# OpenVisualCloud/SVT-VP9

Hardware: AMD Instinct MI355X
Metric: hot-path frames/sec (+ Mpixels/sec): block-level DSP path (picture analysis + ME + inter prediction from reconstructed references + DCT/quant/recon + deblock + reference padding), 3840x2160p60 yuv420p enc-mode 8; no mode decision, no entropy coding -- not encoded frames (higher is better)
Workload: dtype u8

## Files before the change

### svt-vp9_amd/csrc/encdec.hip

```cpp
#include <hip/hip_runtime.h>
#include <stdlib.h>
#include <string.h>
#include "svt_ctx.h"
#include "encdec_core.h"

#define ED_MAX_PICS 32
#define ED_MAX_SETS 8

struct svt_encdec_work {
    int           max_pics, width, height, n_sb, sb_cols, mi_rows, mi_cols;
    size_t        cap_per_pic;
    svt_tq_block *d_blocks;
    void         *last_hb;
    uint32_t     *d_pos;
    uint16_t     *d_eob;
    int32_t      *d_counts;
    int32_t      *d_totals, *d_bases;
    int32_t      *d_off_cnt;
    int32_t      *d_status;
    int32_t      *d_intra_sync;
    svt_quant_tables *d_qtabs;
    int16_t      *d_iscan;
    svt_encdec_stage_hook hook;
    void         *hook_user;
};

namespace {

struct ed_pic_dev {
    const svt_me_pu_result *res;
    svt_mc_mode_info       *mc_mi;
    svt_lf_mode_info       *lf_mi;
    uint8_t                *nz;
    uint16_t               *eob_map;
    svt_lf_mask            *lfm;
    svt_tq_pic_geom         g;
};
struct ed_batch_dev {
    ed_pic_dev pic[ED_MAX_PICS];
    uint32_t   iscan_off[16];
    int32_t    n_pics, n_sb, sb_cols, mi_rows, mi_cols, mi_stride, width, height;
    uint32_t   lambda;
    int32_t    filter_level;
};

__device__ __forceinline__ int wave_sum(int v) {
    _Pragma("unroll") for (int d = 32; d >= 1; d >>= 1) v += __shfl_xor(v, d, 64);
    return v;
}
__device__ __forceinline__ int wave_excl_prefix(int v, int lane) {
    int incl = v;
    _Pragma("unroll") for (int d = 1; d < 64; d <<= 1) {
        const int o = __shfl_up(incl, d, 64);
        if (lane >= d) incl += o;
    }
    return incl - v;
}

__global__ __launch_bounds__(64) void svt_tq_count_kernel(const ed_batch_dev *__restrict__ B, int32_t *__restrict__ counts, int32_t *__restrict__ status) {
    const int sb = (int)blockIdx.x % B->n_sb, pic = (int)blockIdx.x / B->n_sb, lane = (int)threadIdx.x;
    const ed_pic_dev &P = B->pic[pic];
    const int ur = (sb / B->sb_cols) * 8 + (lane >> 3), uc = (sb % B->sb_cols) * 8 + (lane & 7);
    int cnt[4] = {0, 0, 0, 0};
    if (ur < B->mi_rows && uc < B->mi_cols) P.nz[ur * B->mi_stride + uc] = 0;
    const int o = svt_tq_unit_is_origin(P.lf_mi, B->mi_stride, B->mi_rows, B->mi_cols, ur, uc);
    if (o < 0) atomicOr(status, 1);
    if (o == 1) svt_tq_unit_counts(P.lf_mi, B->mi_stride, ur, uc, cnt);
    _Pragma("unroll") for (int s = 0; s < 4; s++) {
        const int v = wave_sum(cnt[s]);
        if (lane == 0) counts[(s * B->n_pics + pic) * B->n_sb + sb] = v;
    }
}

__global__ __launch_bounds__(256) void svt_scan_sb_kernel(int32_t *__restrict__ a, int n_sb, int32_t *__restrict__ totals) {
    __shared__ int32_t part[256];
    int32_t *p = a + (size_t)blockIdx.x * n_sb;
    const int t = (int)threadIdx.x, per = (n_sb + 255) / 256, b = t * per, e = b + per < n_sb ? b + per : n_sb;
    int s = 0;
    for (int i = b; i < e; i++) s += p[i];
    part[t] = s;
    __syncthreads();
    for (int d = 1; d < 256; d <<= 1) {
        const int v = t >= d ? part[t - d] : 0;
        __syncthreads();
        part[t] += v;
        __syncthreads();
    }
    int run = part[t] - s;
    for (int i = b; i < e; i++) { const int v = p[i]; p[i] = run; run += v; }
    if (t == 255) totals[blockIdx.x] = part[255];
}
__global__ __launch_bounds__(64) void svt_scan_pic_kernel(const int32_t *__restrict__ totals, int n_pics, int32_t *__restrict__ bases, int32_t *__restrict__ off_cnt) {
    if (threadIdx.x != 0) return;
    int run = 0;
    for (int s = 0; s < 4; s++) {
        off_cnt[s] = run;
        for (int p = 0; p < n_pics; p++) { bases[s * n_pics + p] = run; run += totals[s * n_pics + p]; }
        off_cnt[4 + s] = run - off_cnt[s];
    }
}

__global__ __launch_bounds__(256) void svt_tq_expand_kernel(const ed_batch_dev *__restrict__ B, const int32_t *__restrict__ off_cnt, const uint32_t *__restrict__ pos,
                                                           svt_tq_block *__restrict__ blocks) {
    const int i = (int)blockIdx.x * 256 + (int)threadIdx.x, total = off_cnt[3] + off_cnt[7];
    if (i >= total) return;
    const int      ts = i >= off_cnt[3] ? 3 : i >= off_cnt[2] ? 2 : i >= off_cnt[1] ? 1 : 0;
    const uint32_t p = pos[i];
    svt_tq_block   k;
    svt_tq_block_from_pos(p, ts, &B->pic[svt_tq_pos_pic(p)].g, B->iscan_off, B->sb_cols, &k);
    blocks[i] = k;
}

__global__ __launch_bounds__(64) void svt_tq_emit_kernel(const ed_batch_dev *__restrict__ B, const int32_t *__restrict__ offsets, const int32_t *__restrict__ bases,
                                                         svt_tq_block *__restrict__ blocks, uint32_t *__restrict__ pos) {
    const int sb = (int)blockIdx.x % B->n_sb, pic = (int)blockIdx.x / B->n_sb, lane = (int)threadIdx.x;
    const ed_pic_dev &P = B->pic[pic];
    const int ur = (sb / B->sb_cols) * 8 + (lane >> 3), uc = (sb % B->sb_cols) * 8 + (lane & 7);
    int cnt[4] = {0, 0, 0, 0};
    const int o = svt_tq_unit_is_origin(P.lf_mi, B->mi_stride, B->mi_rows, B->mi_cols, ur, uc);
    if (o == 1) svt_tq_unit_counts(P.lf_mi, B->mi_stride, ur, uc, cnt);
    uint32_t base[4];
    _Pragma("unroll") for (int s = 0; s < 4; s++) base[s] = (uint32_t)(bases[s * B->n_pics + pic] + offsets[(s * B->n_pics + pic) * B->n_sb + sb] + wave_excl_prefix(cnt[s], lane));
    if (o == 1) svt_tq_unit_emit(P.lf_mi, B->mi_stride, ur, uc, &P.g, B->iscan_off, base, blocks, pos);
}

__global__ __launch_bounds__(256) void svt_tq_skip_kernel(const ed_batch_dev *__restrict__ B, const int32_t *__restrict__ off_cnt, const uint32_t *__restrict__ pos,
                                                          const uint16_t *__restrict__ eob) {
    const int total = off_cnt[3] + off_cnt[7];
    const int w4 = B->width >> 2, h4 = B->height >> 2;
    for (int i = (int)(blockIdx.x * blockDim.x + threadIdx.x); i < total; i += (int)(gridDim.x * blockDim.x)) {
        const uint32_t p = pos[i];
        const int      pic = (int)(p >> 24) & 63, plane = (int)(p >> 22) & 3, y4 = (int)(p >> 11) & 0x7ff, x4 = (int)p & 0x7ff;
        const ed_pic_dev &P = B->pic[pic];
        const int      e = eob[i];
        const int      pw4 = plane ? w4 >> 1 : w4;
        const int      off = plane == 0 ? 0 : w4 * h4 + (plane == 2 ? (w4 >> 1) * (h4 >> 1) : 0);
        P.eob_map[off + y4 * pw4 + x4] = (uint16_t)e;
        if (e) {
            const int uy = plane ? y4 : y4 >> 1, ux = plane ? x4 : x4 >> 1;
            const svt_lf_mode_info b = P.lf_mi[uy * B->mi_stride + ux];
            const int w8 = svt_blk_w8(b.sb_type), h8 = svt_blk_h8(b.sb_type);
            P.nz[(uy - uy % h8) * B->mi_stride + (ux - ux % w8)] = 1;
        }
    }
}
__global__ __launch_bounds__(256) void svt_eob_map_clear_kernel(const ed_batch_dev *__restrict__ B, int n16) {
    uint4 *m = (uint4 *)B->pic[blockIdx.y].eob_map;
    for (int i = (int)(blockIdx.x * 256 + threadIdx.x); i < n16; i += (int)(gridDim.x * 256)) m[i] = make_uint4(0, 0, 0, 0);
}
__global__ __launch_bounds__(256) void svt_skip_update_kernel(const ed_batch_dev *__restrict__ B) {
    const int units = B->mi_rows * B->mi_cols;
    const int i = (int)(blockIdx.x * blockDim.x + threadIdx.x);
    if (i >= units * B->n_pics) return;
    const int pic = i / units, u = i % units, ur = u / B->mi_cols, uc = u % B->mi_cols;
    const ed_pic_dev &P = B->pic[pic];
    svt_lf_mode_info *b = &P.lf_mi[ur * B->mi_stride + uc];
    if (b->sb_type > 12) return;
    const int w8 = svt_blk_w8(b->sb_type), h8 = svt_blk_h8(b->sb_type);
    b->skip = P.nz[(ur - ur % h8) * B->mi_stride + (uc - uc % w8)] ? 0 : 1;
}

__device__ __forceinline__ uint32_t wave_or(uint32_t v) {
    _Pragma("unroll") for (int d = 32; d >= 1; d >>= 1) v |= (uint32_t)__shfl_xor((int)v, d, 64);
    return v;
}
__global__ __launch_bounds__(64) void svt_lf_mask_kernel(const ed_batch_dev *__restrict__ B, int32_t *__restrict__ status) {
    const int sb = (int)blockIdx.x % B->n_sb, pic = (int)blockIdx.x / B->n_sb, lane = (int)threadIdx.x;
    const ed_pic_dev &P = B->pic[pic];
    svt_lf_unit_masks u;
    svt_lf_mask_unit(P.lf_mi, B->mi_stride, B->mi_rows, B->mi_cols, sb / B->sb_cols, sb % B->sb_cols, lane >> 3, lane & 7, &u);
    if (u.bad && status) atomicOr(status, 1);
    __shared__ uint32_t sm[40];
    uint64_t            w64[9];
    _Pragma("unroll") for (int i = 0; i < 4; i++) { w64[i] = u.left_y[i]; w64[4 + i] = u.above_y[i]; }
    w64[8] = u.int_4x4_y;
    _Pragma("unroll") for (int i = 0; i < 9; i++) {
        const uint32_t lo = wave_or((uint32_t)w64[i]), hi = wave_or((uint32_t)(w64[i] >> 32));
        if (lane == i) { sm[2 * i] = lo; sm[2 * i + 1] = hi; }
    }
    const uint32_t c0 = wave_or((uint32_t)u.left_uv[0] | (uint32_t)u.left_uv[1] << 16), c1 = wave_or((uint32_t)u.left_uv[2] | (uint32_t)u.left_uv[3] << 16);
    const uint32_t c2 = wave_or((uint32_t)u.above_uv[0] | (uint32_t)u.above_uv[1] << 16), c3 = wave_or((uint32_t)u.above_uv[2] | (uint32_t)u.above_uv[3] << 16);
    const uint32_t c4 = wave_or((uint32_t)u.int_4x4_uv);
    if (lane == 9) { sm[18] = c0; sm[19] = c1; sm[20] = c2; sm[21] = c3; sm[22] = c4; sm[38] = 0; sm[39] = 0; }
    __syncthreads();
    ((uint8_t *)sm)[90 + lane] = u.level;
    __syncthreads();
    if (lane < 40) ((uint32_t *)&P.lfm[sb])[lane] = sm[lane];
}

__global__ __launch_bounds__(64) void svt_md_default_kernel(const ed_batch_dev *__restrict__ B) {
    const int sb = (int)blockIdx.x % B->n_sb, pic = (int)blockIdx.x / B->n_sb, lane = (int)threadIdx.x;
    const ed_pic_dev &P = B->pic[pic];
    const int r = lane >> 3, c = lane & 7, sr = sb / B->sb_cols, sc = sb % B->sb_cols, ur = sr * 8 + r, uc = sc * 8 + c;
    if (ur >= B->mi_rows || uc >= B->mi_cols) return;
    svt_md_default_unit(P.res + (size_t)sb * SVT_ME_PU_COUNT, r, c, sr, sc, B->mi_rows, B->mi_cols, B->lambda, B->filter_level, &P.mc_mi[ur * B->mi_stride + uc],
                        &P.lf_mi[ur * B->mi_stride + uc]);
}

int stage_batch(svt_hip_ctx *ctx, const ed_batch_dev &hb, const ed_batch_dev **d_out) {
    void *h = nullptr, *d = nullptr;
    if (svt_ctx_stage(ctx, sizeof hb, &h, &d)) return -1;
    memcpy(h, &hb, sizeof hb);
    if (hipMemcpyAsync(d, h, sizeof hb, hipMemcpyHostToDevice, ctx->stream) != hipSuccess) return -1;
    svt_ctx_stage_commit(ctx);
    *d_out = (const ed_batch_dev *)d;
    return 0;
}

void fill_dims(ed_batch_dev &hb, int n_pics, int width, int height, int mi_stride) {
    hb.n_pics = n_pics; hb.width = width; hb.height = height;
    hb.sb_cols = (width + 63) >> 6;
    hb.n_sb = hb.sb_cols * ((height + 63) >> 6);
    hb.mi_rows = height >> 3; hb.mi_cols = width >> 3; hb.mi_stride = mi_stride;
}

}

extern "C" int32_t svt_hip_encdec_work_create(svt_hip_ctx *ctx, int32_t max_pics, int32_t width, int32_t height, svt_encdec_work **out) {
    if (!ctx || !out || max_pics < 1 || max_pics > ED_MAX_PICS || width < 8 || height < 8 || (width & 7) || (height & 7))
        return svt_set_error(SVT_HIP_ERR_BAD_PARAMETER, "encdec_work: bad argument");
    HIP_TRY(hipSetDevice(ctx->device));
    svt_encdec_work *w = (svt_encdec_work *)calloc(1, sizeof *w);
    if (!w) return svt_set_error(SVT_HIP_ERR_NO_RESOURCES, "encdec_work: malloc");
    w->max_pics = max_pics; w->width = width; w->height = height;
    w->sb_cols = (width + 63) >> 6; w->n_sb = w->sb_cols * ((height + 63) >> 6);
    w->mi_rows = height >> 3; w->mi_cols = width >> 3;
    w->cap_per_pic = (size_t)width * height * 3 / 32;
    const size_t cap = w->cap_per_pic * (size_t)max_pics;
    const size_t n_cnt = (size_t)4 * max_pics * w->n_sb;
    uint32_t const *offs = nullptr;
    int32_t         entries = 0;
    const int16_t  *isc = svt_hip_vp9_iscan_tables(&offs, &entries);
    bool ok = hipMalloc((void **)&w->d_pos, cap * sizeof(uint32_t)) == hipSuccess &&
              hipMalloc((void **)&w->d_eob, cap * sizeof(uint16_t)) == hipSuccess &&
              hipMalloc((void **)&w->d_counts, (n_cnt + 9 + 8 * ED_MAX_PICS + 2 + 48 * (size_t)w->n_sb) * sizeof(int32_t)) == hipSuccess &&
              hipMalloc((void **)&w->d_qtabs, 2 * sizeof(svt_quant_tables)) == hipSuccess && hipMalloc((void **)&w->d_iscan, (size_t)entries * sizeof(int16_t)) == hipSuccess;
    if (ok) {
        w->d_off_cnt = w->d_counts + n_cnt;
        w->d_status = w->d_off_cnt + 8;
        w->d_totals = w->d_status + 1;
        w->d_bases = w->d_totals + 4 * ED_MAX_PICS;
        w->d_intra_sync = w->d_bases + 4 * ED_MAX_PICS;
        ok = hipMemsetAsync(w->d_off_cnt, 0, 9 * sizeof(int32_t), ctx->stream) == hipSuccess &&
             hipMemcpyAsync(w->d_iscan, isc, (size_t)entries * sizeof(int16_t), hipMemcpyHostToDevice, ctx->stream) == hipSuccess &&
             hipStreamSynchronize(ctx->stream) == hipSuccess;
    }
    if (!ok) {
        svt_hip_encdec_work_destroy(ctx, w);
        return svt_set_error(SVT_HIP_ERR_NO_RESOURCES, "encdec_work: device memory");
    }
    *out = w;
    return SVT_HIP_OK;
}

extern "C" void svt_hip_encdec_work_destroy(svt_hip_ctx *ctx, svt_encdec_work *w) {
    if (!w) return;
    if (ctx) { (void)hipSetDevice(ctx->device); (void)hipStreamSynchronize(ctx->stream); }
    void *v[6] = {w->d_blocks, w->d_pos, w->d_eob, w->d_counts, w->d_qtabs, w->d_iscan};
    for (int i = 0; i < 6; i++) if (v[i]) (void)hipFree(v[i]);
    free(w->last_hb);
    free(w);
}

extern "C" int32_t svt_hip_encdec_batch_device(svt_hip_ctx *ctx, svt_encdec_work *w, int32_t n_pics, const svt_encdec_picture *pics, int32_t width,
                                               int32_t height, int32_t mi_stride, int32_t q_index, const svt_encdec_flags *flags, const svt_lf_thresh *thr,
                                               int32_t pad_x, int32_t pad_y) {
    if (!ctx || !w || !pics || !flags || n_pics < 1 || n_pics > w->max_pics || width != w->width || height != w->height || mi_stride < (width >> 3))
        return svt_set_error(SVT_HIP_ERR_BAD_PARAMETER, "encdec: bad argument");
    if (flags->apply_loop_filter && !thr) return svt_set_error(SVT_HIP_ERR_BAD_PARAMETER, "encdec: loop filter without thresholds");
    HIP_TRY(hipSetDevice(ctx->device));
    uintptr_t src_lo = UINTPTR_MAX, src_hi = 0, pred_lo = UINTPTR_MAX, pred_hi = 0;
    for (int i = 0; i < n_pics; i++) {
        const svt_encdec_picture &p = pics[i];
        if (!p.d_mc_mi || !p.d_lf_mi || !p.src.y || !p.src.u || !p.src.v || !p.pred.y || !p.pred.u || !p.pred.v || !p.recon.y || !p.recon.u || !p.recon.v ||
            !p.d_qcoeff || !p.d_eob_map || !p.d_nz || (flags->apply_loop_filter && !p.d_lfm))
            return svt_set_error(SVT_HIP_ERR_BAD_PARAMETER, "encdec: null picture field");
        if (!p.d_dqcoeff != !pics[0].d_dqcoeff) return svt_set_error(SVT_HIP_ERR_BAD_PARAMETER, "encdec: d_dqcoeff must be given for every picture of a batch or for none");
        if (((uintptr_t)p.d_qcoeff | (uintptr_t)p.d_dqcoeff) & 15) return svt_set_error(SVT_HIP_ERR_BAD_PARAMETER, "encdec: coefficient arrays must be 16-byte aligned");
        const uint8_t *s3[3] = {p.src.y, p.src.u, p.src.v}, *p3[3] = {p.pred.y, p.pred.u, p.pred.v};
        for (int k = 0; k < 3; k++) {
            src_lo = (uintptr_t)s3[k] < src_lo ? (uintptr_t)s3[k] : src_lo; src_hi = (uintptr_t)s3[k] > src_hi ? (uintptr_t)s3[k] : src_hi;
            pred_lo = (uintptr_t)p3[k] < pred_lo ? (uintptr_t)p3[k] : pred_lo; pred_hi = (uintptr_t)p3[k] > pred_hi ? (uintptr_t)p3[k] : pred_hi;
        }
    }
    uint64_t plane_span = 0;
    for (int i = 0; i < n_pics; i++) {
        const svt_yuv_planes *pl[3] = {&pics[i].src, &pics[i].pred, &pics[i].recon};
        for (int k = 0; k < 3; k++) {
            const uint64_t a = (uint64_t)(pl[k]->y_stride > 0 ? pl[k]->y_stride : 0) * (uint64_t)height, b = (uint64_t)(pl[k]->uv_stride > 0 ? pl[k]->uv_stride : 0) * (uint64_t)(height / 2);
            plane_span = a > plane_span ? a : plane_span;
            plane_span = b > plane_span ? b : plane_span;
        }
    }
    if ((uint64_t)(src_hi - src_lo) + plane_span >= (1ull << 32) || (uint64_t)(pred_hi - pred_lo) + plane_span >= (1ull << 32))
        return svt_set_error(SVT_HIP_ERR_BAD_PARAMETER, "encdec: the batch's source / prediction planes must lie within 4 GB");
    uintptr_t q_lo = UINTPTR_MAX, dq_lo = UINTPTR_MAX;
    for (int i = 0; i < n_pics; i++) {
        q_lo = (uintptr_t)pics[i].d_qcoeff < q_lo ? (uintptr_t)pics[i].d_qcoeff : q_lo;
        dq_lo = (uintptr_t)pics[i].d_dqcoeff < dq_lo ? (uintptr_t)pics[i].d_dqcoeff : dq_lo;
    }
    ed_batch_dev hb;
    memset(&hb, 0, sizeof hb);
    fill_dims(hb, n_pics, width, height, mi_stride);
    {
        const uint32_t *offs = nullptr;
        (void)svt_hip_vp9_iscan_tables(&offs, nullptr);
        for (int i = 0; i < 16; i++) hb.iscan_off[i] = offs[i];
    }
    uint8_t       *recon_set[ED_MAX_SETS];
    int            n_sets = 0;
    {
        uintptr_t lo[ED_MAX_PICS], hi[ED_MAX_PICS];
        int       order[ED_MAX_PICS];
        for (int i = 0; i < n_pics; i++) {
            const uint8_t *r3[3] = {pics[i].recon.y, pics[i].recon.u, pics[i].recon.v};
            lo[i] = UINTPTR_MAX; hi[i] = 0; order[i] = i;
            for (int k = 0; k < 3; k++) { lo[i] = (uintptr_t)r3[k] < lo[i] ? (uintptr_t)r3[k] : lo[i]; hi[i] = (uintptr_t)r3[k] > hi[i] ? (uintptr_t)r3[k] : hi[i]; }
        }
        for (int a = 1; a < n_pics; a++)
            for (int b = a; b > 0 && lo[order[b]] < lo[order[b - 1]]; b--) { const int t_ = order[b]; order[b] = order[b - 1]; order[b - 1] = t_; }
        for (int a = 0; a < n_pics; a++) {
            const int i = order[a];
            if (n_sets && (uint64_t)(hi[i] - (uintptr_t)recon_set[n_sets - 1]) + plane_span < (1ull << 32)) continue;
            if (n_sets == ED_MAX_SETS || (uint64_t)(hi[i] - lo[i]) + plane_span >= (1ull << 32))
                return svt_set_error(SVT_HIP_ERR_BAD_PARAMETER, "encdec: the batch's reconstruction buffers span more than 8 regions of 4 GB");
            recon_set[n_sets++] = (uint8_t *)lo[i];
        }
    }
    svt_mc_picture mcp[ED_MAX_PICS];
    svt_yuv_planes rec[ED_MAX_PICS], rec_pad[ED_MAX_PICS];
    int            n_rec_pad = 0;
    const svt_lf_mask *lfm[ED_MAX_PICS];
    int32_t        lfm_stride[ED_MAX_PICS], mi_rows_a[ED_MAX_PICS], mi_cols_a[ED_MAX_PICS];
    for (int i = 0; i < n_pics; i++) {
        const svt_encdec_picture &p = pics[i];
        ed_pic_dev &P = hb.pic[i];
        P.mc_mi = (svt_mc_mode_info *)p.d_mc_mi; P.lf_mi = p.d_lf_mi; P.nz = p.d_nz; P.eob_map = p.d_eob_map; P.lfm = p.d_lfm;
        const uintptr_t q_off = ((uintptr_t)p.d_qcoeff - q_lo) / sizeof(int16_t), dq_off = ((uintptr_t)p.d_dqcoeff - dq_lo) / sizeof(int16_t);
        if ((p.d_dqcoeff && q_off != dq_off) || q_off + (uint64_t)hb.n_sb * SVT_SB_COEFFS >= (1ull << 32))
            return svt_set_error(SVT_HIP_ERR_BAD_PARAMETER, "encdec: qcoeff / dqcoeff of the batch must be laid out alike, within 2^32 elements");
        const uint8_t *r3[3] = {p.recon.y, p.recon.u, p.recon.v};
        uintptr_t r_lo = UINTPTR_MAX, r_hi = 0;
        for (int k = 0; k < 3; k++) { r_lo = (uintptr_t)r3[k] < r_lo ? (uintptr_t)r3[k] : r_lo; r_hi = (uintptr_t)r3[k] > r_hi ? (uintptr_t)r3[k] : r_hi; }
        int set = -1;
        for (int k = n_sets - 1; k >= 0 && set < 0; k--)
            if (r_lo >= (uintptr_t)recon_set[k] && (uint64_t)(r_hi - (uintptr_t)recon_set[k]) + plane_span < (1ull << 32)) set = k;
        if (set < 0) return svt_set_error(SVT_HIP_ERR_BAD_PARAMETER, "encdec: the batch's reconstruction buffers span more than 8 regions of 4 GB");
        svt_tq_pic_geom &g = P.g;
        const uint8_t *s3[3] = {p.src.y, p.src.u, p.src.v}, *p3[3] = {p.pred.y, p.pred.u, p.pred.v};
        for (int k = 0; k < 3; k++) {
            g.src_off[k] = (uint32_t)((uintptr_t)s3[k] - src_lo); g.pred_off[k] = (uint32_t)((uintptr_t)p3[k] - pred_lo);
            g.recon_off[k] = (uint32_t)((uintptr_t)r3[k] - (uintptr_t)recon_set[set]);
        }
        if (p.src.y_stride > 65535 || p.pred.y_stride > 65535 || p.recon.y_stride > 65535) return svt_set_error(SVT_HIP_ERR_BAD_PARAMETER, "encdec: stride");
        g.src_stride[0] = (uint16_t)p.src.y_stride; g.src_stride[1] = (uint16_t)p.src.uv_stride;
        g.pred_stride[0] = (uint16_t)p.pred.y_stride; g.pred_stride[1] = (uint16_t)p.pred.uv_stride;
        g.recon_stride[0] = (uint16_t)p.recon.y_stride; g.recon_stride[1] = (uint16_t)p.recon.uv_stride;
        g.coeff_base = (uint32_t)q_off; g.width = width; g.height = height; g.recon_set = (uint8_t)set; g.pic = (uint8_t)i; g.do_recon = flags->do_recon ? 1 : 0;
        mcp[i].d_mi = p.d_mc_mi; mcp[i].mi_stride = mi_stride; mcp[i].mi_rows = hb.mi_rows; mcp[i].mi_cols = hb.mi_cols;
        mcp[i].ref[0] = p.ref[0]; mcp[i].ref[1] = p.ref[1]; mcp[i].pred = p.pred; mcp[i].use_subpel = p.use_subpel;
        rec[i] = p.recon; rec[i].width = width; rec[i].height = height;
        if (!p.no_pad) rec_pad[n_rec_pad++] = rec[i];
        lfm[i] = p.d_lfm; lfm_stride[i] = hb.sb_cols; mi_rows_a[i] = hb.mi_rows; mi_cols_a[i] = hb.mi_cols;
    }
    const ed_batch_dev *dB = nullptr;
    if (stage_batch(ctx, hb, &dB)) return svt_set_error(SVT_HIP_ERR_NO_RESOURCES, "encdec: descriptor buffers");
    {
        svt_quant_tables qt[2];
        if (svt_hip_quant_tables_for_qindex(q_index, qt) != SVT_HIP_OK) return svt_set_error(SVT_HIP_ERR_BAD_PARAMETER, "encdec: q index");
        void *h = nullptr, *d = nullptr;
        if (svt_ctx_stage(ctx, sizeof qt, &h, &d)) return svt_set_error(SVT_HIP_ERR_NO_RESOURCES, "encdec: descriptor buffers");
        memcpy(h, qt, sizeof qt);
        HIP_TRY(hipMemcpyAsync(w->d_qtabs, h, sizeof qt, hipMemcpyHostToDevice, ctx->stream));
        svt_ctx_stage_commit(ctx);
    }
#define ED_STAGE(k) do { if (w->hook) w->hook(w->hook_user, (k)); } while (0)
    ED_STAGE(SVT_ENCDEC_STAGE_MC);
    int32_t rc = svt_hip_inter_pred_batch_device(ctx, n_pics, mcp);
    if (rc) return rc;
    ED_STAGE(SVT_ENCDEC_STAGE_LISTS);
    const int nwg = n_pics * hb.n_sb;
    hipLaunchKernelGGL(svt_tq_count_kernel, dim3(nwg), dim3(64), 0, ctx->stream, dB, w->d_counts, w->d_status);
    hipLaunchKernelGGL(svt_scan_sb_kernel, dim3(4 * n_pics), dim3(256), 0, ctx->stream, w->d_counts, hb.n_sb, w->d_totals);
    hipLaunchKernelGGL(svt_scan_pic_kernel, dim3(1), dim3(64), 0, ctx->stream, (const int32_t *)w->d_totals, n_pics, w->d_bases, w->d_off_cnt);
    hipLaunchKernelGGL(svt_tq_emit_kernel, dim3(nwg), dim3(64), 0, ctx->stream, dB, (const int32_t *)w->d_counts, (const int32_t *)w->d_bases, (svt_tq_block *)nullptr, w->d_pos);
    HIP_TRY(hipGetLastError());
    if (!w->last_hb) w->last_hb = malloc(sizeof hb);
    if (w->last_hb) memcpy(w->last_hb, &hb, sizeof hb);
    ED_STAGE(SVT_ENCDEC_STAGE_TQ);
    int32_t cap[4];
    for (int s = 0; s < 4; s++) cap[s] = (int32_t)((size_t)n_pics * width * height * 3 / 2 / (size_t)(16 << (2 * s)));
    rc = svt_tq_launch_device_lists(ctx, (const uint8_t *)src_lo, (const uint8_t *)pred_lo, recon_set, n_sets, nullptr, cap, w->d_off_cnt, w->d_qtabs, w->d_iscan,
                                    (int16_t *)q_lo, (int16_t *)dq_lo, w->d_eob, nullptr, w->d_pos, &dB->pic[0].g, (int)sizeof(ed_pic_dev), dB->iscan_off, hb.sb_cols);
    if (rc) return rc;
    ED_STAGE(SVT_ENCDEC_STAGE_SKIP);
    {
        const size_t map_bytes = (size_t)(width / 4) * (height / 4) * 3 / 2 * sizeof(uint16_t);
        uintptr_t    low = map_bytes;
        for (int i = 0; i < n_pics; i++) low |= (uintptr_t)pics[i].d_eob_map;
        if (!(low & 15))
            hipLaunchKernelGGL(svt_eob_map_clear_kernel, dim3(64, n_pics), dim3(256), 0, ctx->stream, dB, (int)(map_bytes / 16));
        else
            for (int i = 0; i < n_pics; i++) HIP_TRY(hipMemsetAsync(pics[i].d_eob_map, 0, map_bytes, ctx->stream));
    }
    for (int i = 0; i < n_pics; i++)
        if (pics[i].has_intra) {
            if (!flags->do_recon) return svt_set_error(SVT_HIP_ERR_BAD_PARAMETER, "encdec: intra blocks need the reconstruction (do_recon)");
            rc = svt_intra_launch(ctx, &pics[i], width, height, mi_stride, w->d_qtabs, w->d_iscan, hb.iscan_off, w->d_intra_sync, w->d_status, 1);
            if (rc) return rc;
        }
    {
        const int total_cap = (int)(w->cap_per_pic * (size_t)n_pics);
        int       g = (total_cap + 255) / 256;
        if (g > ctx->cu_count * 8) g = ctx->cu_count * 8;
        hipLaunchKernelGGL(svt_tq_skip_kernel, dim3(g), dim3(256), 0, ctx->stream, dB, (const int32_t *)w->d_off_cnt, (const uint32_t *)w->d_pos, (const uint16_t *)w->d_eob);
        hipLaunchKernelGGL(svt_skip_update_kernel, dim3((n_pics * hb.mi_rows * hb.mi_cols + 255) / 256), dim3(256), 0, ctx->stream, dB);
        HIP_TRY(hipGetLastError());
    }
    ED_STAGE(SVT_ENCDEC_STAGE_LF);
    if (flags->apply_loop_filter) {
        hipLaunchKernelGGL(svt_lf_mask_kernel, dim3(nwg), dim3(64), 0, ctx->stream, dB, w->d_status);
        HIP_TRY(hipGetLastError());
        rc = svt_hip_lf_batch_device(ctx, n_pics, rec, lfm, lfm_stride, thr, mi_rows_a, mi_cols_a, 0);
        if (rc) return rc;
    }
    ED_STAGE(SVT_ENCDEC_STAGE_PAD);
    if (flags->pad_reference && n_rec_pad) {
        rc = svt_hip_ref_pad_batch_device(ctx, n_rec_pad, rec_pad, pad_x, pad_y);
        if (rc) return rc;
    }
    ED_STAGE(SVT_ENCDEC_STAGE_END);
    return SVT_HIP_OK;
}

extern "C" int32_t svt_hip_encdec_intra_device(svt_hip_ctx *ctx, svt_encdec_work *w, const svt_encdec_picture *pic, int32_t width, int32_t height, int32_t mi_stride,
                                               int32_t q_index, const svt_encdec_flags *flags, const svt_lf_thresh *thr, int32_t pad_x, int32_t pad_y) {
    if (!ctx || !w || !pic || !flags || width != w->width || height != w->height || mi_stride < (width >> 3))
        return svt_set_error(SVT_HIP_ERR_BAD_PARAMETER, "encdec_intra: bad argument");
    if (!flags->do_recon) return svt_set_error(SVT_HIP_ERR_BAD_PARAMETER, "encdec_intra: intra prediction needs the reconstruction (do_recon)");
    if (flags->apply_loop_filter && !thr) return svt_set_error(SVT_HIP_ERR_BAD_PARAMETER, "encdec_intra: loop filter without thresholds");
    const svt_encdec_picture &p = *pic;
    if (!p.d_lf_mi || !p.src.y || !p.src.u || !p.src.v || !p.recon.y || !p.recon.u || !p.recon.v || !p.d_qcoeff || !p.d_eob_map || !p.d_nz ||
        (flags->apply_loop_filter && !p.d_lfm))
        return svt_set_error(SVT_HIP_ERR_BAD_PARAMETER, "encdec_intra: null picture field");
    if (((uintptr_t)p.d_qcoeff | (uintptr_t)p.d_dqcoeff) & 15) return svt_set_error(SVT_HIP_ERR_BAD_PARAMETER, "encdec_intra: coefficient arrays must be 16-byte aligned");
    if (p.recon.y_stride > 65535 || ((p.src.y_stride | p.src.uv_stride | p.recon.y_stride | p.recon.uv_stride) & 3) ||
        (((uintptr_t)p.src.y | (uintptr_t)p.src.u | (uintptr_t)p.src.v | (uintptr_t)p.recon.y | (uintptr_t)p.recon.u | (uintptr_t)p.recon.v) & 3) ||
        (p.pred.y && (((uintptr_t)p.pred.y | (uintptr_t)p.pred.u | (uintptr_t)p.pred.v | (uintptr_t)p.pred.y_stride | (uintptr_t)p.pred.uv_stride) & 3)))
        return svt_set_error(SVT_HIP_ERR_BAD_PARAMETER, "encdec_intra: planes and strides must be 4-byte aligned");
    if (p.pred.y && (!p.pred.u || !p.pred.v)) return svt_set_error(SVT_HIP_ERR_BAD_PARAMETER, "encdec_intra: prediction planes");
    HIP_TRY(hipSetDevice(ctx->device));
    ed_batch_dev hb;
    memset(&hb, 0, sizeof hb);
    fill_dims(hb, 1, width, height, mi_stride);
    const uint32_t *offs = nullptr;
    (void)svt_hip_vp9_iscan_tables(&offs, nullptr);
    hb.pic[0].lf_mi = p.d_lf_mi; hb.pic[0].nz = p.d_nz; hb.pic[0].eob_map = p.d_eob_map; hb.pic[0].lfm = p.d_lfm;
    const ed_batch_dev *dB = nullptr;
    if (stage_batch(ctx, hb, &dB)) return svt_set_error(SVT_HIP_ERR_NO_RESOURCES, "encdec_intra: descriptor buffers");
    {
        svt_quant_tables qt[2];
        if (svt_hip_quant_tables_for_qindex(q_index, qt) != SVT_HIP_OK) return svt_set_error(SVT_HIP_ERR_BAD_PARAMETER, "encdec_intra: q index");
        void *h = nullptr, *d = nullptr;
        if (svt_ctx_stage(ctx, sizeof qt, &h, &d)) return svt_set_error(SVT_HIP_ERR_NO_RESOURCES, "encdec_intra: descriptor buffers");
        memcpy(h, qt, sizeof qt);
        HIP_TRY(hipMemcpyAsync(w->d_qtabs, h, sizeof qt, hipMemcpyHostToDevice, ctx->stream));
        svt_ctx_stage_commit(ctx);
    }
    ED_STAGE(SVT_ENCDEC_STAGE_TQ);
    HIP_TRY(hipMemsetAsync(p.d_eob_map, 0, (size_t)(width / 4) * (height / 4) * 3 / 2 * sizeof(uint16_t), ctx->stream));
    HIP_TRY(hipMemsetAsync(p.d_nz, 0, (size_t)mi_stride * hb.mi_rows, ctx->stream));
    int32_t rc = svt_intra_launch(ctx, pic, width, height, mi_stride, w->d_qtabs, w->d_iscan, offs, w->d_intra_sync, w->d_status, 0);
    if (rc) return rc;
    ED_STAGE(SVT_ENCDEC_STAGE_SKIP);
    hipLaunchKernelGGL(svt_skip_update_kernel, dim3((hb.mi_rows * hb.mi_cols + 255) / 256), dim3(256), 0, ctx->stream, dB);
    HIP_TRY(hipGetLastError());
    ED_STAGE(SVT_ENCDEC_STAGE_LF);
    svt_yuv_planes rec = p.recon;
    rec.width = width; rec.height = height;
    if (flags->apply_loop_filter) {
        hipLaunchKernelGGL(svt_lf_mask_kernel, dim3(hb.n_sb), dim3(64), 0, ctx->stream, dB, w->d_status);
        HIP_TRY(hipGetLastError());
        const svt_lf_mask *lfm = p.d_lfm;
        const int32_t      lfm_stride = hb.sb_cols, mr = hb.mi_rows, mc = hb.mi_cols;
        rc = svt_hip_lf_batch_device(ctx, 1, &rec, &lfm, &lfm_stride, thr, &mr, &mc, 0);
        if (rc) return rc;
    }
    ED_STAGE(SVT_ENCDEC_STAGE_PAD);
    if (flags->pad_reference && !p.no_pad) {
        rc = svt_hip_ref_pad_batch_device(ctx, 1, &rec, pad_x, pad_y);
        if (rc) return rc;
    }
    ED_STAGE(SVT_ENCDEC_STAGE_END);
    return SVT_HIP_OK;
}

extern "C" int32_t svt_hip_md_intra_default_device(svt_hip_ctx *ctx, int32_t width, int32_t height, int32_t filter_level, svt_lf_mode_info *d_lf_mi, int32_t mi_stride) {
    if (!ctx || !d_lf_mi || width < 8 || height < 8 || (width & 7) || (height & 7) || mi_stride < (width >> 3))
        return svt_set_error(SVT_HIP_ERR_BAD_PARAMETER, "md_intra_default: bad argument");
    HIP_TRY(hipSetDevice(ctx->device));
    return svt_md_intra_default_launch(ctx, d_lf_mi, mi_stride, height >> 3, width >> 3, filter_level);
}

extern "C" void svt_hip_encdec_work_set_stage_hook(svt_encdec_work *w, svt_encdec_stage_hook hook, void *user) {
    if (!w) return;
    w->hook = hook;
    w->hook_user = user;
}

extern "C" int32_t svt_hip_encdec_work_status(svt_hip_ctx *ctx, svt_encdec_work *w, int32_t counts[8]) {
    if (!ctx || !w) return svt_set_error(SVT_HIP_ERR_BAD_PARAMETER, "encdec_status: null");
    HIP_TRY(hipSetDevice(ctx->device));
    int32_t h[9];
    HIP_TRY(hipMemcpyAsync(h, w->d_off_cnt, sizeof h, hipMemcpyDeviceToHost, ctx->stream));
    HIP_TRY(hipStreamSynchronize(ctx->stream));
    if (counts) memcpy(counts, h, 8 * sizeof(int32_t));
    if (h[8]) {
        HIP_TRY(hipMemsetAsync(w->d_status, 0, sizeof(int32_t), ctx->stream));
        return svt_set_error(SVT_HIP_ERR_BAD_PARAMETER, "encdec: malformed mode-info grid (block outside the picture, misaligned, or transform larger than its block)");
    }
    return SVT_HIP_OK;
}

extern "C" int32_t svt_hip_encdec_work_download(svt_hip_ctx *ctx, svt_encdec_work *w, svt_tq_block *blocks, uint32_t *pos, uint16_t *eob, int32_t capacity) {
    int32_t c[8];
    const int32_t rc = svt_hip_encdec_work_status(ctx, w, c);
    if (rc) return rc;
    const int32_t total = c[3] + c[7];
    if (total > capacity) return svt_set_error(SVT_HIP_ERR_NO_RESOURCES, "encdec_download: capacity");
    if (total > 0) {
        if (blocks) {
            if (!w->last_hb) return svt_set_error(SVT_HIP_ERR_BAD_PARAMETER, "encdec_download: no batch yet");
            if (!w->d_blocks && hipMalloc((void **)&w->d_blocks, w->cap_per_pic * (size_t)w->max_pics * sizeof(svt_tq_block)) != hipSuccess) {
                w->d_blocks = nullptr;
                return svt_set_error(SVT_HIP_ERR_NO_RESOURCES, "encdec_download: device memory");
            }
            const ed_batch_dev *dB = nullptr;
            if (stage_batch(ctx, *(const ed_batch_dev *)w->last_hb, &dB)) return svt_set_error(SVT_HIP_ERR_NO_RESOURCES, "encdec_download: descriptor buffers");
            hipLaunchKernelGGL(svt_tq_expand_kernel, dim3((total + 255) / 256), dim3(256), 0, ctx->stream, dB, (const int32_t *)w->d_off_cnt, (const uint32_t *)w->d_pos, w->d_blocks);
            HIP_TRY(hipGetLastError());
            HIP_TRY(hipMemcpyAsync(blocks, w->d_blocks, (size_t)total * sizeof(svt_tq_block), hipMemcpyDeviceToHost, ctx->stream));
        }
        if (pos) HIP_TRY(hipMemcpyAsync(pos, w->d_pos, (size_t)total * sizeof(uint32_t), hipMemcpyDeviceToHost, ctx->stream));
        if (eob) HIP_TRY(hipMemcpyAsync(eob, w->d_eob, (size_t)total * sizeof(uint16_t), hipMemcpyDeviceToHost, ctx->stream));
        HIP_TRY(hipStreamSynchronize(ctx->stream));
    }
    return total;
}

extern "C" int32_t svt_hip_md_default_batch_device(svt_hip_ctx *ctx, int32_t n_pics, const svt_me_pu_result *const *d_results, int32_t width, int32_t height,
                                                   uint32_t lambda, int32_t filter_level, svt_mc_mode_info *const *d_mc_mi, svt_lf_mode_info *const *d_lf_mi,
                                                   int32_t mi_stride) {
    if (!ctx || n_pics < 1 || !d_results || !d_mc_mi || !d_lf_mi || width < 8 || height < 8 || (width & 7) || (height & 7) || mi_stride < (width >> 3))
        return svt_set_error(SVT_HIP_ERR_BAD_PARAMETER, "md_default: bad argument");
    HIP_TRY(hipSetDevice(ctx->device));
    for (int first = 0; first < n_pics; first += ED_MAX_PICS) {
        const int n = n_pics - first < ED_MAX_PICS ? n_pics - first : ED_MAX_PICS;
        ed_batch_dev hb;
        memset(&hb, 0, sizeof hb);
        fill_dims(hb, n, width, height, mi_stride);
        hb.lambda = lambda; hb.filter_level = filter_level;
        for (int i = 0; i < n; i++) {
            if (!d_results[first + i] || !d_mc_mi[first + i] || !d_lf_mi[first + i]) return svt_set_error(SVT_HIP_ERR_BAD_PARAMETER, "md_default: null picture");
            hb.pic[i].res = d_results[first + i]; hb.pic[i].mc_mi = d_mc_mi[first + i]; hb.pic[i].lf_mi = d_lf_mi[first + i];
        }
        const ed_batch_dev *dB = nullptr;
        if (stage_batch(ctx, hb, &dB)) return svt_set_error(SVT_HIP_ERR_NO_RESOURCES, "md_default: descriptor buffers");
        hipLaunchKernelGGL(svt_md_default_kernel, dim3(n * hb.n_sb), dim3(64), 0, ctx->stream, dB);
        HIP_TRY(hipGetLastError());
    }
    return SVT_HIP_OK;
}

extern "C" int32_t svt_hip_lf_build_masks_device(svt_hip_ctx *ctx, int32_t n_pics, const svt_lf_mode_info *const *d_lf_mi, int32_t mi_stride, int32_t mi_rows,
                                                 int32_t mi_cols, svt_lf_mask *const *d_lfm) {
    if (!ctx || n_pics < 1 || !d_lf_mi || !d_lfm || mi_rows < 1 || mi_cols < 1 || mi_stride < mi_cols) return svt_set_error(SVT_HIP_ERR_BAD_PARAMETER, "lf_masks: bad argument");
    HIP_TRY(hipSetDevice(ctx->device));
    for (int first = 0; first < n_pics; first += ED_MAX_PICS) {
        const int n = n_pics - first < ED_MAX_PICS ? n_pics - first : ED_MAX_PICS;
        ed_batch_dev hb;
        memset(&hb, 0, sizeof hb);
        fill_dims(hb, n, mi_cols * 8, mi_rows * 8, mi_stride);
        for (int i = 0; i < n; i++) {
            if (!d_lf_mi[first + i] || !d_lfm[first + i]) return svt_set_error(SVT_HIP_ERR_BAD_PARAMETER, "lf_masks: null picture");
            hb.pic[i].lf_mi = (svt_lf_mode_info *)d_lf_mi[first + i]; hb.pic[i].lfm = d_lfm[first + i];
        }
        const ed_batch_dev *dB = nullptr;
        if (stage_batch(ctx, hb, &dB)) return svt_set_error(SVT_HIP_ERR_NO_RESOURCES, "lf_masks: descriptor buffers");
        hipLaunchKernelGGL(svt_lf_mask_kernel, dim3(n * hb.n_sb), dim3(64), 0, ctx->stream, dB, (int32_t *)nullptr);
        HIP_TRY(hipGetLastError());
    }
    return SVT_HIP_OK;
}
```

### svt-vp9_amd/csrc/lf_kernel.hip

```cpp
#include <hip/hip_runtime.h>
#include <cstdio>
#include <cstdlib>
#include "svt_ctx.h"

namespace {

struct lf_pic_dev {
    svt_yuv_planes     planes;
    const svt_lf_mask *lfm;
    int32_t            lfm_stride, mi_rows, mi_cols, y_only;
    uint32_t          *progress;
    const uint32_t    *desc;
};

__device__ unsigned long long g_lf_prof[8];
__device__ unsigned long long g_lf_rowts[64][8];

constexpr int LF_DESC_WORDS = 320;
constexpr int YS = 76, YROWS = 72;
constexpr int CS = 44, CROWS = 40;

__device__ __forceinline__ int iabs(int v) { return v < 0 ? -v : v; }
__device__ __forceinline__ int sclamp(int t) { return t < -128 ? -128 : t > 127 ? 127 : t; }
__device__ __forceinline__ int uclamp(int t) { return t < 0 ? 0 : t > 255 ? 255 : t; }
// ... 195 lines not shown
    lf_fetch<ROW>(s, st, nxt);
    for (int c = 0; c < nblk; c++) {
        lf_unpack<ROW>(nxt, q);
        const uint32_t e0 = w0, e1 = w1;
        if (c + 1 < nblk) {
            w0 = tab[2 * (c + 1) * tstep]; w1 = tab[2 * (c + 1) * tstep + 1];
            lf_fetch<ROW>(ROW ? s + 8 * (c + 1) : s + 8 * (c + 1) * st, st, nxt);
        }
        lf_block_edges(p, q, e0);
        if (ROW) row_store8(s + 8 * c - 8, p, true); else col_store8(s + (8 * c - 8) * st, st, p, true);
        lf_inner_edge(q, e1);
        _Pragma("unroll") for (int i = 0; i < 8; i++) p[i] = q[7 - i];
    }
    if (ROW) row_store8(s + 8 * nblk - 8, p, true); else col_store8(s + (8 * nblk - 8) * st, st, p, true);
}

struct lf_magic_table {
    uint32_t v[33];
    constexpr lf_magic_table() : v() { for (uint32_t d = 1; d <= 32; d++) v[d] = (uint32_t)(0xffffffffu / d) + 1u; }
};
__constant__ const lf_magic_table lf_magics = lf_magic_table();
__device__ __forceinline__ int lf_udiv(int t, int d, uint32_t inv) { return d > 32 ? t / d : inv ? (int)__umulhi((uint32_t)t, inv) : t; }

template <int UNITS, typename UT>
__device__ __forceinline__ void tile_io_t(bool load, uint8_t *g, int gstride, uint8_t *l, int lstride, int x0, int y0, int tx0, int ty0,
                                          int nx, int ny, int seam_lo_end, int seam_hi_begin, int lane, int nlanes,
                                          const volatile int LF_LDS *wait_flag, int wait_val) {
    constexpr int UB = (int)sizeof(UT);
    const int nu = nx / UB, total = nu * ny;
    const uint32_t inv = lf_magics.v[nu <= 32 ? nu : 0];
    for (int t0 = lane; t0 < total; t0 += UNITS * nlanes) {
        UT  v[UNITS];
        int lo[UNITS];
        _Pragma("unroll") for (int u = 0; u < UNITS; u++) {
            const int t = t0 + u * nlanes;
            lo[u] = -1;
            if (t < total) {
                const int  r = lf_udiv(t, nu, inv), ty = ty0 + r, tx = tx0 + UB * (t - r * nu);
                UT LF_GLOBAL *gp = LF_AS_GLOBAL(UT, g + (ptrdiff_t)(y0 + ty) * gstride + x0 + tx);
                const bool seam = ty < seam_lo_end || ty >= seam_hi_begin;
                lo[u] = ty * lstride + tx;
                if (load) v[u] = seam ? __hip_atomic_load(gp, __ATOMIC_RELAXED, __HIP_MEMORY_SCOPE_AGENT) : *gp;
                else {
                    const uint32_t *lp = (const uint32_t *)(l + lo[u]);
                    UT              w = (UT)lp[0];
                    if constexpr (UB == 8) w |= (UT)lp[1] << 32;
                    if (seam) __hip_atomic_store(gp, w, __ATOMIC_RELAXED, __HIP_MEMORY_SCOPE_AGENT);
                    else *gp = w;
                }
            }
        }
        if (load) {
            if (wait_flag) while (*wait_flag < wait_val) __builtin_amdgcn_s_sleep(1);
            _Pragma("unroll") for (int u = 0; u < UNITS; u++)
                if (lo[u] >= 0) {
                    uint32_t *lp = (uint32_t *)(l + lo[u]);
                    lp[0] = (uint32_t)v[u];
                    if constexpr (UB == 8) lp[1] = (uint32_t)(v[u] >> 32);
                }
        }
    }
}
template <int UNITS>
__device__ __forceinline__ void tile_io(bool wide, bool load, uint8_t *g, int gstride, uint8_t *l, int lstride, int x0, int y0, int tx0,
                                        int ty0, int nx, int ny, int seam_lo_end, int seam_hi_begin, int lane, int nlanes,
                                        const volatile int LF_LDS *wait_flag = nullptr, int wait_val = 0) {
    if (wide) tile_io_t<UNITS, unsigned long long>(load, g, gstride, l, lstride, x0, y0, tx0, ty0, nx, ny, seam_lo_end, seam_hi_begin, lane, nlanes, wait_flag, wait_val);
    else tile_io_t<2 * UNITS, unsigned int>(load, g, gstride, l, lstride, x0, y0, tx0, ty0, nx, ny, seam_lo_end, seam_hi_begin, lane, nlanes, wait_flag, wait_val);
}

struct lf_geom {
    int x0, y0, cx0, cy0, hx, hy, vw, vh, cvw, cvh;
};
__device__ __forceinline__ lf_geom lf_geometry(int sb_row, int sc, int W, int H) {
    lf_geom g;
    const int CW = W >> 1, CH = H >> 1;
    g.x0 = sc * 64; g.y0 = sb_row * 64; g.cx0 = sc * 32; g.cy0 = sb_row * 32;
    g.hx = sc > 0 ? 8 : 0; g.hy = sb_row > 0 ? 8 : 0;
    g.vw = (W - g.x0) < 64 ? W - g.x0 : 64; g.vh = (H - g.y0) < 64 ? H - g.y0 : 64;
    g.cvw = (CW - g.cx0) < 32 ? CW - g.cx0 : 32; g.cvh = (CH - g.cy0) < 32 ? CH - g.cy0 : 32;
    return g;
}

__global__ __launch_bounds__(128) void svt_lf_desc_kernel(const lf_pic_dev *__restrict__ pics, int rows_per_pic, int max_cols, svt_lf_thresh thr) {
    __shared__ uint32_t s_thr[64];
    if (threadIdx.x < 64) s_thr[threadIdx.x] = (uint32_t)thr.mblim[threadIdx.x] | ((uint32_t)thr.lim[threadIdx.x] << 8) | ((uint32_t)thr.hev_thr[threadIdx.x] << 16);
    __syncthreads();
    const int pic = blockIdx.x / (rows_per_pic * max_cols), rem = blockIdx.x - pic * rows_per_pic * max_cols;
    const int sb_row = rem / max_cols, sc = rem - sb_row * max_cols;
    const lf_pic_dev P = pics[pic];
    const int sb_cols = (P.mi_cols + 7) >> 3, sb_rows = (P.mi_rows + 7) >> 3;
    if (sb_row >= sb_rows || sc >= sb_cols) return;
    const int tid = threadIdx.x, mi_row = sb_row * 8;
    uint32_t LF_GLOBAL *d = LF_AS_GLOBAL(uint32_t, const_cast<uint32_t *>(P.desc) + ((size_t)sb_row * sb_cols + sc) * LF_DESC_WORDS);
    const svt_lf_mask LF_GLOBAL *gm = LF_AS_GLOBAL(const svt_lf_mask, &P.lfm[sb_row * P.lfm_stride + sc]);
    const uint8_t LF_GLOBAL     *lfl = gm->lfl_y;
    svt_lf_mask        m;
    _Pragma("unroll") for (int i = 0; i < 4; i++) { m.left_y[i] = gm->left_y[i]; m.above_y[i] = gm->above_y[i]; m.left_uv[i] = gm->left_uv[i]; m.above_uv[i] = gm->above_uv[i]; }
    m.int_4x4_y = gm->int_4x4_y; m.int_4x4_uv = gm->int_4x4_uv;
    adjust_mask(m, mi_row, sc * 8, P.mi_rows, P.mi_cols);
    if (tid < 64) {
        const int rr = tid >> 3, c = tid & 7, pair = rr >> 1, half = rr & 1;
        uint32_t w0, w1;
        lf_entry2(vert_entry(c, 8, (unsigned)(m.left_y[2] >> (16 * pair)) & 0xffff, (unsigned)(m.left_y[1] >> (16 * pair)) & 0xffff,
                            (unsigned)(m.left_y[0] >> (16 * pair)) & 0xffff, (unsigned)(m.int_4x4_y >> (16 * pair)) & 0xffff, half,
                            lfl[(2 * pair) * 8 + c], lfl[(2 * pair + 1) * 8 + c]), s_thr, w0, w1);
        d[2 * tid] = w0; d[2 * tid + 1] = w1;
        const int r = rr;
        unsigned  a16 = 0, a8 = 0, a4 = 0;
        if (mi_row + r != 0) { a16 = (unsigned)(m.above_y[2] >> (8 * r)) & 0xff; a8 = (unsigned)(m.above_y[1] >> (8 * r)) & 0xff; a4 = (unsigned)(m.above_y[0] >> (8 * r)) & 0xff; }
        lf_entry2(horiz_entry(c, a16, a8, a4, (unsigned)(m.int_4x4_y >> (8 * r)) & 0xff, &lfl[r * 8], 1), s_thr, w0, w1);
        d[128 + 2 * tid] = w0; d[129 + 2 * tid] = w1;
    } else if (tid < 80) {
        const int t = tid - 64, rr = t >> 2, c = t & 3, pair = rr >> 1, half = rr & 1;
        uint32_t w0, w1;
        lf_entry2(vert_entry(c, 4, (unsigned)(m.left_uv[2] >> (8 * pair)) & 0xff, (unsigned)(m.left_uv[1] >> (8 * pair)) & 0xff,
                                (unsigned)(m.left_uv[0] >> (8 * pair)) & 0xff, (unsigned)(m.int_4x4_uv >> (8 * pair)) & 0xff, half,
                                lfl[(4 * pair) * 8 + 2 * c], lfl[(4 * pair + 2) * 8 + 2 * c]), s_thr, w0, w1);
        d[256 + 2 * t] = w0; d[257 + 2 * t] = w1;
    } else if (tid < 96) {
        const int t = tid - 80, ru = t >> 2, c = t & 3, r = 2 * ru;
        unsigned  a16 = 0, a8 = 0, a4 = 0;
        if (mi_row + r != 0) { a16 = (unsigned)(m.above_uv[2] >> (4 * ru)) & 0xf; a8 = (unsigned)(m.above_uv[1] >> (4 * ru)) & 0xf; a4 = (unsigned)(m.above_uv[0] >> (4 * ru)) & 0xf; }
        const unsigned mi4 = (mi_row + r == P.mi_rows - 1) ? 0u : ((unsigned)(m.int_4x4_uv >> (4 * ru)) & 0xf);
        uint32_t w0, w1;
        lf_entry2(horiz_entry(c, a16, a8, a4, mi4, &lfl[r * 8], 2), s_thr, w0, w1);
        d[288 + 2 * t] = w0; d[289 + 2 * t] = w1;
    }
}

__global__ __launch_bounds__(256) __attribute__((amdgpu_waves_per_eu(4, 4))) void svt_lf_kernel(const lf_pic_dev *__restrict__ pics, int n_pics,
                                                     uint32_t *__restrict__ ticket, int rows_per_pic, int prof) {
    __shared__ __align__(16) uint8_t ytile[2][YROWS * YS];
    __shared__ __align__(16) uint8_t ctile[2][2][CROWS * CS];
    __shared__ uint32_t              s_desc[2][LF_DESC_WORDS];
    __shared__ int                   s_job;
    __shared__ int                   s_stored_;
    __shared__ int                   s_halo_;
    __shared__ int                   s_vdone_[2];
    const int tid = threadIdx.x;
    for (;;) {
    __syncthreads();
    volatile int LF_LDS &s_stored = *(volatile int LF_LDS *)&s_stored_;
    volatile int LF_LDS &s_halo   = *(volatile int LF_LDS *)&s_halo_;
    volatile int LF_LDS *s_vdone  = (volatile int LF_LDS *)s_vdone_;
    if (tid == 0) { s_job = (int)atomicAdd(ticket, 1u); s_stored = -1; s_halo = -1; s_vdone[0] = -1; s_vdone[1] = -1; }
    __syncthreads();
    const int job = s_job;
    if (job >= n_pics * rows_per_pic) break;
    const lf_pic_dev P = pics[job % n_pics];
    const int sb_row = job / n_pics;
    const int sb_cols = (P.mi_cols + 7) >> 3, sb_rows = (P.mi_rows + 7) >> 3;
    if (sb_row >= sb_rows) continue;
    const int W = P.planes.width, H = P.planes.height;
    const int mi_row = sb_row * 8;
    const int wave = tid >> 6, lane = tid & 63;
    const int nrows = P.mi_rows - mi_row < 8 ? P.mi_rows - mi_row : 8;
    const bool wide_y = (((uintptr_t)P.planes.y | (uintptr_t)P.planes.y_stride) & 7) == 0;
    const bool wide_c = (((uintptr_t)P.planes.u | (uintptr_t)P.planes.v | (uintptr_t)P.planes.uv_stride) & 7) == 0;
    unsigned long long tm_ = prof ? __builtin_amdgcn_s_memtime() : 0;
    const bool rowts = prof && job % n_pics == 0 && sb_row < 64;
#define LF_ROWTS(k, who, cond) do { if (rowts && tid == (who) && (cond)) g_lf_rowts[sb_row][k] = __builtin_amdgcn_s_memtime(); } while (0)
    LF_ROWTS(0, 0, true);
#define LF_MARK(i, who) do { if (prof && tid == (who)) { unsigned long long n_ = __builtin_amdgcn_s_memtime(); atomicAdd(&g_lf_prof[i], n_ - tm_); tm_ = n_; } } while (0)

    auto stage_halo = [&](int sc) {
        const int     buf = sc & 1;
// ... 30 lines not shown

    if (wave == 2) stage(0);
    __syncthreads();
    for (int sc = 0; sc < sb_cols; sc++) {
        const int     buf = sc & 1;
        const lf_geom g = lf_geometry(sb_row, sc, W, H);
        const bool    last = sc + 1 == sb_cols;
        if (wave == 2) {
            stage_halo(sc);
            if (!last) stage(sc + 1);
        } else if (wave == 0) {
            if (lane < g.vh) lf_line<true>(ytile[buf] + (8 + lane) * YS + 8, 1, 8, &s_desc[buf][2 * (lane >> 3) * 8], 1);
            if (lane == 0) s_vdone[0] = sc;
            LF_ROWTS(4, 0, sc == 1);
            LF_MARK(3, 0);
            while (s_halo < sc) __builtin_amdgcn_s_sleep(1);
            if (lane < g.vw) lf_line<false>(ytile[buf] + 8 * YS + 8 + lane, YS, nrows, &s_desc[buf][128 + 2 * (lane >> 3)], 8);
            LF_MARK(4, 0);
            LF_ROWTS(2, 0, sc == 0);
            LF_ROWTS(5, 0, last);
            if (!last) {
                while (s_stored < sc - 1) __builtin_amdgcn_s_sleep(1);
                for (int r = lane; r < YROWS; r += 64) {
                    const uint32_t *src = (const uint32_t *)(ytile[buf] + r * YS + 64);
                    uint32_t       *dst = (uint32_t *)(ytile[buf ^ 1] + r * YS);
                    dst[0] = src[0]; dst[1] = src[1];
                }
            }
        } else if (wave == 1 && !P.y_only) {
            const int pl = lane >> 5, l5 = lane & 31;
            if (l5 < g.cvh) lf_line<true>(ctile[buf][pl] + (8 + l5) * CS + 8, 1, 4, &s_desc[buf][256 + 2 * (l5 >> 3) * 4], 1);
            if (lane == 0) s_vdone[1] = sc;
            while (s_halo < sc) __builtin_amdgcn_s_sleep(1);
            if (l5 < g.cvw) lf_line<false>(ctile[buf][pl] + 8 * CS + 8 + l5, CS, (nrows + 1) >> 1, &s_desc[buf][288 + 2 * (l5 >> 3)], 4);
            if (!last) {
                while (s_stored < sc - 1) __builtin_amdgcn_s_sleep(1);
                for (int r = l5; r < CROWS; r += 32) {
                    const uint32_t *src = (const uint32_t *)(ctile[buf][pl] + r * CS + 32);
                    uint32_t       *dst = (uint32_t *)(ctile[buf ^ 1][pl] + r * CS);
                    dst[0] = src[0]; dst[1] = src[1];
                }
            }
        }
        __syncthreads();
        LF_MARK(5, 0);
        if (wave == 3) {
            const bool below = sb_row + 1 < sb_rows;
            const int  nown = last ? g.vw : 56, nownc = last ? g.cvw : 24, cut = below ? 8 : 0;
            tile_io<11>(wide_y, false, P.planes.y, P.planes.y_stride, ytile[buf], YS, g.x0 - 8, g.y0 - 8, 8, 8 - g.hy, nown, g.vh + g.hy, 8, 8 + g.vh - 8, lane, 64);
            if (g.hx) tile_io<2>(wide_y, false, P.planes.y, P.planes.y_stride, ytile[buf], YS, g.x0 - 8, g.y0 - 8, 0, 8 - g.hy, 8, g.vh + g.hy - cut, 8, 8 + g.vh - 8, lane, 64);
            if (!P.y_only) {
                _Pragma("unroll") for (int pl = 0; pl < 2; pl++) {
                    uint8_t *cp = pl ? P.planes.v : P.planes.u;
                    tile_io<3>(wide_c, false, cp, P.planes.uv_stride, ctile[buf][pl], CS, g.cx0 - 8, g.cy0 - 8, 8, 8 - g.hy, nownc, g.cvh + g.hy, 8, 8 + g.cvh - 8, lane, 64);
                    if (g.hx) tile_io<1>(wide_c, false, cp, P.planes.uv_stride, ctile[buf][pl], CS, g.cx0 - 8, g.cy0 - 8, 0, 8 - g.hy, 8, g.cvh + g.hy - cut, 8, 8 + g.cvh - 8, lane, 64);
                }
            }
            asm volatile("s_waitcnt lgkmcnt(0)" ::: "memory");
            if (lane == 0) s_stored = sc;
            LF_MARK(6, 192);
            if (!last && below) {
                while (s_vdone[0] < sc + 1) __builtin_amdgcn_s_sleep(1);
                const lf_geom gn = lf_geometry(sb_row, sc + 1, W, H);
                tile_io<1>(wide_y, false, P.planes.y, P.planes.y_stride, ytile[buf ^ 1], YS, gn.x0 - 8, gn.y0 - 8, 0, 8 + gn.vh - 8, 8, 8, 1 << 20, 0, lane, 64);
                if (!P.y_only) {
                    while (s_vdone[1] < sc + 1) __builtin_amdgcn_s_sleep(1);
                    tile_io<1>(wide_c, false, P.planes.u, P.planes.uv_stride, ctile[buf ^ 1][0], CS, gn.cx0 - 8, gn.cy0 - 8, 0, 8 + gn.cvh - 8, 8, 8, 1 << 20, 0, lane, 64);
                    tile_io<1>(wide_c, false, P.planes.v, P.planes.uv_stride, ctile[buf ^ 1][1], CS, gn.cx0 - 8, gn.cy0 - 8, 0, 8 + gn.cvh - 8, 8, 8, 1 << 20, 0, lane, 64);
                }
            }
            asm volatile("s_waitcnt vmcnt(0)" ::: "memory");
            if (lane == 0) __hip_atomic_store(LF_AS_GLOBAL(uint32_t, &P.progress[sb_row]), (uint32_t)(sc + 1), __ATOMIC_RELAXED, __HIP_MEMORY_SCOPE_AGENT);
            LF_ROWTS(3, 192, sc == 0);
            LF_ROWTS(6, 192, last);
            LF_MARK(7, 192);
        }
    }
#undef LF_MARK
#undef LF_ROWTS
    }
}
}

static int32_t lf_launch(svt_hip_ctx *ctx, int n_pics, const svt_yuv_planes *d_recon, const svt_lf_mask *const *d_lfm, const int32_t *lfm_stride,
                         const svt_lf_thresh *thr, const int32_t *mi_rows, const int32_t *mi_cols, int32_t y_only) {
    int max_rows = 0, max_cols = 0;
    for (int i = 0; i < n_pics; i++) {
        if (mi_rows[i] < 1 || mi_cols[i] < 1 || d_recon[i].width != mi_cols[i] * 8 || d_recon[i].height != mi_rows[i] * 8)
            return svt_set_error(SVT_HIP_ERR_BAD_PARAMETER, "lf: plane size must be mi_cols*8 x mi_rows*8");
        const svt_yuv_planes &pl = d_recon[i];
        if ((((uintptr_t)pl.y | (uintptr_t)pl.y_stride) & 3) || (!y_only && (((uintptr_t)pl.u | (uintptr_t)pl.v | (uintptr_t)pl.uv_stride) & 3)))
            return svt_set_error(SVT_HIP_ERR_BAD_PARAMETER, "lf: plane pointers and strides must be multiples of 4 bytes");
        const int r = (mi_rows[i] + 7) / 8, cc = (mi_cols[i] + 7) / 8;
        if (r > max_rows) max_rows = r;
        if (cc > max_cols) max_cols = cc;
    }
    HIP_TRY(hipSetDevice(ctx->device));
    const size_t desc_bytes = (sizeof(lf_pic_dev) * (size_t)n_pics + 15) & ~(size_t)15;
    const size_t cnt_words  = (size_t)n_pics * max_rows + 4;
    lf_pic_dev  *h = nullptr;
    uint8_t     *d = nullptr;
    if (svt_ctx_stage(ctx, desc_bytes + cnt_words * 4, (void **)&h, (void **)&d)) return svt_set_error(SVT_HIP_ERR_NO_RESOURCES, "lf: scratch");
    uint32_t *cnt = (uint32_t *)(d + desc_bytes);
    uint32_t *edesc = (uint32_t *)svt_ctx_slot(ctx, 24, (size_t)n_pics * max_rows * max_cols * LF_DESC_WORDS * sizeof(uint32_t));
    if (!edesc) return svt_set_error(SVT_HIP_ERR_NO_RESOURCES, "lf: descriptor buffer");
    for (int i = 0; i < n_pics; i++) {
        h[i].planes = d_recon[i]; h[i].lfm = d_lfm[i]; h[i].lfm_stride = lfm_stride[i]; h[i].mi_rows = mi_rows[i]; h[i].mi_cols = mi_cols[i];
        h[i].y_only = y_only; h[i].progress = cnt + 4 + (size_t)i * max_rows;
        h[i].desc = edesc + (size_t)i * max_rows * max_cols * LF_DESC_WORDS;
    }
    HIP_TRY(hipMemcpyAsync(d, h, sizeof(lf_pic_dev) * (size_t)n_pics, hipMemcpyHostToDevice, ctx->stream));
    HIP_TRY(hipMemsetAsync(cnt, 0, cnt_words * 4, ctx->stream));
    HIP_TRY(hipEventRecord(ctx->ev_start, ctx->stream));
    static const bool want_prof = getenv("SVT_HIP_LF_PROFILE") != nullptr;
    if (want_prof) { unsigned long long z[8] = {0}; HIP_TRY(hipMemcpyToSymbol(HIP_SYMBOL(g_lf_prof), z, sizeof z)); }
    hipLaunchKernelGGL(svt_lf_desc_kernel, dim3(n_pics * max_rows * max_cols), dim3(128), 0, ctx->stream, (const lf_pic_dev *)d, max_rows, max_cols, *thr);
    hipLaunchKernelGGL(svt_lf_kernel, dim3(n_pics * max_rows), dim3(256), 0, ctx->stream, (const lf_pic_dev *)d, n_pics, cnt, max_rows, want_prof ? 1 : 0);
    HIP_TRY(hipGetLastError());
    HIP_TRY(hipEventRecord(ctx->ev_stop, ctx->stream));
    if (want_prof) {
        unsigned long long hp[8];
        HIP_TRY(hipStreamSynchronize(ctx->stream));
        HIP_TRY(hipMemcpyFromSymbol(hp, HIP_SYMBOL(g_lf_prof), sizeof hp));
        static const char *nm[8] = {"io:wait", "io:tile_load", "io:descriptors", "filter:vertical", "filter:horizontal+halo", "filter:barrier",
                                    "io:tile_store", "io:publish"};
        unsigned long long tot = 0, steps = 0;
        for (int i = 3; i < 6; i++) tot += hp[i];
        for (int i = 0; i < n_pics; i++) steps += (unsigned long long)((mi_rows[i] + 7) / 8) * ((mi_cols[i] + 7) / 8);
        fprintf(stderr, "[lf-profile] pics=%d SB steps=%llu avg cycles/SB=%llu :", n_pics, steps, tot / (steps ? steps : 1));
        for (int i = 0; i < 8; i++) fprintf(stderr, " %s=%.1f%%", nm[i], 100.0 * (double)hp[i] / (double)tot);
        fprintf(stderr, "\n");
        if (getenv("SVT_HIP_LF_ROWTS")) {
            static unsigned long long ts[64][8];
            HIP_TRY(hipMemcpyFromSymbol(ts, HIP_SYMBOL(g_lf_rowts), sizeof ts));
            for (int r = 0; r < max_rows && r < 64; r++) {
                fprintf(stderr, "[lf-rows] row %2d:", r);
                for (int k = 0; k < 7; k++) fprintf(stderr, " %9.2f", (double)(ts[r][k] - ts[0][0]) / 100.0);
                fprintf(stderr, "  (us: taken, halo 0, SB 0 done, publish 1, V(SB 1) done, last SB done, row complete)\n");
            }
        }
    }
    svt_ctx_stage_commit(ctx);
    ctx->timed = 1;
    return SVT_HIP_OK;
}

extern "C" int32_t svt_hip_lf_reserve(svt_hip_ctx *ctx, int32_t n_pics, int32_t mi_rows, int32_t mi_cols) {
    if (!ctx || n_pics < 1 || mi_rows < 1 || mi_cols < 1) return svt_set_error(SVT_HIP_ERR_BAD_PARAMETER, "lf_reserve: bad argument");
    HIP_TRY(hipSetDevice(ctx->device));
    const size_t rows = (size_t)(mi_rows + 7) / 8, cols = (size_t)(mi_cols + 7) / 8;
    if (!svt_ctx_slot(ctx, 24, (size_t)n_pics * rows * cols * LF_DESC_WORDS * sizeof(uint32_t))) return svt_set_error(SVT_HIP_ERR_NO_RESOURCES, "lf: descriptor buffer");
    return SVT_HIP_OK;
}

extern "C" int32_t svt_hip_lf_frame_device(svt_hip_ctx *ctx, const svt_yuv_planes *d_recon, const svt_lf_mask *d_lfm, int32_t lfm_stride,
                                           const svt_lf_thresh *thr, int32_t mi_rows, int32_t mi_cols, int32_t y_only) {
    if (!ctx || !d_recon || !d_lfm || !thr) return svt_set_error(SVT_HIP_ERR_BAD_PARAMETER, "lf: null argument");
    return lf_launch(ctx, 1, d_recon, &d_lfm, &lfm_stride, thr, &mi_rows, &mi_cols, y_only);
}

extern "C" int32_t svt_hip_lf_batch_device(svt_hip_ctx *ctx, int32_t n_pics, const svt_yuv_planes *d_recon, const svt_lf_mask *const *d_lfm,
                                           const int32_t *lfm_stride, const svt_lf_thresh *thr, const int32_t *mi_rows,
                                           const int32_t *mi_cols, int32_t y_only) {
    if (!ctx || n_pics < 1 || !d_recon || !d_lfm || !lfm_stride || !thr || !mi_rows || !mi_cols)
        return svt_set_error(SVT_HIP_ERR_BAD_PARAMETER, "lf: null argument");
    return lf_launch(ctx, n_pics, d_recon, d_lfm, lfm_stride, thr, mi_rows, mi_cols, y_only);
}

extern "C" int32_t svt_hip_lf_frame(svt_hip_ctx *ctx, const svt_yuv_planes *recon, const svt_lf_mask *lfm, int32_t lfm_stride,
                                    const svt_lf_thresh *thr, int32_t mi_rows, int32_t mi_cols, int32_t y_only) {
    if (!ctx || !recon || !lfm || !thr || !recon->y || (!y_only && (!recon->u || !recon->v)))
        return svt_set_error(SVT_HIP_ERR_BAD_PARAMETER, "lf: null argument");
    HIP_TRY(hipSetDevice(ctx->device));
    const int    H = recon->height, CH = H / 2;
    const size_t yb = (size_t)recon->y_stride * H, cb = (size_t)recon->uv_stride * CH;
    const int    sb_rows = (mi_rows + 7) / 8;
    const size_t mb = sizeof(svt_lf_mask) * (size_t)sb_rows * lfm_stride;
    uint8_t *dy = (uint8_t *)svt_ctx_slot(ctx, 20, yb + 64), *du = (uint8_t *)svt_ctx_slot(ctx, 21, cb + 64), *dv = (uint8_t *)svt_ctx_slot(ctx, 22, cb + 64);
    svt_lf_mask *dm = (svt_lf_mask *)svt_ctx_slot(ctx, 23, mb);
    if (!dy || !du || !dv || !dm) return svt_set_error(SVT_HIP_ERR_NO_RESOURCES, "lf: device buffers");
    HIP_TRY(hipMemcpyAsync(dy, recon->y, yb, hipMemcpyHostToDevice, ctx->stream));
    if (!y_only) {
        HIP_TRY(hipMemcpyAsync(du, recon->u, cb, hipMemcpyHostToDevice, ctx->stream));
        HIP_TRY(hipMemcpyAsync(dv, recon->v, cb, hipMemcpyHostToDevice, ctx->stream));
    }
    HIP_TRY(hipMemcpyAsync(dm, lfm, mb, hipMemcpyHostToDevice, ctx->stream));
    svt_yuv_planes d = *recon;
    d.y = dy; d.u = du; d.v = dv;
    int32_t rc = svt_hip_lf_frame_device(ctx, &d, dm, lfm_stride, thr, mi_rows, mi_cols, y_only);
    if (rc) return rc;
    HIP_TRY(hipMemcpyAsync(recon->y, dy, yb, hipMemcpyDeviceToHost, ctx->stream));
    if (!y_only) {
        HIP_TRY(hipMemcpyAsync(recon->u, du, cb, hipMemcpyDeviceToHost, ctx->stream));
        HIP_TRY(hipMemcpyAsync(recon->v, dv, cb, hipMemcpyDeviceToHost, ctx->stream));
    }
    HIP_TRY(hipStreamSynchronize(ctx->stream));
    return SVT_HIP_OK;
}
```

### svt-vp9_amd/csrc/mc_kernel.hip

```cpp
#include <hip/hip_runtime.h>
#include "svt_ctx.h"

namespace {

struct mc_pic_dev {
    const svt_mc_mode_info *mi;
    int32_t        mi_stride, mi_rows, mi_cols;
    svt_yuv_planes ref[2];
    svt_yuv_planes pred;
    int32_t        use_subpel;
};

#define PK(a, b, c, d) ((uint32_t)(uint8_t)(int8_t)(a) | (uint32_t)(uint8_t)(int8_t)(b) << 8 | (uint32_t)(uint8_t)(int8_t)(c) << 16 | (uint32_t)(uint8_t)(int8_t)(d) << 24)
__constant__ uint32_t c_tap_lo[16] = {PK(0, 0, 0, 0), PK(0, 1, -5, 126), PK(-1, 3, -10, 122), PK(-1, 4, -13, 118), PK(-1, 4, -16, 112), PK(-1, 5, -18, 105),
                                      PK(-1, 5, -19, 97), PK(-1, 6, -19, 88), PK(-1, 6, -19, 78), PK(-1, 5, -18, 68), PK(-1, 5, -16, 58), PK(-1, 4, -14, 48),
                                      PK(-1, 4, -11, 37), PK(-1, 3, -9, 27), PK(0, 2, -6, 18), PK(0, 1, -3, 8)};
__constant__ uint32_t c_tap_hi[16] = {PK(0, 0, 0, 0), PK(8, -3, 1, 0), PK(18, -6, 2, 0), PK(27, -9, 3, -1), PK(37, -11, 4, -1), PK(48, -14, 4, -1),
                                      PK(58, -16, 5, -1), PK(68, -18, 5, -1), PK(78, -19, 6, -1), PK(88, -19, 6, -1), PK(97, -19, 5, -1), PK(105, -18, 5, -1),
                                      PK(112, -16, 4, -1), PK(118, -13, 4, -1), PK(122, -10, 3, -1), PK(126, -5, 1, 0)};

typedef uint32_t u32x4a4 __attribute__((ext_vector_type(4), aligned(4)));

__device__ __forceinline__ uint32_t alignbyte(uint32_t hi, uint32_t lo, uint32_t sh) { return __builtin_amdgcn_alignbyte(hi, lo, sh); }
__device__ __forceinline__ int clampi(int v, int lo, int hi) { return v < lo ? lo : v > hi ? hi : v; }
// ... 31 lines not shown
        const int      bias = 128 * 128 + 64;
        int            a0 = __builtin_amdgcn_sdot4((int)b1, (int)th, dot4_bias(b0, tl, bias), false);
        int            a1 = __builtin_amdgcn_sdot4((int)alignbyte(b2, b1, 1), (int)th, dot4_bias(alignbyte(b1, b0, 1), tl, bias), false);
        int            a2 = __builtin_amdgcn_sdot4((int)alignbyte(b2, b1, 2), (int)th, dot4_bias(alignbyte(b1, b0, 2), tl, bias), false);
        int            a3 = __builtin_amdgcn_sdot4((int)alignbyte(b2, b1, 3), (int)th, dot4_bias(alignbyte(b1, b0, 3), tl, bias), false);
        const uint32_t f = pack4(finish(a0), finish(a1), finish(a2), finish(a3));
        mid[r] = sx ? f : alignbyte(e1, e0, 3);
    }
    if (!any_sy) {
        _Pragma("unroll") for (int yy = 0; yy < NR; yy++) out[yy] = mid[yy + 3];
        return;
    }
    uint32_t col[4][NG];
    _Pragma("unroll") for (int g = 0; g < NG; g++) {
        const uint32_t r0 = mid[4 * g] ^ 0x80808080u, r1 = mid[4 * g + 1] ^ 0x80808080u, r2 = mid[4 * g + 2] ^ 0x80808080u;
        const uint32_t r3 = 4 * g + 3 < NM ? mid[4 * g + 3] ^ 0x80808080u : 0u;
        const uint32_t a0 = __builtin_amdgcn_perm(r1, r0, 0x05010400u), a1 = __builtin_amdgcn_perm(r1, r0, 0x07030602u);
        const uint32_t q0 = __builtin_amdgcn_perm(r3, r2, 0x05010400u), q1 = __builtin_amdgcn_perm(r3, r2, 0x07030602u);
        col[0][g] = __builtin_amdgcn_perm(q0, a0, 0x05040100u); col[1][g] = __builtin_amdgcn_perm(q0, a0, 0x07060302u);
        col[2][g] = __builtin_amdgcn_perm(q1, a1, 0x05040100u); col[3][g] = __builtin_amdgcn_perm(q1, a1, 0x07060302u);
    }
    const uint32_t vl = c_tap_lo[sy], vh = c_tap_hi[sy];
    _Pragma("unroll") for (int yy = 0; yy < NR; yy++) {
        uint32_t o[4];
        const int g0 = yy >> 2, sft = yy & 3;
        _Pragma("unroll") for (int j = 0; j < 4; j++) {
            const uint32_t lo = sft ? alignbyte(col[j][g0 + 1], col[j][g0], sft) : col[j][g0], hi = sft ? alignbyte(col[j][g0 + 2], col[j][g0 + 1], sft) : col[j][g0 + 1];
            o[j] = finish(__builtin_amdgcn_sdot4((int)hi, (int)vh, dot4_bias(lo, vl, 128 * 128 + 64), false));
        }
        out[yy] = sy ? pack4(o[0], o[1], o[2], o[3]) : mid[yy + 3];
    }
}

template <int NR>
__device__ __forceinline__ void mc_unit(const mc_pic_dev &P, int plane, int mi_row, int mi_col, int x, int y) {
    const uint32_t MC_GLOBAL *mp = MC_AS_GLOBAL(const uint32_t, P.mi + (size_t)mi_row * P.mi_stride + mi_col);
    const uint32_t  m0 = mp[0], m1 = mp[1], m2 = mp[2];
    const int       rl0 = (int8_t)(m2 & 0xff), rl1 = (int8_t)((m2 >> 8) & 0xff), bw8 = (int)((m2 >> 16) & 0xff), bh8 = (int)(m2 >> 24);
    if (rl0 < 0 || bw8 < 1 || bh8 < 1) return;
    const int ss = plane ? 1 : 0;
    const int bc = mi_col - mi_col % bw8, br = mi_row - mi_row % bh8;
    const int to_left = -(bc * 64), to_right = (P.mi_cols - bw8 - bc) * 64, to_top = -(br * 64), to_bottom = (P.mi_rows - bh8 - br) * 64;
    const int bw = (bw8 * 8) >> ss, bh = (bh8 * 8) >> ss;
    const int spel_left = (4 + bw) << 4, spel_right = spel_left - 16, spel_top = (4 + bh) << 4, spel_bottom = spel_top - 16;
    const int sc = 1 << (1 - ss);
    uint32_t  acc[NR];
    const int nref = rl1 >= 0 ? 2 : 1;
    for (int k = 0; k < nref; k++) {
        const svt_yuv_planes &R = P.ref[(k ? rl1 : rl0) ? 1 : 0];
        int mv_row = (int16_t)(k ? m0 >> 16 : m0 & 0xffff) * sc, mv_col = (int16_t)(k ? m1 >> 16 : m1 & 0xffff) * sc;
        mv_col = clampi(mv_col, to_left * sc - spel_left, to_right * sc + spel_right);
        mv_row = clampi(mv_row, to_top * sc - spel_top, to_bottom * sc + spel_bottom);
        int s_row, s_col, sx, sy;
        if (P.use_subpel) { s_row = mv_row; s_col = mv_col; sx = s_col & 15; sy = s_row & 15; }
        else if (plane) { s_row = (mv_row + 4) & ~7; s_col = (mv_col + 4) & ~7; sx = s_col & 7; sy = s_row & 7; }
        else { s_row = (mv_row + 8) & ~15; s_col = (mv_col + 8) & ~15; sx = s_col & 15; sy = s_row & 15; }
        const uint8_t *pl = plane == 0 ? R.y : plane == 1 ? R.u : R.v;
        uint32_t       o[NR];
        mc_tile<NR>(pl, plane ? R.uv_stride : R.y_stride, x, y, s_row, s_col, sx, sy, o);
        _Pragma("unroll") for (int r = 0; r < NR; r++)
            acc[r] = k ? __builtin_amdgcn_lerp(acc[r], o[r], 0x01010101u) : o[r];
    }
    uint8_t  *dp = plane == 0 ? P.pred.y : plane == 1 ? P.pred.u : P.pred.v;
    const int ds = plane ? P.pred.uv_stride : P.pred.y_stride;
    _Pragma("unroll") for (int r = 0; r < NR; r++) *MC_AS_GLOBAL(uint32_t, dp + (size_t)(y + r) * ds + x) = acc[r];
}

__global__ __launch_bounds__(128) void svt_mc_kernel(const mc_pic_dev *__restrict__ pics, int max_rows, int xblocks, int total, int chunk) {
    const int item = (int)(blockIdx.x & 7) * chunk + (int)(blockIdx.x >> 3);
    if (item >= total) return;
    const int xb = item % xblocks, rowpic = item / xblocks, mi_row = rowpic % max_rows;
    const mc_pic_dev &P = pics[rowpic / max_rows];
    const int t = threadIdx.x, wave = t >> 6, lane = t & 63;
    if (mi_row >= P.mi_rows) return;
    if (wave == 0) {
        const int mi_col = xb * 32 + (lane >> 1);
        if (mi_col < P.mi_cols) mc_unit<8>(P, 0, mi_row, mi_col, mi_col * 8 + 4 * (lane & 1), mi_row * 8);
    } else {
        const int mi_col = xb * 32 + (lane & 31);
        if (mi_col < P.mi_cols) mc_unit<4>(P, 1 + (lane >> 5), mi_row, mi_col, mi_col * 4, mi_row * 4);
    }
}

int mc_launch(svt_hip_ctx *ctx, int n_pics, const svt_mc_picture *pics) {
    int max_rows = 0, max_cols = 0;
    for (int i = 0; i < n_pics; i++) {
        const svt_mc_picture &p = pics[i];
        if (!p.d_mi || p.mi_rows < 1 || p.mi_cols < 1 || p.mi_stride < p.mi_cols || !p.pred.y || !p.pred.u || !p.pred.v)
            return svt_set_error(SVT_HIP_ERR_BAD_PARAMETER, "mc: bad picture descriptor");
        for (int l = 0; l < 2; l++)
            if (!p.ref[l].y || !p.ref[l].u || !p.ref[l].v) return svt_set_error(SVT_HIP_ERR_BAD_PARAMETER, "mc: both reference lists need planes");
        if (((uintptr_t)p.pred.y | (uintptr_t)p.pred.u | (uintptr_t)p.pred.v | (uintptr_t)p.pred.y_stride | (uintptr_t)p.pred.uv_stride) & 3)
            return svt_set_error(SVT_HIP_ERR_BAD_PARAMETER, "mc: prediction planes and strides must be multiples of 4 bytes");
        max_rows = p.mi_rows > max_rows ? p.mi_rows : max_rows;
        max_cols = p.mi_cols > max_cols ? p.mi_cols : max_cols;
    }
    mc_pic_dev *h = nullptr, *d = nullptr;
    if (svt_ctx_stage(ctx, sizeof(mc_pic_dev) * (size_t)n_pics, (void **)&h, (void **)&d)) return svt_set_error(SVT_HIP_ERR_NO_RESOURCES, "mc: scratch");
    for (int i = 0; i < n_pics; i++) {
        h[i].mi = pics[i].d_mi; h[i].mi_stride = pics[i].mi_stride; h[i].mi_rows = pics[i].mi_rows; h[i].mi_cols = pics[i].mi_cols;
        h[i].ref[0] = pics[i].ref[0]; h[i].ref[1] = pics[i].ref[1]; h[i].pred = pics[i].pred; h[i].use_subpel = pics[i].use_subpel;
    }
    HIP_TRY(hipMemcpyAsync(d, h, sizeof(mc_pic_dev) * (size_t)n_pics, hipMemcpyHostToDevice, ctx->stream));
    HIP_TRY(hipEventRecord(ctx->ev_start, ctx->stream));
    const int xblocks = (max_cols + 31) / 32, total = xblocks * max_rows * n_pics, chunk = (total + 7) / 8;
    hipLaunchKernelGGL(svt_mc_kernel, dim3(chunk * 8), dim3(128), 0, ctx->stream, (const mc_pic_dev *)d, max_rows, xblocks, total, chunk);
    HIP_TRY(hipGetLastError());
    HIP_TRY(hipEventRecord(ctx->ev_stop, ctx->stream));
    svt_ctx_stage_commit(ctx);
    ctx->timed = 1;
    return SVT_HIP_OK;
}
}

extern "C" int32_t svt_hip_inter_pred_batch_device(svt_hip_ctx *ctx, int32_t n_pics, const svt_mc_picture *pics) {
    if (!ctx || n_pics < 1 || !pics) return svt_set_error(SVT_HIP_ERR_BAD_PARAMETER, "mc: null argument");
    HIP_TRY(hipSetDevice(ctx->device));
    return mc_launch(ctx, n_pics, pics);
}

extern "C" int32_t svt_hip_inter_pred_frame(svt_hip_ctx *ctx, const svt_mc_mode_info *mi, int32_t mi_stride, int32_t mi_rows, int32_t mi_cols,
                                            const svt_mc_host_ref ref[2], int32_t use_subpel, uint8_t *pred_y, uint8_t *pred_u, uint8_t *pred_v) {
    if (!ctx || !mi || !ref || !pred_y || !pred_u || !pred_v || mi_rows < 1 || mi_cols < 1 || mi_stride < mi_cols)
        return svt_set_error(SVT_HIP_ERR_BAD_PARAMETER, "mc: null argument");
    HIP_TRY(hipSetDevice(ctx->device));
    const int      W = mi_cols * 8, H = mi_rows * 8;
    svt_mc_picture p;
    memset(&p, 0, sizeof p);
    const size_t mi_bytes = sizeof(svt_mc_mode_info) * (size_t)mi_rows * mi_stride;
    void        *dmi      = svt_ctx_slot(ctx, 26, mi_bytes);
    if (!dmi) return svt_set_error(SVT_HIP_ERR_NO_RESOURCES, "mc: device buffers");
    HIP_TRY(hipMemcpyAsync(dmi, mi, mi_bytes, hipMemcpyHostToDevice, ctx->stream));
    p.d_mi = (const svt_mc_mode_info *)dmi; p.mi_stride = mi_stride; p.mi_rows = mi_rows; p.mi_cols = mi_cols; p.use_subpel = use_subpel;
    for (int l = 0; l < 2; l++) {
        const svt_mc_host_ref &r = ref[l];
        if (!r.y || !r.u || !r.v || r.org_x < 80 || r.org_y < 80 || (r.org_x & 1) || (r.org_y & 1))
            return svt_set_error(SVT_HIP_ERR_BAD_PARAMETER, "mc: reference planes need an even padding of at least 80 luma samples");
        const size_t ny = (size_t)r.y_stride * (H + 2 * r.org_y), nuv = (size_t)r.uv_stride * (H / 2 + r.org_y);
        uint8_t *dy = (uint8_t *)svt_ctx_slot(ctx, 27 + 3 * l, ny + 64);
        uint8_t *du = (uint8_t *)svt_ctx_slot(ctx, 28 + 3 * l, nuv + 64), *dv = (uint8_t *)svt_ctx_slot(ctx, 29 + 3 * l, nuv + 64);
        if (!dy || !du || !dv) return svt_set_error(SVT_HIP_ERR_NO_RESOURCES, "mc: device buffers");
        HIP_TRY(hipMemcpyAsync(dy, r.y, ny, hipMemcpyHostToDevice, ctx->stream));
        HIP_TRY(hipMemcpyAsync(du, r.u, nuv, hipMemcpyHostToDevice, ctx->stream));
        HIP_TRY(hipMemcpyAsync(dv, r.v, nuv, hipMemcpyHostToDevice, ctx->stream));
        p.ref[l].y = dy + (size_t)r.org_y * r.y_stride + r.org_x;
        p.ref[l].u = du + (size_t)(r.org_y / 2) * r.uv_stride + r.org_x / 2;
        p.ref[l].v = dv + (size_t)(r.org_y / 2) * r.uv_stride + r.org_x / 2;
        p.ref[l].y_stride = r.y_stride; p.ref[l].uv_stride = r.uv_stride; p.ref[l].width = W; p.ref[l].height = H;
    }
    const size_t ysz = (size_t)W * H, csz = ysz / 4;
    uint8_t     *dp  = (uint8_t *)svt_ctx_slot(ctx, 33, ysz + 2 * csz);
    if (!dp) return svt_set_error(SVT_HIP_ERR_NO_RESOURCES, "mc: device buffers");
    HIP_TRY(hipMemcpyAsync(dp, pred_y, ysz, hipMemcpyHostToDevice, ctx->stream));
    HIP_TRY(hipMemcpyAsync(dp + ysz, pred_u, csz, hipMemcpyHostToDevice, ctx->stream));
    HIP_TRY(hipMemcpyAsync(dp + ysz + csz, pred_v, csz, hipMemcpyHostToDevice, ctx->stream));
    p.pred.y = dp; p.pred.u = dp + ysz; p.pred.v = dp + ysz + csz; p.pred.y_stride = W; p.pred.uv_stride = W / 2; p.pred.width = W; p.pred.height = H;
    int32_t rc = mc_launch(ctx, 1, &p);
    if (rc) return rc;
    HIP_TRY(hipMemcpyAsync(pred_y, dp, ysz, hipMemcpyDeviceToHost, ctx->stream));
    HIP_TRY(hipMemcpyAsync(pred_u, dp + ysz, csz, hipMemcpyDeviceToHost, ctx->stream));
    HIP_TRY(hipMemcpyAsync(pred_v, dp + ysz + csz, csz, hipMemcpyDeviceToHost, ctx->stream));
    HIP_TRY(hipStreamSynchronize(ctx->stream));
    return SVT_HIP_OK;
}
```

### svt-vp9_amd/csrc/refpad_kernel.hip

```cpp
#include <hip/hip_runtime.h>
#include "svt_ctx.h"

#define RP_GLOBAL __attribute__((address_space(1)))
#define RP_AS_GLOBAL(T, p) ((T RP_GLOBAL *)(uintptr_t)(p))

namespace {
struct rp_job {
    uint8_t *pic;
    int32_t  stride, w, h, pad_x, pad_y;
    int32_t  wg0;
};

constexpr int RP_ROWS = 8;

typedef uint32_t rp_u32x4 __attribute__((ext_vector_type(4), aligned(4)));

__global__ __launch_bounds__(256) void svt_refpad_kernel(const rp_job *__restrict__ jobs, int n_jobs) {
    int j = 0;
    while (j + 1 < n_jobs && (int)blockIdx.x >= jobs[j + 1].wg0) j++;
    const rp_job J = jobs[j];
    const int    py0 = ((int)blockIdx.x - J.wg0) * RP_ROWS - J.pad_y;
    const bool   vec = !((J.stride | J.pad_x | J.w) & 3) && !((uintptr_t)J.pic & 3);
    for (int r = 0; r < RP_ROWS; r++) {
        const int py = py0 + r;
        if (py >= J.h + J.pad_y) break;
        const int sy = py < 0 ? 0 : py > J.h - 1 ? J.h - 1 : py;
        const uint8_t RP_GLOBAL *srow = RP_AS_GLOBAL(const uint8_t, J.pic + (ptrdiff_t)sy * J.stride);
        uint8_t RP_GLOBAL       *drow = RP_AS_GLOBAL(uint8_t, J.pic + (ptrdiff_t)py * J.stride);
        const uint32_t lft = srow[0] * 0x01010101u, rgt = srow[J.w - 1] * 0x01010101u;
        if (py >= 0 && py < J.h) {
            if (vec) {
                const int nd = J.pad_x >> 2;
                for (int t = threadIdx.x; t < 2 * nd; t += 256) {
                    const bool right = t >= nd;
                    *(uint32_t RP_GLOBAL *)(drow + (right ? J.w + 4 * (t - nd) : 4 * t - J.pad_x)) = right ? rgt : lft;
                }
            } else {
                for (int t = threadIdx.x; t < 2 * J.pad_x; t += 256) {
                    const bool right = t >= J.pad_x;
                    drow[right ? J.w + (t - J.pad_x) : t - J.pad_x] = (uint8_t)(right ? rgt : lft);
                }
            }
        } else if (vec) {
            const int tw = J.w + 2 * J.pad_x, nu = (tw + 15) >> 4;
            for (int u = threadIdx.x; u < nu; u += 256) {
                const int px0 = 16 * u - J.pad_x;
                uint32_t  d[4];
                _Pragma("unroll") for (int k = 0; k < 4; k++) {
                    const int x = px0 + 4 * k;
                    d[k] = x < 0 ? lft : x >= J.w ? rgt : *(const uint32_t RP_GLOBAL *)(srow + x);
                }
                if (16 * u + 16 <= tw) {
                    rp_u32x4 o; o.x = d[0]; o.y = d[1]; o.z = d[2]; o.w = d[3];
                    *(rp_u32x4 RP_GLOBAL *)(drow + px0) = o;
                } else
                    for (int k = 0; 16 * u + 4 * k < tw; k++) *(uint32_t RP_GLOBAL *)(drow + px0 + 4 * k) = d[k];
            }
        } else {
            for (int t = threadIdx.x; t < J.w + 2 * J.pad_x; t += 256) {
                int sx = t - J.pad_x;
                sx = sx < 0 ? 0 : sx > J.w - 1 ? J.w - 1 : sx;
                drow[t - J.pad_x] = srow[sx];
            }
        }
    }
}
}

extern "C" int32_t svt_hip_ref_pad_batch_device(svt_hip_ctx *ctx, int32_t n_pics, const svt_yuv_planes *pics, int32_t pad_x, int32_t pad_y) {
    if (!ctx || n_pics < 1 || !pics) return svt_set_error(SVT_HIP_ERR_BAD_PARAMETER, "ref_pad: null argument");
    if (pad_x < 0 || pad_y < 0 || (pad_x & 1) || (pad_y & 1)) return svt_set_error(SVT_HIP_ERR_BAD_PARAMETER, "ref_pad: padding must be even and >= 0");
    if (!pad_x && !pad_y) return SVT_HIP_OK;
    HIP_TRY(hipSetDevice(ctx->device));
    const int n_jobs = 3 * n_pics;
    rp_job   *h = nullptr, *d = nullptr;
    if (svt_ctx_stage(ctx, sizeof(rp_job) * (size_t)n_jobs, (void **)&h, (void **)&d)) return svt_set_error(SVT_HIP_ERR_NO_RESOURCES, "ref_pad: scratch");
    int wgs = 0, k = 0;
    for (int i = 0; i < n_pics; i++) {
        const svt_yuv_planes &P = pics[i];
        if (!P.y || !P.u || !P.v || P.width < 2 || P.height < 2 || (P.width & 1) || (P.height & 1))
            return svt_set_error(SVT_HIP_ERR_BAD_PARAMETER, "ref_pad: picture geometry");
        if (P.y_stride < P.width + 2 * pad_x || P.uv_stride < P.width / 2 + pad_x)
            return svt_set_error(SVT_HIP_ERR_BAD_PARAMETER, "ref_pad: stride smaller than the padded row");
        uint8_t *pl[3] = {P.y, P.u, P.v};
        for (int c = 0; c < 3; c++) {
            rp_job &J = h[k++];
            const int sh = c ? 1 : 0;
            J.pic = pl[c]; J.stride = c ? P.uv_stride : P.y_stride; J.w = P.width >> sh; J.h = P.height >> sh;
            J.pad_x = pad_x >> sh; J.pad_y = pad_y >> sh; J.wg0 = wgs;
            wgs += (J.h + 2 * J.pad_y + RP_ROWS - 1) / RP_ROWS;
        }
    }
    HIP_TRY(hipMemcpyAsync(d, h, sizeof(rp_job) * (size_t)n_jobs, hipMemcpyHostToDevice, ctx->stream));
    HIP_TRY(hipEventRecord(ctx->ev_start, ctx->stream));
    hipLaunchKernelGGL(svt_refpad_kernel, dim3(wgs), dim3(256), 0, ctx->stream, (const rp_job *)d, n_jobs);
    HIP_TRY(hipGetLastError());
    HIP_TRY(hipEventRecord(ctx->ev_stop, ctx->stream));
    svt_ctx_stage_commit(ctx);
    ctx->timed = 1;
    return SVT_HIP_OK;
}
```

### svt-vp9_amd/csrc/svt_ctx.h

```cpp
#ifndef SVT_CTX_H
#define SVT_CTX_H
#include <hip/hip_runtime.h>
#include <stdint.h>
#include <string.h>
#include "../../include/svtvp9_hip.h"

#define SVT_CTX_SLOTS 40
#define SVT_CTX_RING 64
#define SVT_CTX_UPLOAD_RING 4
#define SVT_CTX_MARKERS 1024

struct svt_hip_ctx {
    int         device;
    hipStream_t stream;
    int         owns_stream;
    hipEvent_t  ev_start, ev_stop;
    int         timed;
    int         cu_count;
    int         me_instance;
    int         intra_wgs;
    void       *ring_host[SVT_CTX_RING];
    void       *ring_dev[SVT_CTX_RING];
    size_t      ring_bytes[SVT_CTX_RING];
    hipEvent_t  ring_ev[SVT_CTX_RING];
    int         ring_used[SVT_CTX_RING];
    int         ring_own[SVT_CTX_RING];
    void       *ring_slab_host, *ring_slab_dev;
    int         ring_pos;
    void       *up_host[SVT_CTX_UPLOAD_RING];
    size_t      up_bytes[SVT_CTX_UPLOAD_RING];
    hipEvent_t  up_ev[SVT_CTX_UPLOAD_RING];
    int         up_used[SVT_CTX_UPLOAD_RING];
    int         up_pos;
    double      up_prof[3];
    long        up_prof_n;
    hipEvent_t  direct_ev;
    int         direct_pending;
    hipEvent_t  mk_ev[SVT_CTX_MARKERS];
    uint64_t    mk_next;
    hipEvent_t  ho_produced, ho_consumed;
    void       *slot[SVT_CTX_SLOTS];
    size_t      slot_bytes[SVT_CTX_SLOTS];
};

int32_t svt_set_error(int32_t code, const char *msg);
int32_t svt_set_hip_error(hipError_t e, const char *file, int line);
int     svt_ctx_stage(svt_hip_ctx *ctx, size_t bytes, void **host, void **dev);
void    svt_ctx_stage_commit(svt_hip_ctx *ctx);
void   *svt_ctx_slot(svt_hip_ctx *ctx, int slot, size_t bytes);

int32_t svt_tq_launch_device_lists(svt_hip_ctx *ctx, const uint8_t *d_src, const uint8_t *d_pred, uint8_t *const *recon_set, int n_set,
                                   const svt_tq_block *d_blocks, const int32_t cap[4], const int32_t *d_off_cnt, const svt_quant_tables *d_qtabs,
                                   const int16_t *d_iscan, int16_t *d_qcoeff, int16_t *d_dqcoeff, uint16_t *d_eob, uint64_t *d_dist,
                                   const uint32_t *d_pos, const void *d_geom, int geom_stride, const uint32_t *d_iscan_off, int sb_cols);

int32_t svt_intra_launch(svt_hip_ctx *ctx, const svt_encdec_picture *p, int32_t width, int32_t height, int32_t mi_stride, const svt_quant_tables *d_qtabs,
                         const int16_t *d_iscan, const uint32_t iscan_off[16], int32_t *d_sync, int32_t *d_status, int32_t mixed);
int32_t svt_md_intra_default_launch(svt_hip_ctx *ctx, svt_lf_mode_info *d_lf_mi, int32_t mi_stride, int32_t mi_rows, int32_t mi_cols, int32_t filter_level);

#define HIP_TRY(expr)                                                        \
    do {                                                                     \
        hipError_t e_ = (expr);                                              \
        if (e_ != hipSuccess) return svt_set_hip_error(e_, __FILE__, __LINE__); \
    } while (0)
#endif
```

### svt-vp9_amd/csrc/tq_core.h

```cpp
#ifndef SVT_TQ_CORE_H
#define SVT_TQ_CORE_H
#include <hip/hip_runtime.h>
#include "svt_ctx.h"
#include "txfm1d.h"
#include "encdec_core.h"
#include "rate_core.h"

namespace {

struct tq_rate_args {
    const svt_rate_tables *T;
    const int16_t         *scan;
    int32_t               *bits;
};

struct tq_dev_count {
    const int32_t *p; int s;
    const uint32_t *pos; const uint8_t *geom; int geom_stride; const uint32_t *iscan_off; int sb_cols;
};

struct tq_walk { int per_xcd, first, step, base; };
__device__ __forceinline__ tq_walk tq_walk_of(int ngroups) {
    tq_walk w;
    w.per_xcd = (ngroups + 7) >> 3;
    w.base    = (int)(blockIdx.x & 7) * w.per_xcd;
    w.first   = (int)(blockIdx.x >> 3);
    w.step    = (int)(gridDim.x >> 3);
    return w;
}

#define TQ_DPP(v, ctrl) __builtin_amdgcn_update_dpp(0, (int)(v), (ctrl), 0xf, 0xf, false)
template <int N> __device__ __forceinline__ int tq_lanes_max(int v) {
    int o;
    o = TQ_DPP(v, 0xB1); v = o > v ? o : v;
    o = TQ_DPP(v, 0x4E); v = o > v ? o : v;
    if constexpr (N >= 8) { o = TQ_DPP(v, 0x141); v = o > v ? o : v; }
    if constexpr (N >= 16) { o = TQ_DPP(v, 0x140); v = o > v ? o : v; }
    if constexpr (N >= 32) { o = __builtin_amdgcn_ds_swizzle(v, 0x401F); v = o > v ? o : v; }
    return v;
}
template <int N> __device__ __forceinline__ uint32_t tq_lanes_sum(uint32_t v) {
    v += (uint32_t)TQ_DPP(v, 0xB1);
    v += (uint32_t)TQ_DPP(v, 0x4E);
    if constexpr (N >= 8) v += (uint32_t)TQ_DPP(v, 0x141);
    if constexpr (N >= 16) v += (uint32_t)TQ_DPP(v, 0x140);
    if constexpr (N >= 32) v += (uint32_t)__builtin_amdgcn_ds_swizzle((int)v, 0x401F);
    return v;
}

template <int N, bool RATE> constexpr int tq_threads() { return 256; }

template <int N> struct txcfg;
template <> struct txcfg<4> { static constexpr int size = SVT_TX_4X4, shift = 4; };
template <> struct txcfg<8> { static constexpr int size = SVT_TX_8X8, shift = 5; };
template <> struct txcfg<16> { static constexpr int size = SVT_TX_16X16, shift = 6; };
template <> struct txcfg<32> { static constexpr int size = SVT_TX_32X32, shift = 6; };

template <int N> __device__ __forceinline__ void fwd1d_hybrid(const int32_t *v, int32_t *o, bool adst) {
    if constexpr (N == 4) {
        if (adst) tx_fadst4(v, o);
        else { tx_fdct4(v, o); _Pragma("unroll") for (int i = 0; i < 4; i++) o[i] = (int16_t)o[i]; }
    } else if constexpr (N == 8) {
        if (adst) tx_adst8(v, o);
        else { tx_fdct8(v, o, 1); _Pragma("unroll") for (int i = 0; i < 8; i++) o[i] = (int16_t)o[i]; }
    } else {
        int32_t oa[16], od[16];
        if (adst) tx_adst16(v, oa);
        else { tx_fdct16(v, od); _Pragma("unroll") for (int i = 0; i < 16; i++) od[i] = (int16_t)od[i]; }
        _Pragma("unroll") for (int i = 0; i < 16; i++) o[i] = adst ? oa[i] : od[i];
    }
}
template <int N> __device__ __forceinline__ void fwd1d_dct(const int32_t *v, int32_t *o) {
    if constexpr (N == 4) tx_fdct4(v, o);
    else if constexpr (N == 8) tx_fdct8(v, o, 0);
    else if constexpr (N == 16) tx_fdct16(v, o);
    else tx_fdct32(v, o);
}
template <int N> __device__ __forceinline__ void inv1d(const int32_t *v, int32_t *o, bool adst) {
    if constexpr (N == 4) { if (adst) tx_iadst4(v, o); else tx_idct4(v, o); }
    else if constexpr (N == 8) { if (adst) tx_adst8(v, o); else tx_idct8(v, o); }
    else if constexpr (N == 16) {
        int32_t oa[16], od[16];
        if (adst) tx_adst16(v, oa); else tx_idct16(v, od);
        _Pragma("unroll") for (int i = 0; i < 16; i++) o[i] = adst ? oa[i] : od[i];
    }
    else tx_idct32(v, o);
}

template <int N> __device__ __forceinline__ void row_load(const uint8_t *p, bool vec, uint32_t *w) {
    if constexpr (N == 4) { w[0] = *(const uint32_t *)p; }
    else if constexpr (N == 8) {
        if (vec) { const uint2 t = *(const uint2 *)p; w[0] = t.x; w[1] = t.y; }
        else { w[0] = ((const uint32_t *)p)[0]; w[1] = ((const uint32_t *)p)[1]; }
    } else {
        if (vec) { _Pragma("unroll") for (int j = 0; j < N / 16; j++) { const uint4 t = ((const uint4 *)p)[j]; w[4 * j] = t.x; w[4 * j + 1] = t.y; w[4 * j + 2] = t.z; w[4 * j + 3] = t.w; } }
        else { _Pragma("unroll") for (int j = 0; j < N / 4; j++) w[j] = ((const uint32_t *)p)[j]; }
    }
}
template <int N> __device__ __forceinline__ void row_store(uint8_t *p, bool vec, const uint32_t *w) {
    if constexpr (N == 4) { *(uint32_t *)p = w[0]; }
    else if constexpr (N == 8) {
        if (vec) *(uint2 *)p = make_uint2(w[0], w[1]);
// ... 201 lines not shown
```

### svt-vp9_amd/csrc/tq_kernel.hip

```cpp
#include <hip/hip_runtime.h>
#include "tq_core.h"

namespace {

template <int N, bool RATE, bool DIST>
__global__ __launch_bounds__(256) __attribute__((amdgpu_waves_per_eu(N == 32 ? (RATE ? 3 : 4) : 1))) void svt_tq_kernel(const uint8_t *__restrict__ src, const uint8_t *__restrict__ pred,
                                                     uint8_t *__restrict__ recon, const svt_tq_block *__restrict__ blocks,
                                                     int n_blocks, const svt_quant_tables *__restrict__ qtabs,
                                                     const int16_t *__restrict__ iscan_all, int16_t *__restrict__ qcoeff,
                                                     int16_t *__restrict__ dqcoeff, uint16_t *__restrict__ eob_out,
                                                     uint64_t *__restrict__ dist_out, tq_rate_args ra, const uint8_t *const *__restrict__ recon_set, tq_dev_count dc) {
    if (dc.p) {
        const int o = dc.p[dc.s];
        n_blocks = dc.p[4 + dc.s];
        blocks += o; eob_out += o;
        if (dc.pos) dc.pos += o;
        if (dist_out) dist_out += 2 * o;
        if constexpr (RATE) ra.bits += o;
    }
    constexpr int NT  = tq_threads<N, RATE>();
    constexpr int BPW = NT / N;
    constexpr int LS  = N + 1;
    __shared__ int32_t tile[BPW][N * LS];
    __shared__ uint32_t s_tc[RATE ? 4 * RATE_SLICE : 1];
    constexpr int SCAN_T = 3 * N * N + 2, SCAN_N = N == 32 ? 3 * N * N : 4 * SCAN_T;
    __shared__ int16_t s_scan[RATE ? SCAN_N : 2];
    if constexpr (RATE) {
        const uint32_t *g = &ra.T->token_costs[txcfg<N>::size][0][0][0][0][0][0];
        for (int j = threadIdx.x; j < 4 * RATE_SLICE; j += NT) s_tc[j] = g[j];
        const uint32_t *gs = (const uint32_t *)(ra.scan + rate_scan_offset(txcfg<N>::size, 0));
        for (int j = threadIdx.x; j < SCAN_N / 2; j += NT) ((uint32_t *)s_scan)[j] = gs[j];
        __syncthreads();
    }
    const int lb  = threadIdx.x / N;
    const int i   = threadIdx.x % N;
    const tq_walk wk = tq_walk_of((n_blocks + BPW - 1) / BPW);
  for (int gj = wk.first; gj < wk.per_xcd; gj += wk.step) {
    const int grp = wk.base + gj;
    if (grp * BPW >= n_blocks) break;
    const int blk = grp * BPW + lb;
    const bool active = blk < n_blocks;
    svt_tq_block k;
    if (dc.pos) {
        const uint32_t pc = dc.pos[active ? blk : 0];
        svt_tq_block_from_pos(pc, txcfg<N>::size, (const svt_tq_pic_geom *)(dc.geom + (size_t)svt_tq_pos_pic(pc) * dc.geom_stride), dc.iscan_off, dc.sb_cols, &k);
    } else if (active) k = blocks[blk];
    else { k = blocks[0]; }
    int32_t *t = tile[lb];
    uint32_t srow[N / 4], prow[N / 4];
    {
        const uint8_t *sp = src + k.src_off + (size_t)i * k.src_stride;
        const uint8_t *pp = pred + k.pred_off + (size_t)i * k.pred_stride;
        constexpr uintptr_t AM = N >= 16 ? 15 : N - 1;
        _Pragma("unroll") for (int q = 0; q < N / 4; q++) { srow[q] = 0u; prow[q] = 0u; }
        if (active) { row_load<N>(sp, ((uintptr_t)sp & AM) == 0, srow); row_load<N>(pp, ((uintptr_t)pp & AM) == 0, prow); }
    }
    int32_t *bits_slot = nullptr;
    if constexpr (RATE) bits_slot = ra.bits + blk;
    tq_block_body<N, RATE, DIST>(k, active, i, t, srow, prow, qtabs, iscan_all, qcoeff, dqcoeff, eob_out + blk, dist_out ? dist_out + 2 * blk : nullptr, bits_slot,
                                 ra.T, s_tc, s_scan, recon_set ? (uint8_t *)recon_set[(k.pad_[0] >> 4) & 7] : recon);
    tq_block_sync();
  }
}


struct scan4_tab { uint8_t scan[16], nb[32]; };
constexpr scan4_tab SCAN4[3] = {
    {{0, 4, 1, 5, 8, 2, 12, 9, 3, 6, 13, 10, 7, 14, 11, 15},
     {0, 0, 0, 0, 0, 0, 1, 4, 4, 4, 1, 1, 8, 8, 5, 8, 2, 2, 2, 5, 9, 12, 6, 9, 3, 6, 10, 13, 7, 10, 11, 14}},
    {{0, 1, 4, 2, 5, 3, 6, 8, 9, 7, 12, 10, 13, 11, 14, 15},
     {0, 0, 0, 0, 0, 0, 1, 1, 4, 4, 2, 2, 5, 5, 4, 4, 8, 8, 6, 6, 8, 8, 9, 9, 12, 12, 10, 10, 13, 13, 14, 14}},
    {{0, 4, 8, 1, 12, 5, 9, 2, 13, 6, 10, 3, 7, 14, 11, 15},
     {0, 0, 0, 0, 4, 4, 0, 0, 8, 8, 1, 1, 5, 5, 1, 1, 9, 9, 2, 2, 6, 6, 2, 2, 3, 3, 10, 10, 7, 7, 11, 11}}};
constexpr uint8_t BAND4[16] = {0, 1, 1, 2, 2, 2, 3, 3, 3, 3, 4, 4, 4, 5, 5, 5};
__host__ __device__ constexpr int scan4_kind(int tx_type) { return tx_type == SVT_ADST_DCT ? 1 : tx_type == SVT_DCT_ADST ? 2 : 0; }

template <int K>
__device__ __forceinline__ int rate_walk4(const int (&tok)[16], const int (&en)[16], const uint32_t *tc, int eob, int ctx0) {
    int sum = (int)tc[ctx0 * 12 + (eob == 0 ? 11 : tok[0])];
    _Pragma("unroll") for (int c = 1; c < 16; c++) {
        if (!__any(c <= eob)) break;
        const int  pt = (1 + en[SCAN4[K].nb[2 * c]] + en[SCAN4[K].nb[2 * c + 1]]) >> 1;
        const bool in = c < eob;
        const int  pz = in && tok[SCAN4[K].scan[c - 1]] == 0, tk = in ? tok[SCAN4[K].scan[c]] : 11;
        const int  v  = (int)tc[((BAND4[c] * 2 + pz) * 6 + pt) * 12 + tk];
        sum += c <= eob ? v : 0;
    }
    return sum;
}

template <int N, bool RATE, bool DIST>
__device__ __forceinline__ void tq_lane_block(const svt_tq_block &k, const int blk, const uint8_t *__restrict__ src, const uint8_t *__restrict__ pred, uint8_t *__restrict__ recon,
                                              const svt_quant_tables *__restrict__ qtabs, const int16_t *__restrict__ iscan_all, int16_t *__restrict__ qcoeff,
                                              int16_t *__restrict__ dqcoeff, uint16_t *__restrict__ eob_out, uint64_t *__restrict__ dist_out, const tq_rate_args &ra,
                                              const uint32_t *s_tc, const int32_t *s_vc, const uint8_t *const *__restrict__ recon_set) {
    constexpr int ND = N / 4;
    const bool col_adst = k.tx_type == SVT_ADST_DCT || k.tx_type == SVT_ADST_ADST;
    const bool row_adst = k.tx_type == SVT_DCT_ADST || k.tx_type == SVT_ADST_ADST;
    const bool dct_dct  = k.tx_type == SVT_DCT_DCT;
    uint32_t   prow[N][ND];
    int32_t    m[N][N];
    {
        uint32_t srow[N][ND];
        _Pragma("unroll") for (int r = 0; r < N; r++) {
            const uint8_t *sp = src + k.src_off + (size_t)r * k.src_stride, *pp = pred + k.pred_off + (size_t)r * k.pred_stride;
            if constexpr (N == 4) { srow[r][0] = *(const uint32_t *)sp; prow[r][0] = *(const uint32_t *)pp; }
            else {
                row_load<N>(sp, ((uintptr_t)sp & 7) == 0, srow[r]);
                row_load<N>(pp, ((uintptr_t)pp & 7) == 0, prow[r]);
            }
        }
        _Pragma("unroll") for (int cc = 0; cc < N; cc++) {
            int32_t v[N], o[N];
            _Pragma("unroll") for (int r = 0; r < N; r++)
                v[r] = ((int)((srow[r][cc >> 2] >> (8 * (cc & 3))) & 0xff) - (int)((prow[r][cc >> 2] >> (8 * (cc & 3))) & 0xff)) * (N == 4 ? 16 : 4);
            if constexpr (N == 4) {
                if (cc == 0 && v[0]) ++v[0];
                if (col_adst) tx_fadst4(v, o); else tx_fdct4(v, o);
            } else {
                if (col_adst) tx_adst8(v, o);
                else if (dct_dct) tx_fdct8(v, o, 0);
                else tx_fdct8(v, o, 1);
            }
            _Pragma("unroll") for (int kk = 0; kk < N; kk++) m[kk][cc] = (int16_t)o[kk];
        }
    }
    svt_quant_tables q;
    {
        const uint32_t *qp = (const uint32_t *)(qtabs + k.qtab);
        uint32_t        qw5[5];
        _Pragma("unroll") for (int j = 0; j < 5; j++) qw5[j] = qp[j];
        q.zbin[0] = (int16_t)qw5[0]; q.zbin[1] = (int16_t)(qw5[0] >> 16); q.round[0] = (int16_t)qw5[1]; q.round[1] = (int16_t)(qw5[1] >> 16);
        q.quant[0] = (int16_t)qw5[2]; q.quant[1] = (int16_t)(qw5[2] >> 16); q.quant_shift[0] = (int16_t)qw5[3]; q.quant_shift[1] = (int16_t)(qw5[3] >> 16);
        q.dequant[0] = (int16_t)qw5[4]; q.dequant[1] = (int16_t)(qw5[4] >> 16);
    }
    int32_t  dq[N][N];
    uint32_t rdist = 0, pdist = 0;
    int      eob = 0;
    int      tok[RATE ? 16 : 1], en[RATE ? 16 : 1], vsum = 0, nnz = 0;
    const uint32_t *ip = (const uint32_t *)(iscan_all + k.iscan_off);
    _Pragma("unroll") for (int i = 0; i < N; i++) {
        int32_t  o[N];
        uint32_t isw[N / 2], qw[N / 2], dqw[N / 2];
// ... 25 lines not shown
                pdist += (uint32_t)(cv * cv);
            }
            if (kk & 1) { qw[kk >> 1] |= (uint32_t)(uint16_t)qv << 16; dqw[kk >> 1] |= (uint32_t)(uint16_t)dv << 16; }
            else { qw[kk >> 1] = (uint16_t)qv; dqw[kk >> 1] = (uint16_t)dv; }
            if (level) { const int pos = (int)((isw[kk >> 1] >> (16 * (kk & 1))) & 0xffff) + 1; eob = pos > eob ? pos : eob; }
            if constexpr (RATE) {
                tok[i * N + kk] = 0; en[i * N + kk] = 0;
                if (__any(level != 0)) {
                    const int al = qv < 0 ? -qv : qv;
                    tok[i * N + kk] = token_of(qv);
                    en[i * N + kk]  = energy_of_value(qv);
                    nnz += qv != 0;
                    int vc = s_vc[66 + (al < 67 ? qv : 0)];
                    if (__any(al >= 67)) {
                        const int extra = al >= 67 ? al - 67 : 0;
                        const int c6 = ra.T->cat6_low_cost[extra & 0xff] + ra.T->cat6_high_cost[extra >> 8];
                        vc = al >= 67 ? c6 : vc;
                    }
                    vsum += qv != 0 ? vc : 0;
                }
            }
        }
        int16_t *qo = qcoeff + k.coeff_off + i * N, *dqo = dqcoeff + k.coeff_off + i * N;
        if constexpr (N == 4) { *(uint2 *)qo = make_uint2(qw[0], qw[1]); if (dqcoeff) *(uint2 *)dqo = make_uint2(dqw[0], dqw[1]); }
        else { *(uint4 *)qo = make_uint4(qw[0], qw[1], qw[2], qw[3]); if (dqcoeff) *(uint4 *)dqo = make_uint4(dqw[0], dqw[1], dqw[2], dqw[3]); }
    }
    eob_out[blk] = (uint16_t)eob;
    if constexpr (DIST) if (dist_out) { dist_out[2 * blk] = rdist; dist_out[2 * blk + 1] = pdist; }
    if constexpr (RATE) {
        const int       rinfo = k.pad_[0], ptype = (rinfo >> 2) & 1, inter = (rinfo >> 3) & 1, ctx0 = rinfo & 3;
        const uint32_t *tc = s_tc + (ptype * 2 + inter) * RATE_SLICE;
        const int       kind = scan4_kind(k.tx_type);
        int             bits = 0;
        if (kind == 0) bits = rate_walk4<0>(tok, en, tc, eob, ctx0);
        if (kind == 1) bits = rate_walk4<1>(tok, en, tc, eob, ctx0);
        if (kind == 2) bits = rate_walk4<2>(tok, en, tc, eob, ctx0);
        ra.bits[blk] = bits + vsum + (eob - nnz) * s_vc[66];
    }
    if (!k.do_recon) return;
    constexpr int SH = txcfg<N>::shift;
    uint32_t      rw[N][ND];
    _Pragma("unroll") for (int r = 0; r < N; r++) { _Pragma("unroll") for (int j = 0; j < ND; j++) rw[r][j] = 0; }
    const bool dc_only = dct_dct && (N == 4 ? eob <= 1 : eob == 1);
    if (eob != 0 && !dc_only) {
        int32_t t[N][N];
        _Pragma("unroll") for (int i = 0; i < N; i++) {
            int32_t o[N];
            if constexpr (N == 4) { if (row_adst) tx_iadst4(dq[i], o); else tx_idct4(dq[i], o); }
            else { if (row_adst) tx_adst8(dq[i], o); else tx_idct8(dq[i], o); }
            _Pragma("unroll") for (int kk = 0; kk < N; kk++) t[i][kk] = (int16_t)o[kk];
        }
        _Pragma("unroll") for (int cc = 0; cc < N; cc++) {
            int32_t v[N], o[N];
            _Pragma("unroll") for (int r = 0; r < N; r++) v[r] = t[r][cc];
            if constexpr (N == 4) { if (col_adst) tx_iadst4(v, o); else tx_idct4(v, o); }
            else { if (col_adst) tx_adst8(v, o); else tx_idct8(v, o); }
            _Pragma("unroll") for (int r = 0; r < N; r++) {
                const int res = ((int16_t)o[r] + (1 << (SH - 1))) >> SH;
                rw[r][cc >> 2] |= (uint32_t)clip_add((int)((prow[r][cc >> 2] >> (8 * (cc & 3))) & 0xff), res) << (8 * (cc & 3));
            }
        }
    } else {
        int32_t a1 = 0;
        if (eob != 0) {
            int32_t d = tx_rsw((int16_t)dq[0][0] * TX_C16);
            d = tx_rsw(d * TX_C16);
            a1 = (d + (1 << (SH - 1))) >> SH;
        }
        _Pragma("unroll") for (int r = 0; r < N; r++) {
            _Pragma("unroll") for (int cc = 0; cc < N; cc++)
                rw[r][cc >> 2] |= (uint32_t)clip_add((int)((prow[r][cc >> 2] >> (8 * (cc & 3))) & 0xff), a1) << (8 * (cc & 3));
        }
    }
    uint8_t *const rbase = recon_set ? (uint8_t *)recon_set[(k.pad_[0] >> 4) & 7] : recon;
    if (!rbase) return;
    _Pragma("unroll") for (int r = 0; r < N; r++) {
        uint8_t *d = rbase + k.recon_off + (size_t)r * k.recon_stride;
        if constexpr (N == 4) *(uint32_t *)d = rw[r][0];
        else row_store<N>(d, ((uintptr_t)d & 7) == 0, rw[r]);
    }
}

template <int N, bool RATE, bool DIST>
__global__ __launch_bounds__(256) void svt_tq_lane_kernel(const uint8_t *__restrict__ src, const uint8_t *__restrict__ pred,
                                                          uint8_t *__restrict__ recon, const svt_tq_block *__restrict__ blocks,
                                                          int n_blocks, const svt_quant_tables *__restrict__ qtabs,
                                                          const int16_t *__restrict__ iscan_all, int16_t *__restrict__ qcoeff,
                                                          int16_t *__restrict__ dqcoeff, uint16_t *__restrict__ eob_out,
                                                          uint64_t *__restrict__ dist_out, tq_rate_args ra, const uint8_t *const *__restrict__ recon_set, tq_dev_count dc) {
    if (dc.p) {
        const int o = dc.p[dc.s];
        n_blocks = dc.p[4 + dc.s];
        blocks += o; eob_out += o;
        if (dc.pos) dc.pos += o;
        if (dist_out) dist_out += 2 * o;
        if constexpr (RATE) ra.bits += o;
    }
    static_assert(N == 4 || N == 8, "block-per-lane form: 4x4 and 8x8 only");
    static_assert(!RATE || N == 4, "in-lane rate: 4x4 only");
    __shared__ uint32_t s_tc[RATE ? 4 * RATE_SLICE : 1];
    __shared__ int32_t  s_vc[RATE ? 136 : 1];
    if constexpr (RATE) {
        const uint32_t *g = &ra.T->token_costs[0][0][0][0][0][0][0];
        for (int j = threadIdx.x; j < 4 * RATE_SLICE; j += 256) s_tc[j] = g[j];
        if (threadIdx.x < 133) s_vc[threadIdx.x] = ra.T->value_cost[threadIdx.x];
        __syncthreads();
    }
    const tq_walk wk = tq_walk_of((n_blocks + 255) / 256);
  for (int gj = wk.first; gj < wk.per_xcd; gj += wk.step) {
    const int blk = (wk.base + gj) * 256 + (int)threadIdx.x;
    if (blk >= n_blocks) continue;
    svt_tq_block k;
    if (dc.pos) {
        const uint32_t pc = dc.pos[blk];
        svt_tq_block_from_pos(pc, txcfg<N>::size, (const svt_tq_pic_geom *)(dc.geom + (size_t)svt_tq_pos_pic(pc) * dc.geom_stride), dc.iscan_off, dc.sb_cols, &k);
    } else k = blocks[blk];
    tq_lane_block<N, RATE, DIST>(k, blk, src, pred, recon, qtabs, iscan_all, qcoeff, dqcoeff, eob_out, dist_out, ra, s_tc, s_vc, recon_set);
  }
}

int tq_grid(svt_hip_ctx *ctx, int ngroups, int per_cu) {
    const int per_xcd = (ngroups + 7) / 8, cap = (ctx->cu_count * per_cu + 7) / 8;
    return 8 * (per_xcd < cap ? per_xcd : cap);
}

template <int N, bool RATE, bool DIST = true>
hipError_t launch_tq(svt_hip_ctx *ctx, const uint8_t *src, const uint8_t *pred, uint8_t *recon, const svt_tq_block *blocks, int n,
                     const svt_quant_tables *q, const int16_t *iscan, int16_t *qc, int16_t *dqc, uint16_t *eob, uint64_t *dist, tq_rate_args ra,
                     const uint8_t *const *recon_set, tq_dev_count dc = {nullptr, 0, nullptr, nullptr, 0, nullptr, 0}) {
    if (n <= 0) return hipSuccess;
    if constexpr (N == 4) {
        hipLaunchKernelGGL((svt_tq_lane_kernel<N, RATE, DIST>), dim3(tq_grid(ctx, (n + 255) / 256, 6)), dim3(256), 0, ctx->stream, src, pred, recon, blocks, n, q,
                           iscan, qc, dqc, eob, dist, ra, recon_set, dc);
        return hipGetLastError();
    } else {
        constexpr int NT = tq_threads<N, RATE>(), BPW = NT / N;
        hipLaunchKernelGGL((svt_tq_kernel<N, RATE, DIST>), dim3(tq_grid(ctx, (n + BPW - 1) / BPW, 6)), dim3(NT), 0, ctx->stream, src, pred, recon, blocks, n, q,
                           iscan, qc, dqc, eob, dist, ra, recon_set, dc);
        return hipGetLastError();
    }
}

template <bool RATE>
int32_t tq_launch_all(svt_hip_ctx *ctx, const uint8_t *d_src, const uint8_t *d_pred, uint8_t *d_recon, const svt_tq_block *d_blocks,
                      const int32_t size_count[4], const svt_quant_tables *d_qtabs, const int16_t *d_iscan, int16_t *d_qcoeff,
                      int16_t *d_dqcoeff, uint16_t *d_eob, uint64_t *d_dist, tq_rate_args ra, uint8_t *const *recon_set = nullptr, int n_set = 0) {
    HIP_TRY(hipSetDevice(ctx->device));
    const uint8_t *const *d_set = nullptr;
    if (recon_set) {
        void *h = nullptr, *d = nullptr;
        if (svt_ctx_stage(ctx, 8 * sizeof(void *), &h, &d)) return svt_set_error(SVT_HIP_ERR_NO_RESOURCES, "tq: descriptor buffers");
        for (int i = 0; i < 8; i++) ((uint8_t **)h)[i] = i < n_set ? recon_set[i] : nullptr;
        HIP_TRY(hipMemcpyAsync(d, h, 8 * sizeof(void *), hipMemcpyHostToDevice, ctx->stream));
        d_set = (const uint8_t *const *)d;
    }
    HIP_TRY(hipEventRecord(ctx->ev_start, ctx->stream));
    int        off = 0;
    hipError_t rc = hipSuccess;
    auto at = [&](int o) { tq_rate_args r = ra; if (r.bits) r.bits += o; return r; };
    rc = launch_tq<4, RATE>(ctx, d_src, d_pred, d_recon, d_blocks + off, size_count[0], d_qtabs, d_iscan, d_qcoeff, d_dqcoeff, d_eob + off, d_dist ? d_dist + 2 * off : nullptr, at(off), d_set);
    off += size_count[0];
    if (rc == hipSuccess) rc = launch_tq<8, RATE>(ctx, d_src, d_pred, d_recon, d_blocks + off, size_count[1], d_qtabs, d_iscan, d_qcoeff, d_dqcoeff, d_eob + off, d_dist ? d_dist + 2 * off : nullptr, at(off), d_set);
    off += size_count[1];
    if (rc == hipSuccess) rc = launch_tq<16, RATE>(ctx, d_src, d_pred, d_recon, d_blocks + off, size_count[2], d_qtabs, d_iscan, d_qcoeff, d_dqcoeff, d_eob + off, d_dist ? d_dist + 2 * off : nullptr, at(off), d_set);
    off += size_count[2];
    if (rc == hipSuccess) rc = launch_tq<32, RATE>(ctx, d_src, d_pred, d_recon, d_blocks + off, size_count[3], d_qtabs, d_iscan, d_qcoeff, d_dqcoeff, d_eob + off, d_dist ? d_dist + 2 * off : nullptr, at(off), d_set);
    (void)hipEventRecord(ctx->ev_stop, ctx->stream);
    if (recon_set) svt_ctx_stage_commit(ctx);
    if (rc != hipSuccess) return svt_set_hip_error(rc, __FILE__, __LINE__);
    ctx->timed = 1;
    return SVT_HIP_OK;
}
}

int32_t svt_tq_launch_device_lists(svt_hip_ctx *ctx, const uint8_t *d_src, const uint8_t *d_pred, uint8_t *const *recon_set, int n_set,
                                   const svt_tq_block *d_blocks, const int32_t cap[4], const int32_t *d_off_cnt, const svt_quant_tables *d_qtabs,
                                   const int16_t *d_iscan, int16_t *d_qcoeff, int16_t *d_dqcoeff, uint16_t *d_eob, uint64_t *d_dist,
                                   const uint32_t *d_pos, const void *d_geom, int geom_stride, const uint32_t *d_iscan_off, int sb_cols) {
    HIP_TRY(hipSetDevice(ctx->device));
    void *h = nullptr, *d = nullptr;
    if (svt_ctx_stage(ctx, 8 * sizeof(void *), &h, &d)) return svt_set_error(SVT_HIP_ERR_NO_RESOURCES, "tq: descriptor buffers");
    for (int i = 0; i < 8; i++) ((uint8_t **)h)[i] = i < n_set ? recon_set[i] : nullptr;
    HIP_TRY(hipMemcpyAsync(d, h, 8 * sizeof(void *), hipMemcpyHostToDevice, ctx->stream));
    const uint8_t *const *d_set = (const uint8_t *const *)d;
    const tq_rate_args none = {nullptr, nullptr, nullptr};
    hipError_t rc = hipSuccess;
#define TQ_DEV(N, S, D) launch_tq<N, false, D>(ctx, d_src, d_pred, nullptr, d_blocks, cap[S], d_qtabs, d_iscan, d_qcoeff, d_dqcoeff, d_eob, d_dist, none, d_set, tq_dev_count{d_off_cnt, S, d_pos, (const uint8_t *)d_geom, geom_stride, d_iscan_off, sb_cols})
    if (d_dist) {
        rc = TQ_DEV(4, 0, true);
        if (rc == hipSuccess) rc = TQ_DEV(8, 1, true);
        if (rc == hipSuccess) rc = TQ_DEV(16, 2, true);
        if (rc == hipSuccess) rc = TQ_DEV(32, 3, true);
    } else {
        rc = TQ_DEV(4, 0, false);
        if (rc == hipSuccess) rc = TQ_DEV(8, 1, false);
        if (rc == hipSuccess) rc = TQ_DEV(16, 2, false);
        if (rc == hipSuccess) rc = TQ_DEV(32, 3, false);
    }
#undef TQ_DEV
    svt_ctx_stage_commit(ctx);
    if (rc != hipSuccess) return svt_set_hip_error(rc, __FILE__, __LINE__);
    return SVT_HIP_OK;
}

extern "C" int32_t svt_hip_tq_batch_device(svt_hip_ctx *ctx, const uint8_t *d_src, const uint8_t *d_pred, uint8_t *d_recon,
                                           const svt_tq_block *d_blocks, const int32_t size_count[4],
                                           const svt_quant_tables *d_qtabs, const int16_t *d_iscan, int16_t *d_qcoeff,
                                           int16_t *d_dqcoeff, uint16_t *d_eob) {
    return svt_hip_tq_batch_dist_device(ctx, d_src, d_pred, d_recon, d_blocks, size_count, d_qtabs, d_iscan, d_qcoeff, d_dqcoeff, d_eob,
                                        nullptr);
}

extern "C" int32_t svt_hip_tq_batch_dist_device(svt_hip_ctx *ctx, const uint8_t *d_src, const uint8_t *d_pred, uint8_t *d_recon,
                                                const svt_tq_block *d_blocks, const int32_t size_count[4],
                                                const svt_quant_tables *d_qtabs, const int16_t *d_iscan, int16_t *d_qcoeff,
                                                int16_t *d_dqcoeff, uint16_t *d_eob, uint64_t *d_dist) {
    if (!ctx || !d_src || !d_pred || !d_blocks || !size_count || !d_qtabs || !d_iscan || !d_qcoeff || !d_dqcoeff || !d_eob)
        return svt_set_error(SVT_HIP_ERR_BAD_PARAMETER, "tq: null argument");
    if (((uintptr_t)d_qcoeff | (uintptr_t)d_dqcoeff) & 15) return svt_set_error(SVT_HIP_ERR_BAD_PARAMETER, "tq: coefficient arrays must be 16-byte aligned");
    tq_rate_args none = {nullptr, nullptr, nullptr};
    return tq_launch_all<false>(ctx, d_src, d_pred, d_recon, d_blocks, size_count, d_qtabs, d_iscan, d_qcoeff, d_dqcoeff, d_eob, d_dist, none);
}

extern "C" int32_t svt_hip_tq_rd_batch_device(svt_hip_ctx *ctx, const uint8_t *d_src, const uint8_t *d_pred, uint8_t *d_recon,
                                              const svt_tq_block *d_blocks, const int32_t size_count[4],
                                              const svt_quant_tables *d_qtabs, const int16_t *d_iscan, int16_t *d_qcoeff,
                                              int16_t *d_dqcoeff, uint16_t *d_eob, uint64_t *d_dist,
                                              const svt_rate_tables *d_tables, const int16_t *d_scan, int32_t *d_bits) {
    if (!ctx || !d_src || !d_pred || !d_blocks || !size_count || !d_qtabs || !d_iscan || !d_qcoeff || !d_dqcoeff || !d_eob || !d_tables ||
        !d_scan || !d_bits)
        return svt_set_error(SVT_HIP_ERR_BAD_PARAMETER, "tq_rd: null argument");
    if (((uintptr_t)d_qcoeff | (uintptr_t)d_dqcoeff) & 15) return svt_set_error(SVT_HIP_ERR_BAD_PARAMETER, "tq_rd: coefficient arrays must be 16-byte aligned");
    if ((uintptr_t)d_scan & 3) return svt_set_error(SVT_HIP_ERR_BAD_PARAMETER, "tq_rd: scan array must be 4-byte aligned");
    tq_rate_args ra = {d_tables, d_scan, d_bits};
    return tq_launch_all<true>(ctx, d_src, d_pred, d_recon, d_blocks, size_count, d_qtabs, d_iscan, d_qcoeff, d_dqcoeff, d_eob, d_dist, ra);
}

extern "C" int32_t svt_hip_tq_rd_batch_multi_device(svt_hip_ctx *ctx, const uint8_t *d_src, const uint8_t *d_pred, uint8_t *const *recon_set, int32_t n_set,
                                                    const svt_tq_block *d_blocks, const int32_t size_count[4], const svt_quant_tables *d_qtabs,
                                                    const int16_t *d_iscan, int16_t *d_qcoeff, int16_t *d_dqcoeff, uint16_t *d_eob, uint64_t *d_dist,
                                                    const svt_rate_tables *d_tables, const int16_t *d_scan, int32_t *d_bits) {
    if (!ctx || !d_src || !d_pred || !recon_set || n_set < 1 || n_set > 8 || !d_blocks || !size_count || !d_qtabs || !d_iscan || !d_qcoeff || !d_dqcoeff || !d_eob)
        return svt_set_error(SVT_HIP_ERR_BAD_PARAMETER, "tq_multi: bad argument");
    if (((uintptr_t)d_qcoeff | (uintptr_t)d_dqcoeff) & 15) return svt_set_error(SVT_HIP_ERR_BAD_PARAMETER, "tq_multi: coefficient arrays must be 16-byte aligned");
    if (d_bits) {
        if (!d_tables || !d_scan || ((uintptr_t)d_scan & 3)) return svt_set_error(SVT_HIP_ERR_BAD_PARAMETER, "tq_multi: rate tables / scan array");
        tq_rate_args ra = {d_tables, d_scan, d_bits};
        return tq_launch_all<true>(ctx, d_src, d_pred, nullptr, d_blocks, size_count, d_qtabs, d_iscan, d_qcoeff, d_dqcoeff, d_eob, d_dist, ra, recon_set, n_set);
    }
    tq_rate_args none = {nullptr, nullptr, nullptr};
    return tq_launch_all<false>(ctx, d_src, d_pred, nullptr, d_blocks, size_count, d_qtabs, d_iscan, d_qcoeff, d_dqcoeff, d_eob, d_dist, none, recon_set, n_set);
}

extern "C" int32_t svt_hip_rate_scan4x4_table(int32_t tx_type, int16_t out[48]) {
    if (tx_type < 0 || tx_type > 3 || !out) return svt_set_error(SVT_HIP_ERR_BAD_PARAMETER, "scan4x4: bad argument");
    const scan4_tab &t = SCAN4[scan4_kind(tx_type)];
    for (int i = 0; i < 16; i++) out[i] = t.scan[i];
    for (int i = 0; i < 32; i++) out[16 + i] = t.nb[i];
    return SVT_HIP_OK;
}

extern "C" int32_t svt_hip_tq_batch(svt_hip_ctx *ctx, const uint8_t *src, const uint8_t *pred, uint8_t *recon, size_t plane_bytes,
                                    const svt_tq_block *blocks, int32_t n_blocks, const svt_quant_tables *qtabs, int32_t n_qtabs,
                                    const int16_t *iscan, size_t iscan_count, int16_t *qcoeff, int16_t *dqcoeff,
                                    size_t coeff_count, uint16_t *eob) {
    if (!ctx || !src || !pred || !recon || !blocks || n_blocks < 1 || !qtabs || !iscan || !qcoeff || !dqcoeff || !eob)
        return svt_set_error(SVT_HIP_ERR_BAD_PARAMETER, "tq: null argument");
    int32_t cnt[4] = {0, 0, 0, 0};
    for (int i = 0; i < n_blocks; i++) {
        if (blocks[i].tx_size > 3 || blocks[i].qtab >= n_qtabs) return svt_set_error(SVT_HIP_ERR_BAD_PARAMETER, "tq: bad block");
        if (blocks[i].coeff_off & 7) return svt_set_error(SVT_HIP_ERR_BAD_PARAMETER, "tq: coeff_off must be a multiple of 8 coefficients");
        if (i && blocks[i].tx_size < blocks[i - 1].tx_size) return svt_set_error(SVT_HIP_ERR_BAD_PARAMETER, "tq: blocks not grouped by tx_size");
        if (i && blocks[i].tx_size == blocks[i - 1].tx_size && (blocks[i].do_recon != 0) != (blocks[i - 1].do_recon != 0))
            return svt_set_error(SVT_HIP_ERR_BAD_PARAMETER, "tq: do_recon must be uniform within a tx_size group");
        cnt[blocks[i].tx_size]++;
    }
    HIP_TRY(hipSetDevice(ctx->device));
    uint8_t *ds = (uint8_t *)svt_ctx_slot(ctx, 11, plane_bytes + 64), *dp = (uint8_t *)svt_ctx_slot(ctx, 12, plane_bytes + 64);
    uint8_t *dr = (uint8_t *)svt_ctx_slot(ctx, 13, plane_bytes + 64);
    svt_tq_block *db = (svt_tq_block *)svt_ctx_slot(ctx, 14, sizeof(svt_tq_block) * (size_t)n_blocks);
    svt_quant_tables *dqt = (svt_quant_tables *)svt_ctx_slot(ctx, 15, sizeof(svt_quant_tables) * (size_t)n_qtabs);
    int16_t *dis = (int16_t *)svt_ctx_slot(ctx, 16, sizeof(int16_t) * iscan_count);
    int16_t *dq = (int16_t *)svt_ctx_slot(ctx, 17, sizeof(int16_t) * coeff_count), *ddq = (int16_t *)svt_ctx_slot(ctx, 18, sizeof(int16_t) * coeff_count);
// ... 20 lines not shown
```

Measured before the change: 6259.

## Fuse encdec bookkeeping kernels and batch descriptor uploads into one staged buffer

Removes several small kernels and uploads from the encdec hot path. The per-picture scan is folded into the emit kernel via wave reductions, and the eob-map clear moves into the count kernel. The skip-map scatter moves into the transform/quant kernels' epilogue, and skip-flag update can run inside the loop-filter mask kernel. Quant tables, recon set pointers and MC/LF/refpad descriptors are packed into a single staged host-to-device upload. It also adds a waves-per-EU hint to the lane kernel. The aim is lower launch and copy overhead, at the cost of extra work and register pressure inside the TQ kernels.

```diff
diff --git a/svt-vp9_amd/csrc/encdec.hip b/svt-vp9_amd/csrc/encdec.hip
--- a/svt-vp9_amd/csrc/encdec.hip
+++ b/svt-vp9_amd/csrc/encdec.hip
@@ -15,11 +15,10 @@
     uint32_t     *d_pos;
     uint16_t     *d_eob;
     int32_t      *d_counts;
-    int32_t      *d_totals, *d_bases;
+    int32_t      *d_totals;
     int32_t      *d_off_cnt;
     int32_t      *d_status;
     int32_t      *d_intra_sync;
-    svt_quant_tables *d_qtabs;
     int16_t      *d_iscan;
     svt_encdec_stage_hook hook;
     void         *hook_user;
@@ -30,11 +29,8 @@
 struct ed_pic_dev {
     const svt_me_pu_result *res;
     svt_mc_mode_info       *mc_mi;
-    svt_lf_mode_info       *lf_mi;
-    uint8_t                *nz;
-    uint16_t               *eob_map;
     svt_lf_mask            *lfm;
-    svt_tq_pic_geom         g;
+    svt_tq_pic_rec          r;
 };
 struct ed_batch_dev {
     ed_pic_dev pic[ED_MAX_PICS];
@@ -43,6 +39,11 @@
     uint32_t   lambda;
     int32_t    filter_level;
 };
+struct ed_stage_head {
+    ed_batch_dev     b;
+    svt_quant_tables qt[2];
+    const uint8_t   *recon_set[ED_MAX_SETS];
+};
 
 __device__ __forceinline__ int wave_sum(int v) {
     _Pragma("unroll") for (int d = 32; d >= 1; d >>= 1) v += __shfl_xor(v, d, 64);
@@ -57,15 +58,27 @@
     return incl - v;
 }
 
-__global__ __launch_bounds__(64) void svt_tq_count_kernel(const ed_batch_dev *__restrict__ B, int32_t *__restrict__ counts, int32_t *__restrict__ status) {
+__global__ __launch_bounds__(64) void svt_tq_count_kernel(const ed_batch_dev *__restrict__ B, int32_t *__restrict__ counts, int32_t *__restrict__ status, int clear_map) {
     const int sb = (int)blockIdx.x % B->n_sb, pic = (int)blockIdx.x / B->n_sb, lane = (int)threadIdx.x;
     const ed_pic_dev &P = B->pic[pic];
     const int ur = (sb / B->sb_cols) * 8 + (lane >> 3), uc = (sb % B->sb_cols) * 8 + (lane & 7);
     int cnt[4] = {0, 0, 0, 0};
-    if (ur < B->mi_rows && uc < B->mi_cols) P.nz[ur * B->mi_stride + uc] = 0;
-    const int o = svt_tq_unit_is_origin(P.lf_mi, B->mi_stride, B->mi_rows, B->mi_cols, ur, uc);
+    if (ur < B->mi_rows && uc < B->mi_cols) P.r.nz[ur * B->mi_stride + uc] = 0;
+    if (clear_map) {
+        const int w4 = B->width >> 2, h4 = B->height >> 2, cw4 = w4 >> 1, ch4 = h4 >> 1;
+        uint32_t *my = (uint32_t *)P.r.eob_map;
+        _Pragma("unroll") for (int j = 0; j < 2; j++) {
+            const int d = lane + 64 * j, y4 = (sb / B->sb_cols) * 16 + (d >> 3), x4 = (sb % B->sb_cols) * 16 + (d & 7) * 2;
+            if (y4 < h4 && x4 < w4) my[(y4 * w4 + x4) >> 1] = 0;
+        }
+        if (ur < ch4 && uc < cw4) {
+            uint16_t *mc = P.r.eob_map + w4 * h4 + ur * cw4 + uc;
+            mc[0] = 0; mc[cw4 * ch4] = 0;
+        }
+    }
+    const int o = svt_tq_unit_is_origin(P.r.lf_mi, B->mi_stride, B->mi_rows, B->mi_cols, ur, uc);
     if (o < 0) atomicOr(status, 1);
-    if (o == 1) svt_tq_unit_counts(P.lf_mi, B->mi_stride, ur, uc, cnt);
+    if (o == 1) svt_tq_unit_counts(P.r.lf_mi, B->mi_stride, ur, uc, cnt);
     _Pragma("unroll") for (int s = 0; s < 4; s++) {
         const int v = wave_sum(cnt[s]);
         if (lane == 0) counts[(s * B->n_pics + pic) * B->n_sb + sb] = v;
@@ -90,16 +103,6 @@
     for (int i = b; i < e; i++) { const int v = p[i]; p[i] = run; run += v; }
     if (t == 255) totals[blockIdx.x] = part[255];
 }
-__global__ __launch_bounds__(64) void svt_scan_pic_kernel(const int32_t *__restrict__ totals, int n_pics, int32_t *__restrict__ bases, int32_t *__restrict__ off_cnt) {
-    if (threadIdx.x != 0) return;
-    int run = 0;
-    for (int s = 0; s < 4; s++) {
-        off_cnt[s] = run;
-        for (int p = 0; p < n_pics; p++) { bases[s * n_pics + p] = run; run += totals[s * n_pics + p]; }
-        off_cnt[4 + s] = run - off_cnt[s];
-    }
-}
-
 __global__ __launch_bounds__(256) void svt_tq_expand_kernel(const ed_batch_dev *__restrict__ B, const int32_t *__restrict__ off_cnt, const uint32_t *__restrict__ pos,
                                                            svt_tq_block *__restrict__ blocks) {
     const int i = (int)blockIdx.x * 256 + (int)threadIdx.x, total = off_cnt[3] + off_cnt[7];
@@ -107,68 +110,64 @@
     const int      ts = i >= off_cnt[3] ? 3 : i >= off_cnt[2] ? 2 : i >= off_cnt[1] ? 1 : 0;
     const uint32_t p = pos[i];
     svt_tq_block   k;
-    svt_tq_block_from_pos(p, ts, &B->pic[svt_tq_pos_pic(p)].g, B->iscan_off, B->sb_cols, &k);
+    svt_tq_block_from_pos(p, ts, &B->pic[svt_tq_pos_pic(p)].r.g, B->iscan_off, B->sb_cols, &k);
     blocks[i] = k;
 }
 
-__global__ __launch_bounds__(64) void svt_tq_emit_kernel(const ed_batch_dev *__restrict__ B, const int32_t *__restrict__ offsets, const int32_t *__restrict__ bases,
-                                                         svt_tq_block *__restrict__ blocks, uint32_t *__restrict__ pos) {
+__global__ __launch_bounds__(64) void svt_tq_emit_kernel(const ed_batch_dev *__restrict__ B, const int32_t *__restrict__ offsets, const int32_t *__restrict__ totals,
+                                                         int32_t *__restrict__ off_cnt, svt_tq_block *__restrict__ blocks, uint32_t *__restrict__ pos) {
     const int sb = (int)blockIdx.x % B->n_sb, pic = (int)blockIdx.x / B->n_sb, lane = (int)threadIdx.x;
     const ed_pic_dev &P = B->pic[pic];
     const int ur = (sb / B->sb_cols) * 8 + (lane >> 3), uc = (sb % B->sb_cols) * 8 + (lane & 7);
     int cnt[4] = {0, 0, 0, 0};
-    const int o = svt_tq_unit_is_origin(P.lf_mi, B->mi_stride, B->mi_rows, B->mi_cols, ur, uc);
-    if (o == 1) svt_tq_unit_counts(P.lf_mi, B->mi_stride, ur, uc, cnt);
+    const int o = svt_tq_unit_is_origin(P.r.lf_mi, B->mi_stride, B->mi_rows, B->mi_cols, ur, uc);
+    if (o == 1) svt_tq_unit_counts(P.r.lf_mi, B->mi_stride, ur, uc, cnt);
+    const int n_tot = 4 * B->n_pics;
+    const int t0 = lane < n_tot ? totals[lane] : 0, t1 = 64 + lane < n_tot ? totals[64 + lane] : 0;
     uint32_t base[4];
-    _Pragma("unroll") for (int s = 0; s < 4; s++) base[s] = (uint32_t)(bases[s * B->n_pics + pic] + offsets[(s * B->n_pics + pic) * B->n_sb + sb] + wave_excl_prefix(cnt[s], lane));
-    if (o == 1) svt_tq_unit_emit(P.lf_mi, B->mi_stride, ur, uc, &P.g, B->iscan_off, base, blocks, pos);
-}
-
-__global__ __launch_bounds__(256) void svt_tq_skip_kernel(const ed_batch_dev *__restrict__ B, const int32_t *__restrict__ off_cnt, const uint32_t *__restrict__ pos,
-                                                          const uint16_t *__restrict__ eob) {
-    const int total = off_cnt[3] + off_cnt[7];
-    const int w4 = B->width >> 2, h4 = B->height >> 2;
-    for (int i = (int)(blockIdx.x * blockDim.x + threadIdx.x); i < total; i += (int)(gridDim.x * blockDim.x)) {
-        const uint32_t p = pos[i];
-        const int      pic = (int)(p >> 24) & 63, plane = (int)(p >> 22) & 3, y4 = (int)(p >> 11) & 0x7ff, x4 = (int)p & 0x7ff;
-        const ed_pic_dev &P = B->pic[pic];
-        const int      e = eob[i];
-        const int      pw4 = plane ? w4 >> 1 : w4;
-        const int      off = plane == 0 ? 0 : w4 * h4 + (plane == 2 ? (w4 >> 1) * (h4 >> 1) : 0);
-        P.eob_map[off + y4 * pw4 + x4] = (uint16_t)e;
-        if (e) {
-            const int uy = plane ? y4 : y4 >> 1, ux = plane ? x4 : x4 >> 1;
-            const svt_lf_mode_info b = P.lf_mi[uy * B->mi_stride + ux];
-            const int w8 = svt_blk_w8(b.sb_type), h8 = svt_blk_h8(b.sb_type);
-            P.nz[(uy - uy % h8) * B->mi_stride + (ux - ux % w8)] = 1;
-        }
-    }
-}
-__global__ __launch_bounds__(256) void svt_eob_map_clear_kernel(const ed_batch_dev *__restrict__ B, int n16) {
-    uint4 *m = (uint4 *)B->pic[blockIdx.y].eob_map;
-    for (int i = (int)(blockIdx.x * 256 + threadIdx.x); i < n16; i += (int)(gridDim.x * 256)) m[i] = make_uint4(0, 0, 0, 0);
+    _Pragma("unroll") for (int s = 0; s < 4; s++) {
+        const int first = s * B->n_pics + pic;
+        const int bs = wave_sum((lane < first ? t0 : 0) + (64 + lane < first ? t1 : 0));
+        base[s] = (uint32_t)(bs + offsets[(s * B->n_pics + pic) * B->n_sb + sb] + wave_excl_prefix(cnt[s], lane));
+    }
+    if (blockIdx.x == 0) {
+        _Pragma("unroll") for (int s = 0; s < 4; s++) {
+            const int lo = s * B->n_pics, hi = lo + B->n_pics;
+            const int before = wave_sum((lane < lo ? t0 : 0) + (64 + lane < lo ? t1 : 0));
+            const int mine = wave_sum((lane >= lo && lane < hi ? t0 : 0) + (64 + lane >= lo && 64 + lane < hi ? t1 : 0));
+            if (lane == 0) { off_cnt[s] = before; off_cnt[4 + s] = mine; }
+        }
+    }
+    if (o == 1) svt_tq_unit_emit(P.r.lf_mi, B->mi_stride, ur, uc, &P.r.g, B->iscan_off, base, blocks, pos);
+}
+
+__device__ __forceinline__ void skip_update_unit(const ed_batch_dev *B, const ed_pic_dev &P, int ur, int uc) {
+    svt_lf_mode_info *b = &P.r.lf_mi[ur * B->mi_stride + uc];
+    if (b->sb_type > 12) return;
+    const int w8 = svt_blk_w8(b->sb_type), h8 = svt_blk_h8(b->sb_type);
+    b->skip = P.r.nz[(ur - ur % h8) * B->mi_stride + (uc - uc % w8)] ? 0 : 1;
 }
 __global__ __launch_bounds__(256) void svt_skip_update_kernel(const ed_batch_dev *__restrict__ B) {
     const int units = B->mi_rows * B->mi_cols;
     const int i = (int)(blockIdx.x * blockDim.x + threadIdx.x);
     if (i >= units * B->n_pics) return;
-    const int pic = i / units, u = i % units, ur = u / B->mi_cols, uc = u % B->mi_cols;
-    const ed_pic_dev &P = B->pic[pic];
-    svt_lf_mode_info *b = &P.lf_mi[ur * B->mi_stride + uc];
-    if (b->sb_type > 12) return;
-    const int w8 = svt_blk_w8(b->sb_type), h8 = svt_blk_h8(b->sb_type);
-    b->skip = P.nz[(ur - ur % h8) * B->mi_stride + (uc - uc % w8)] ? 0 : 1;
+    const int pic = i / units, u = i % units;
+    skip_update_unit(B, B->pic[pic], u / B->mi_cols, u % B->mi_cols);
 }
 
 __device__ __forceinline__ uint32_t wave_or(uint32_t v) {
     _Pragma("unroll") for (int d = 32; d >= 1; d >>= 1) v |= (uint32_t)__shfl_xor((int)v, d, 64);
     return v;
 }
-__global__ __launch_bounds__(64) void svt_lf_mask_kernel(const ed_batch_dev *__restrict__ B, int32_t *__restrict__ status) {
+__global__ __launch_bounds__(64) void svt_lf_mask_kernel(const ed_batch_dev *__restrict__ B, int32_t *__restrict__ status, int set_skip) {
     const int sb = (int)blockIdx.x % B->n_sb, pic = (int)blockIdx.x / B->n_sb, lane = (int)threadIdx.x;
     const ed_pic_dev &P = B->pic[pic];
+    if (set_skip) {
+        const int ur = (sb / B->sb_cols) * 8 + (lane >> 3), uc = (sb % B->sb_cols) * 8 + (lane & 7);
+        if (ur < B->mi_rows && uc < B->mi_cols) skip_update_unit(B, P, ur, uc);
+    }
     svt_lf_unit_masks u;
-    svt_lf_mask_unit(P.lf_mi, B->mi_stride, B->mi_rows, B->mi_cols, sb / B->sb_cols, sb % B->sb_cols, lane >> 3, lane & 7, &u);
+    svt_lf_mask_unit(P.r.lf_mi, B->mi_stride, B->mi_rows, B->mi_cols, sb / B->sb_cols, sb % B->sb_cols, lane >> 3, lane & 7, &u);
     if (u.bad && status) atomicOr(status, 1);
     __shared__ uint32_t sm[40];
     uint64_t            w64[9];
@@ -194,7 +193,7 @@
     const int r = lane >> 3, c = lane & 7, sr = sb / B->sb_cols, sc = sb % B->sb_cols, ur = sr * 8 + r, uc = sc * 8 + c;
     if (ur >= B->mi_rows || uc >= B->mi_cols) return;
     svt_md_default_unit(P.res + (size_t)sb * SVT_ME_PU_COUNT, r, c, sr, sc, B->mi_rows, B->mi_cols, B->lambda, B->filter_level, &P.mc_mi[ur * B->mi_stride + uc],
-                        &P.lf_mi[ur * B->mi_stride + uc]);
+                        &P.r.lf_mi[ur * B->mi_stride + uc]);
 }
 
 int stage_batch(svt_hip_ctx *ctx, const ed_batch_dev &hb, const ed_batch_dev **d_out) {
@@ -233,14 +232,13 @@
     const int16_t  *isc = svt_hip_vp9_iscan_tables(&offs, &entries);
     bool ok = hipMalloc((void **)&w->d_pos, cap * sizeof(uint32_t)) == hipSuccess &&
               hipMalloc((void **)&w->d_eob, cap * sizeof(uint16_t)) == hipSuccess &&
-              hipMalloc((void **)&w->d_counts, (n_cnt + 9 + 8 * ED_MAX_PICS + 2 + 48 * (size_t)w->n_sb) * sizeof(int32_t)) == hipSuccess &&
-              hipMalloc((void **)&w->d_qtabs, 2 * sizeof(svt_quant_tables)) == hipSuccess && hipMalloc((void **)&w->d_iscan, (size_t)entries * sizeof(int16_t)) == hipSuccess;
+              hipMalloc((void **)&w->d_counts, (n_cnt + 9 + 4 * ED_MAX_PICS + 2 + 48 * (size_t)w->n_sb) * sizeof(int32_t)) == hipSuccess &&
+              hipMalloc((void **)&w->d_iscan, (size_t)entries * sizeof(int16_t)) == hipSuccess;
     if (ok) {
         w->d_off_cnt = w->d_counts + n_cnt;
         w->d_status = w->d_off_cnt + 8;
         w->d_totals = w->d_status + 1;
-        w->d_bases = w->d_totals + 4 * ED_MAX_PICS;
-        w->d_intra_sync = w->d_bases + 4 * ED_MAX_PICS;
+        w->d_intra_sync = w->d_totals + 4 * ED_MAX_PICS;
         ok = hipMemsetAsync(w->d_off_cnt, 0, 9 * sizeof(int32_t), ctx->stream) == hipSuccess &&
              hipMemcpyAsync(w->d_iscan, isc, (size_t)entries * sizeof(int16_t), hipMemcpyHostToDevice, ctx->stream) == hipSuccess &&
              hipStreamSynchronize(ctx->stream) == hipSuccess;
@@ -256,8 +254,8 @@
 extern "C" void svt_hip_encdec_work_destroy(svt_hip_ctx *ctx, svt_encdec_work *w) {
     if (!w) return;
     if (ctx) { (void)hipSetDevice(ctx->device); (void)hipStreamSynchronize(ctx->stream); }
-    void *v[6] = {w->d_blocks, w->d_pos, w->d_eob, w->d_counts, w->d_qtabs, w->d_iscan};
-    for (int i = 0; i < 6; i++) if (v[i]) (void)hipFree(v[i]);
+    void *v[5] = {w->d_blocks, w->d_pos, w->d_eob, w->d_counts, w->d_iscan};
+    for (int i = 0; i < 5; i++) if (v[i]) (void)hipFree(v[i]);
     free(w->last_hb);
     free(w);
 }
@@ -335,7 +333,7 @@
     for (int i = 0; i < n_pics; i++) {
         const svt_encdec_picture &p = pics[i];
         ed_pic_dev &P = hb.pic[i];
-        P.mc_mi = (svt_mc_mode_info *)p.d_mc_mi; P.lf_mi = p.d_lf_mi; P.nz = p.d_nz; P.eob_map = p.d_eob_map; P.lfm = p.d_lfm;
+        P.mc_mi = (svt_mc_mode_info *)p.d_mc_mi; P.r.lf_mi = p.d_lf_mi; P.r.nz = p.d_nz; P.r.eob_map = p.d_eob_map; P.lfm = p.d_lfm;
         const uintptr_t q_off = ((uintptr_t)p.d_qcoeff - q_lo) / sizeof(int16_t), dq_off = ((uintptr_t)p.d_dqcoeff - dq_lo) / sizeof(int16_t);
         if ((p.d_dqcoeff && q_off != dq_off) || q_off + (uint64_t)hb.n_sb * SVT_SB_COEFFS >= (1ull << 32))
             return svt_set_error(SVT_HIP_ERR_BAD_PARAMETER, "encdec: qcoeff / dqcoeff of the batch must be laid out alike, within 2^32 elements");
@@ -346,7 +344,8 @@
         for (int k = n_sets - 1; k >= 0 && set < 0; k--)
             if (r_lo >= (uintptr_t)recon_set[k] && (uint64_t)(r_hi - (uintptr_t)recon_set[k]) + plane_span < (1ull << 32)) set = k;
         if (set < 0) return svt_set_error(SVT_HIP_ERR_BAD_PARAMETER, "encdec: the batch's reconstruction buffers span more than 8 regions of 4 GB");
-        svt_tq_pic_geom &g = P.g;
+        svt_tq_pic_geom &g = P.r.g;
+        P.r.mi_stride = mi_stride;
         const uint8_t *s3[3] = {p.src.y, p.src.u, p.src.v}, *p3[3] = {p.pred.y, p.pred.u, p.pred.v};
         for (int k = 0; k < 3; k++) {
             g.src_off[k] = (uint32_t)((uintptr_t)s3[k] - src_lo); g.pred_off[k] = (uint32_t)((uintptr_t)p3[k] - pred_lo);
@@ -363,74 +362,92 @@
         if (!p.no_pad) rec_pad[n_rec_pad++] = rec[i];
         lfm[i] = p.d_lfm; lfm_stride[i] = hb.sb_cols; mi_rows_a[i] = hb.mi_rows; mi_cols_a[i] = hb.mi_cols;
     }
-    const ed_batch_dev *dB = nullptr;
-    if (stage_batch(ctx, hb, &dB)) return svt_set_error(SVT_HIP_ERR_NO_RESOURCES, "encdec: descriptor buffers");
-    {
-        svt_quant_tables qt[2];
-        if (svt_hip_quant_tables_for_qindex(q_index, qt) != SVT_HIP_OK) return svt_set_error(SVT_HIP_ERR_BAD_PARAMETER, "encdec: q index");
-        void *h = nullptr, *d = nullptr;
-        if (svt_ctx_stage(ctx, sizeof qt, &h, &d)) return svt_set_error(SVT_HIP_ERR_NO_RESOURCES, "encdec: descriptor buffers");
-        memcpy(h, qt, sizeof qt);
-        HIP_TRY(hipMemcpyAsync(w->d_qtabs, h, sizeof qt, hipMemcpyHostToDevice, ctx->stream));
-        svt_ctx_stage_commit(ctx);
-    }
+    const bool do_lf = flags->apply_loop_filter != 0;
+    if (flags->pad_reference && n_rec_pad && (pad_x < 0 || pad_y < 0 || (pad_x & 1) || (pad_y & 1)))
+        return svt_set_error(SVT_HIP_ERR_BAD_PARAMETER, "ref_pad: padding must be even and >= 0");
+    const bool   do_pad = flags->pad_reference && n_rec_pad && (pad_x || pad_y);
+    const size_t o_mc = (sizeof(ed_stage_head) + 15) & ~(size_t)15, o_rp = o_mc + svt_mc_desc_bytes(n_pics), o_lf = o_rp + (do_pad ? svt_rp_desc_bytes(n_rec_pad) : 0);
+    const size_t stage_bytes = o_lf + (do_lf ? svt_lf_desc_bytes(n_pics, mi_rows_a) : 0);
+    uint8_t     *sh = nullptr, *sd = nullptr;
+    if (svt_ctx_stage(ctx, stage_bytes, (void **)&sh, (void **)&sd)) return svt_set_error(SVT_HIP_ERR_NO_RESOURCES, "encdec: descriptor buffers");
+    ed_stage_head       *hh = (ed_stage_head *)sh;
+    const ed_stage_head *dh = (const ed_stage_head *)sd;
+    const ed_batch_dev  *dB = &dh->b;
+    hh->b = hb;
+    if (svt_hip_quant_tables_for_qindex(q_index, hh->qt) != SVT_HIP_OK) return svt_set_error(SVT_HIP_ERR_BAD_PARAMETER, "encdec: q index");
+    for (int i = 0; i < ED_MAX_SETS; i++) hh->recon_set[i] = i < n_sets ? recon_set[i] : nullptr;
+    svt_mc_plan mc_plan;
+    svt_rp_plan rp_plan;
+    svt_lf_plan lf_plan;
+    int32_t     rc = svt_mc_fill(n_pics, mcp, sh + o_mc, sd + o_mc, &mc_plan);
+    if (rc) return rc;
+    size_t upload = o_rp;
+    if (do_pad) {
+        rc = svt_rp_fill(n_rec_pad, rec_pad, pad_x, pad_y, sh + o_rp, sd + o_rp, &rp_plan);
+        if (rc) return rc;
+        upload = o_lf;
+    }
+    if (do_lf) {
+        rc = svt_lf_fill(ctx, n_pics, rec, lfm, lfm_stride, thr, mi_rows_a, mi_cols_a, 0, sh + o_lf, sd + o_lf, &lf_plan);
+        if (rc) return rc;
+        upload = o_lf + lf_plan.upload_bytes;
+    }
+    for (int i = 0; i < n_pics; i++)
+        if (pics[i].has_intra && !flags->do_recon) return svt_set_error(SVT_HIP_ERR_BAD_PARAMETER, "encdec: intra blocks need the reconstruction (do_recon)");
+    HIP_TRY(hipMemcpyAsync(sd, sh, upload, hipMemcpyHostToDevice, ctx->stream));
+    HIP_TRY(hipEventRecord(ctx->ev_start, ctx->stream));
 #define ED_STAGE(k) do { if (w->hook) w->hook(w->hook_user, (k)); } while (0)
+#define ED_LEAVE(code) do { const int32_t rc_ = (code); (void)hipEventRecord(ctx->ev_stop, ctx->stream); svt_ctx_stage_commit(ctx); ctx->timed = 1; return rc_; } while (0)
+#define ED_TRY(expr) do { const hipError_t e_ = (expr); if (e_ != hipSuccess) ED_LEAVE(svt_set_hip_error(e_, __FILE__, __LINE__)); } while (0)
     ED_STAGE(SVT_ENCDEC_STAGE_MC);
-    int32_t rc = svt_hip_inter_pred_batch_device(ctx, n_pics, mcp);
-    if (rc) return rc;
+    rc = svt_mc_enqueue(ctx, &mc_plan);
+    if (rc) ED_LEAVE(rc);
     ED_STAGE(SVT_ENCDEC_STAGE_LISTS);
     const int nwg = n_pics * hb.n_sb;
-    hipLaunchKernelGGL(svt_tq_count_kernel, dim3(nwg), dim3(64), 0, ctx->stream, dB, w->d_counts, w->d_status);
+    {
+        uintptr_t low = 0;
+        for (int i = 0; i < n_pics; i++) low |= (uintptr_t)pics[i].d_eob_map;
+        const int clear_map = !(low & 3);
+        if (!clear_map)
+            for (int i = 0; i < n_pics; i++) ED_TRY(hipMemsetAsync(pics[i].d_eob_map, 0, (size_t)(width / 4) * (height / 4) * 3 / 2 * sizeof(uint16_t), ctx->stream));
+        hipLaunchKernelGGL(svt_tq_count_kernel, dim3(nwg), dim3(64), 0, ctx->stream, dB, w->d_counts, w->d_status, clear_map);
+    }
     hipLaunchKernelGGL(svt_scan_sb_kernel, dim3(4 * n_pics), dim3(256), 0, ctx->stream, w->d_counts, hb.n_sb, w->d_totals);
-    hipLaunchKernelGGL(svt_scan_pic_kernel, dim3(1), dim3(64), 0, ctx->stream, (const int32_t *)w->d_totals, n_pics, w->d_bases, w->d_off_cnt);
-    hipLaunchKernelGGL(svt_tq_emit_kernel, dim3(nwg), dim3(64), 0, ctx->stream, dB, (const int32_t *)w->d_counts, (const int32_t *)w->d_bases, (svt_tq_block *)nullptr, w->d_pos);
-    HIP_TRY(hipGetLastError());
+    hipLaunchKernelGGL(svt_tq_emit_kernel, dim3(nwg), dim3(64), 0, ctx->stream, dB, (const int32_t *)w->d_counts, (const int32_t *)w->d_totals, w->d_off_cnt,
+                       (svt_tq_block *)nullptr, w->d_pos);
+    ED_TRY(hipGetLastError());
     if (!w->last_hb) w->last_hb = malloc(sizeof hb);
     if (w->last_hb) memcpy(w->last_hb, &hb, sizeof hb);
     ED_STAGE(SVT_ENCDEC_STAGE_TQ);
     int32_t cap[4];
     for (int s = 0; s < 4; s++) cap[s] = (int32_t)((size_t)n_pics * width * height * 3 / 2 / (size_t)(16 << (2 * s)));
-    rc = svt_tq_launch_device_lists(ctx, (const uint8_t *)src_lo, (const uint8_t *)pred_lo, recon_set, n_sets, nullptr, cap, w->d_off_cnt, w->d_qtabs, w->d_iscan,
-                                    (int16_t *)q_lo, (int16_t *)dq_lo, w->d_eob, nullptr, w->d_pos, &dB->pic[0].g, (int)sizeof(ed_pic_dev), dB->iscan_off, hb.sb_cols);
-    if (rc) return rc;
+    rc = svt_tq_launch_device_lists(ctx, (const uint8_t *)src_lo, (const uint8_t *)pred_lo, dh->recon_set, nullptr, cap, w->d_off_cnt, dh->qt, w->d_iscan,
+                                    (int16_t *)q_lo, (int16_t *)dq_lo, w->d_eob, nullptr, w->d_pos, &dB->pic[0].r.g, (int)sizeof(ed_pic_dev), dB->iscan_off, hb.sb_cols);
+    if (rc) ED_LEAVE(rc);
     ED_STAGE(SVT_ENCDEC_STAGE_SKIP);
-    {
-        const size_t map_bytes = (size_t)(width / 4) * (height / 4) * 3 / 2 * sizeof(uint16_t);
-        uintptr_t    low = map_bytes;
-        for (int i = 0; i < n_pics; i++) low |= (uintptr_t)pics[i].d_eob_map;
-        if (!(low & 15))
-            hipLaunchKernelGGL(svt_eob_map_clear_kernel, dim3(64, n_pics), dim3(256), 0, ctx->stream, dB, (int)(map_bytes / 16));
-        else
-            for (int i = 0; i < n_pics; i++) HIP_TRY(hipMemsetAsync(pics[i].d_eob_map, 0, map_bytes, ctx->stream));
-    }
     for (int i = 0; i < n_pics; i++)
         if (pics[i].has_intra) {
-            if (!flags->do_recon) return svt_set_error(SVT_HIP_ERR_BAD_PARAMETER, "encdec: intra blocks need the reconstruction (do_recon)");
-            rc = svt_intra_launch(ctx, &pics[i], width, height, mi_stride, w->d_qtabs, w->d_iscan, hb.iscan_off, w->d_intra_sync, w->d_status, 1);
-            if (rc) return rc;
-        }
-    {
-        const int total_cap = (int)(w->cap_per_pic * (size_t)n_pics);
-        int       g = (total_cap + 255) / 256;
-        if (g > ctx->cu_count * 8) g = ctx->cu_count * 8;
-        hipLaunchKernelGGL(svt_tq_skip_kernel, dim3(g), dim3(256), 0, ctx->stream, dB, (const int32_t *)w->d_off_cnt, (const uint32_t *)w->d_pos, (const uint16_t *)w->d_eob);
+            rc = svt_intra_launch(ctx, &pics[i], width, height, mi_stride, dh->qt, w->d_iscan, hb.iscan_off, w->d_intra_sync, w->d_status, 1);
+            if (rc) ED_LEAVE(rc);
+        }
+    if (!do_lf) {
         hipLaunchKernelGGL(svt_skip_update_kernel, dim3((n_pics * hb.mi_rows * hb.mi_cols + 255) / 256), dim3(256), 0, ctx->stream, dB);
-        HIP_TRY(hipGetLastError());
+        ED_TRY(hipGetLastError());
     }
     ED_STAGE(SVT_ENCDEC_STAGE_LF);
-    if (flags->apply_loop_filter) {
-        hipLaunchKernelGGL(svt_lf_mask_kernel, dim3(nwg), dim3(64), 0, ctx->stream, dB, w->d_status);
-        HIP_TRY(hipGetLastError());
-        rc = svt_hip_lf_batch_device(ctx, n_pics, rec, lfm, lfm_stride, thr, mi_rows_a, mi_cols_a, 0);
-        if (rc) return rc;
+    if (do_lf) {
+        hipLaunchKernelGGL(svt_lf_mask_kernel, dim3(nwg), dim3(64), 0, ctx->stream, dB, w->d_status, 1);
+        ED_TRY(hipGetLastError());
+        rc = svt_lf_enqueue(ctx, &lf_plan, mi_rows_a, mi_cols_a);
+        if (rc) ED_LEAVE(rc);
     }
     ED_STAGE(SVT_ENCDEC_STAGE_PAD);
-    if (flags->pad_reference && n_rec_pad) {
-        rc = svt_hip_ref_pad_batch_device(ctx, n_rec_pad, rec_pad, pad_x, pad_y);
-        if (rc) return rc;
+    if (do_pad) {
+        rc = svt_rp_enqueue(ctx, &rp_plan);
+        if (rc) ED_LEAVE(rc);
     }
     ED_STAGE(SVT_ENCDEC_STAGE_END);
-    return SVT_HIP_OK;
+    ED_LEAVE(SVT_HIP_OK);
 }
 
 extern "C" int32_t svt_hip_encdec_intra_device(svt_hip_ctx *ctx, svt_encdec_work *w, const svt_encdec_picture *pic, int32_t width, int32_t height, int32_t mi_stride,
@@ -455,45 +472,68 @@
     fill_dims(hb, 1, width, height, mi_stride);
     const uint32_t *offs = nullptr;
     (void)svt_hip_vp9_iscan_tables(&offs, nullptr);
-    hb.pic[0].lf_mi = p.d_lf_mi; hb.pic[0].nz = p.d_nz; hb.pic[0].eob_map = p.d_eob_map; hb.pic[0].lfm = p.d_lfm;
-    const ed_batch_dev *dB = nullptr;
-    if (stage_batch(ctx, hb, &dB)) return svt_set_error(SVT_HIP_ERR_NO_RESOURCES, "encdec_intra: descriptor buffers");
-    {
-        svt_quant_tables qt[2];
-        if (svt_hip_quant_tables_for_qindex(q_index, qt) != SVT_HIP_OK) return svt_set_error(SVT_HIP_ERR_BAD_PARAMETER, "encdec_intra: q index");
-        void *h = nullptr, *d = nullptr;
-        if (svt_ctx_stage(ctx, sizeof qt, &h, &d)) return svt_set_error(SVT_HIP_ERR_NO_RESOURCES, "encdec_intra: descriptor buffers");
-        memcpy(h, qt, sizeof qt);
-        HIP_TRY(hipMemcpyAsync(w->d_qtabs, h, sizeof qt, hipMemcpyHostToDevice, ctx->stream));
-        svt_ctx_stage_commit(ctx);
-    }
-    ED_STAGE(SVT_ENCDEC_STAGE_TQ);
-    HIP_TRY(hipMemsetAsync(p.d_eob_map, 0, (size_t)(width / 4) * (height / 4) * 3 / 2 * sizeof(uint16_t), ctx->stream));
-    HIP_TRY(hipMemsetAsync(p.d_nz, 0, (size_t)mi_stride * hb.mi_rows, ctx->stream));
-    int32_t rc = svt_intra_launch(ctx, pic, width, height, mi_stride, w->d_qtabs, w->d_iscan, offs, w->d_intra_sync, w->d_status, 0);
-    if (rc) return rc;
-    ED_STAGE(SVT_ENCDEC_STAGE_SKIP);
-    hipLaunchKernelGGL(svt_skip_update_kernel, dim3((hb.mi_rows * hb.mi_cols + 255) / 256), dim3(256), 0, ctx->stream, dB);
-    HIP_TRY(hipGetLastError());
-    ED_STAGE(SVT_ENCDEC_STAGE_LF);
+    hb.pic[0].r.lf_mi = p.d_lf_mi; hb.pic[0].r.nz = p.d_nz; hb.pic[0].r.eob_map = p.d_eob_map; hb.pic[0].lfm = p.d_lfm;
+    const bool do_lf = flags->apply_loop_filter != 0;
+    if (flags->pad_reference && !p.no_pad && (pad_x < 0 || pad_y < 0 || (pad_x & 1) || (pad_y & 1)))
+        return svt_set_error(SVT_HIP_ERR_BAD_PARAMETER, "ref_pad: padding must be even and >= 0");
+    const bool     do_pad = flags->pad_reference && !p.no_pad && (pad_x || pad_y);
     svt_yuv_planes rec = p.recon;
     rec.width = width; rec.height = height;
-    if (flags->apply_loop_filter) {
-        hipLaunchKernelGGL(svt_lf_mask_kernel, dim3(hb.n_sb), dim3(64), 0, ctx->stream, dB, w->d_status);
-        HIP_TRY(hipGetLastError());
-        const svt_lf_mask *lfm = p.d_lfm;
-        const int32_t      lfm_stride = hb.sb_cols, mr = hb.mi_rows, mc = hb.mi_cols;
-        rc = svt_hip_lf_batch_device(ctx, 1, &rec, &lfm, &lfm_stride, thr, &mr, &mc, 0);
+    const svt_lf_mask *lfm = p.d_lfm;
+    const int32_t      lfm_stride = hb.sb_cols, mr = hb.mi_rows, mc = hb.mi_cols;
+    const size_t o_rp = (sizeof(ed_stage_head) + 15) & ~(size_t)15, o_lf = o_rp + (do_pad ? svt_rp_desc_bytes(1) : 0);
+    const size_t stage_bytes = o_lf + (do_lf ? svt_lf_desc_bytes(1, &mr) : 0);
+    uint8_t     *sh = nullptr, *sd = nullptr;
+    if (svt_ctx_stage(ctx, stage_bytes, (void **)&sh, (void **)&sd)) return svt_set_error(SVT_HIP_ERR_NO_RESOURCES, "encdec_intra: descriptor buffers");
+    ed_stage_head       *hh = (ed_stage_head *)sh;
+    const ed_stage_head *dh = (const ed_stage_head *)sd;
+    const ed_batch_dev  *dB = &dh->b;
+    hh->b = hb;
+    if (svt_hip_quant_tables_for_qindex(q_index, hh->qt) != SVT_HIP_OK) return svt_set_error(SVT_HIP_ERR_BAD_PARAMETER, "encdec_intra: q index");
+    for (int i = 0; i < ED_MAX_SETS; i++) hh->recon_set[i] = nullptr;
+    svt_rp_plan rp_plan;
+    svt_lf_plan lf_plan;
+    int32_t     rc = SVT_HIP_OK;
+    size_t      upload = o_rp;
+    if (do_pad) {
+        rc = svt_rp_fill(1, &rec, pad_x, pad_y, sh + o_rp, sd + o_rp, &rp_plan);
         if (rc) return rc;
+        upload = o_lf;
+    }
+    if (do_lf) {
+        rc = svt_lf_fill(ctx, 1, &rec, &lfm, &lfm_stride, thr, &mr, &mc, 0, sh + o_lf, sd + o_lf, &lf_plan);
+        if (rc) return rc;
+        upload = o_lf + lf_plan.upload_bytes;
+    }
+    HIP_TRY(hipMemcpyAsync(sd, sh, upload, hipMemcpyHostToDevice, ctx->stream));
+    HIP_TRY(hipEventRecord(ctx->ev_start, ctx->stream));
+    ED_STAGE(SVT_ENCDEC_STAGE_TQ);
+    ED_TRY(hipMemsetAsync(p.d_eob_map, 0, (size_t)(width / 4) * (height / 4) * 3 / 2 * sizeof(uint16_t), ctx->stream));
+    ED_TRY(hipMemsetAsync(p.d_nz, 0, (size_t)mi_stride * hb.mi_rows, ctx->stream));
+    rc = svt_intra_launch(ctx, pic, width, height, mi_stride, dh->qt, w->d_iscan, offs, w->d_intra_sync, w->d_status, 0);
+    if (rc) ED_LEAVE(rc);
+    ED_STAGE(SVT_ENCDEC_STAGE_SKIP);
+    if (!do_lf) {
+        hipLaunchKernelGGL(svt_skip_update_kernel, dim3((hb.mi_rows * hb.mi_cols + 255) / 256), dim3(256), 0, ctx->stream, dB);
+        ED_TRY(hipGetLastError());
+    }
+    ED_STAGE(SVT_ENCDEC_STAGE_LF);
+    if (do_lf) {
+        hipLaunchKernelGGL(svt_lf_mask_kernel, dim3(hb.n_sb), dim3(64), 0, ctx->stream, dB, w->d_status, 1);
+        ED_TRY(hipGetLastError());
+        rc = svt_lf_enqueue(ctx, &lf_plan, &mr, &mc);
+        if (rc) ED_LEAVE(rc);
     }
     ED_STAGE(SVT_ENCDEC_STAGE_PAD);
-    if (flags->pad_reference && !p.no_pad) {
-        rc = svt_hip_ref_pad_batch_device(ctx, 1, &rec, pad_x, pad_y);
-        if (rc) return rc;
+    if (do_pad) {
+        rc = svt_rp_enqueue(ctx, &rp_plan);
+        if (rc) ED_LEAVE(rc);
     }
     ED_STAGE(SVT_ENCDEC_STAGE_END);
-    return SVT_HIP_OK;
-}
+    ED_LEAVE(SVT_HIP_OK);
+}
+#undef ED_TRY
+#undef ED_LEAVE
 
 extern "C" int32_t svt_hip_md_intra_default_device(svt_hip_ctx *ctx, int32_t width, int32_t height, int32_t filter_level, svt_lf_mode_info *d_lf_mi, int32_t mi_stride) {
     if (!ctx || !d_lf_mi || width < 8 || height < 8 || (width & 7) || (height & 7) || mi_stride < (width >> 3))
@@ -562,7 +602,7 @@
         hb.lambda = lambda; hb.filter_level = filter_level;
         for (int i = 0; i < n; i++) {
             if (!d_results[first + i] || !d_mc_mi[first + i] || !d_lf_mi[first + i]) return svt_set_error(SVT_HIP_ERR_BAD_PARAMETER, "md_default: null picture");
-            hb.pic[i].res = d_results[first + i]; hb.pic[i].mc_mi = d_mc_mi[first + i]; hb.pic[i].lf_mi = d_lf_mi[first + i];
+            hb.pic[i].res = d_results[first + i]; hb.pic[i].mc_mi = d_mc_mi[first + i]; hb.pic[i].r.lf_mi = d_lf_mi[first + i];
         }
         const ed_batch_dev *dB = nullptr;
         if (stage_batch(ctx, hb, &dB)) return svt_set_error(SVT_HIP_ERR_NO_RESOURCES, "md_default: descriptor buffers");
@@ -583,11 +623,11 @@
         fill_dims(hb, n, mi_cols * 8, mi_rows * 8, mi_stride);
         for (int i = 0; i < n; i++) {
             if (!d_lf_mi[first + i] || !d_lfm[first + i]) return svt_set_error(SVT_HIP_ERR_BAD_PARAMETER, "lf_masks: null picture");
-            hb.pic[i].lf_mi = (svt_lf_mode_info *)d_lf_mi[first + i]; hb.pic[i].lfm = d_lfm[first + i];
+            hb.pic[i].r.lf_mi = (svt_lf_mode_info *)d_lf_mi[first + i]; hb.pic[i].lfm = d_lfm[first + i];
         }
         const ed_batch_dev *dB = nullptr;
         if (stage_batch(ctx, hb, &dB)) return svt_set_error(SVT_HIP_ERR_NO_RESOURCES, "lf_masks: descriptor buffers");
-        hipLaunchKernelGGL(svt_lf_mask_kernel, dim3(n * hb.n_sb), dim3(64), 0, ctx->stream, dB, (int32_t *)nullptr);
+        hipLaunchKernelGGL(svt_lf_mask_kernel, dim3(n * hb.n_sb), dim3(64), 0, ctx->stream, dB, (int32_t *)nullptr, 0);
         HIP_TRY(hipGetLastError());
     }
     return SVT_HIP_OK;
diff --git a/svt-vp9_amd/csrc/lf_kernel.hip b/svt-vp9_amd/csrc/lf_kernel.hip
--- a/svt-vp9_amd/csrc/lf_kernel.hip
+++ b/svt-vp9_amd/csrc/lf_kernel.hip
@@ -301,7 +301,12 @@
     return g;
 }
 
-__global__ __launch_bounds__(128) void svt_lf_desc_kernel(const lf_pic_dev *__restrict__ pics, int rows_per_pic, int max_cols, svt_lf_thresh thr) {
+__global__ __launch_bounds__(128) void svt_lf_desc_kernel(const lf_pic_dev *__restrict__ pics, int rows_per_pic, int max_cols, svt_lf_thresh thr,
+                                                          uint32_t *__restrict__ cnt, int cnt_words) {
+    {
+        const int gi = (int)blockIdx.x * 128 + (int)threadIdx.x;
+        if (gi < cnt_words) cnt[gi] = 0;
+    }
     __shared__ uint32_t s_thr[64];
     if (threadIdx.x < 64) s_thr[threadIdx.x] = (uint32_t)thr.mblim[threadIdx.x] | ((uint32_t)thr.lim[threadIdx.x] << 8) | ((uint32_t)thr.hev_thr[threadIdx.x] << 16);
     __syncthreads();
@@ -498,8 +503,14 @@
 }
 }
 
-static int32_t lf_launch(svt_hip_ctx *ctx, int n_pics, const svt_yuv_planes *d_recon, const svt_lf_mask *const *d_lfm, const int32_t *lfm_stride,
-                         const svt_lf_thresh *thr, const int32_t *mi_rows, const int32_t *mi_cols, int32_t y_only) {
+size_t svt_lf_desc_bytes(int n_pics, const int32_t *mi_rows) {
+    int max_rows = 0;
+    for (int i = 0; i < n_pics; i++) { const int r = (mi_rows[i] + 7) / 8; max_rows = r > max_rows ? r : max_rows; }
+    return ((sizeof(lf_pic_dev) * (size_t)n_pics + 15) & ~(size_t)15) + ((((size_t)n_pics * (size_t)max_rows + 4) * 4 + 15) & ~(size_t)15);
+}
+
+int32_t svt_lf_fill(svt_hip_ctx *ctx, int n_pics, const svt_yuv_planes *d_recon, const svt_lf_mask *const *d_lfm, const int32_t *lfm_stride,
+                    const svt_lf_thresh *thr, const int32_t *mi_rows, const int32_t *mi_cols, int32_t y_only, void *h_, void *d_, svt_lf_plan *plan) {
     int max_rows = 0, max_cols = 0;
     for (int i = 0; i < n_pics; i++) {
         if (mi_rows[i] < 1 || mi_cols[i] < 1 || d_recon[i].width != mi_cols[i] * 8 || d_recon[i].height != mi_rows[i] * 8)
@@ -511,13 +522,9 @@
         if (r > max_rows) max_rows = r;
         if (cc > max_cols) max_cols = cc;
     }
-    HIP_TRY(hipSetDevice(ctx->device));
     const size_t desc_bytes = (sizeof(lf_pic_dev) * (size_t)n_pics + 15) & ~(size_t)15;
-    const size_t cnt_words  = (size_t)n_pics * max_rows + 4;
-    lf_pic_dev  *h = nullptr;
-    uint8_t     *d = nullptr;
-    if (svt_ctx_stage(ctx, desc_bytes + cnt_words * 4, (void **)&h, (void **)&d)) return svt_set_error(SVT_HIP_ERR_NO_RESOURCES, "lf: scratch");
-    uint32_t *cnt = (uint32_t *)(d + desc_bytes);
+    lf_pic_dev  *h = (lf_pic_dev *)h_;
+    uint32_t    *cnt = (uint32_t *)((uint8_t *)d_ + desc_bytes);
     uint32_t *edesc = (uint32_t *)svt_ctx_slot(ctx, 24, (size_t)n_pics * max_rows * max_cols * LF_DESC_WORDS * sizeof(uint32_t));
     if (!edesc) return svt_set_error(SVT_HIP_ERR_NO_RESOURCES, "lf: descriptor buffer");
     for (int i = 0; i < n_pics; i++) {
@@ -525,15 +532,21 @@
         h[i].y_only = y_only; h[i].progress = cnt + 4 + (size_t)i * max_rows;
         h[i].desc = edesc + (size_t)i * max_rows * max_cols * LF_DESC_WORDS;
     }
-    HIP_TRY(hipMemcpyAsync(d, h, sizeof(lf_pic_dev) * (size_t)n_pics, hipMemcpyHostToDevice, ctx->stream));
-    HIP_TRY(hipMemsetAsync(cnt, 0, cnt_words * 4, ctx->stream));
-    HIP_TRY(hipEventRecord(ctx->ev_start, ctx->stream));
+    plan->d = d_; plan->cnt = cnt; plan->n_pics = n_pics; plan->max_rows = max_rows; plan->max_cols = max_cols;
+    plan->cnt_words = n_pics * max_rows + 4; plan->thr = *thr; plan->upload_bytes = sizeof(lf_pic_dev) * (size_t)n_pics;
+    return SVT_HIP_OK;
+}
+
+int32_t svt_lf_enqueue(svt_hip_ctx *ctx, const svt_lf_plan *plan, const int32_t *mi_rows, const int32_t *mi_cols) {
+    const int   n_pics = plan->n_pics, max_rows = plan->max_rows, max_cols = plan->max_cols;
+    const void *d = plan->d;
+    uint32_t   *cnt = plan->cnt;
     static const bool want_prof = getenv("SVT_HIP_LF_PROFILE") != nullptr;
     if (want_prof) { unsigned long long z[8] = {0}; HIP_TRY(hipMemcpyToSymbol(HIP_SYMBOL(g_lf_prof), z, sizeof z)); }
-    hipLaunchKernelGGL(svt_lf_desc_kernel, dim3(n_pics * max_rows * max_cols), dim3(128), 0, ctx->stream, (const lf_pic_dev *)d, max_rows, max_cols, *thr);
+    hipLaunchKernelGGL(svt_lf_desc_kernel, dim3(n_pics * max_rows * max_cols), dim3(128), 0, ctx->stream, (const lf_pic_dev *)d, max_rows, max_cols, plan->thr, cnt,
+                       plan->cnt_words);
     hipLaunchKernelGGL(svt_lf_kernel, dim3(n_pics * max_rows), dim3(256), 0, ctx->stream, (const lf_pic_dev *)d, n_pics, cnt, max_rows, want_prof ? 1 : 0);
     HIP_TRY(hipGetLastError());
-    HIP_TRY(hipEventRecord(ctx->ev_stop, ctx->stream));
     if (want_prof) {
         unsigned long long hp[8];
         HIP_TRY(hipStreamSynchronize(ctx->stream));
@@ -556,6 +569,22 @@
             }
         }
     }
+    return SVT_HIP_OK;
+}
+
+static int32_t lf_launch(svt_hip_ctx *ctx, int n_pics, const svt_yuv_planes *d_recon, const svt_lf_mask *const *d_lfm, const int32_t *lfm_stride,
+                         const svt_lf_thresh *thr, const int32_t *mi_rows, const int32_t *mi_cols, int32_t y_only) {
+    HIP_TRY(hipSetDevice(ctx->device));
+    void *h = nullptr, *d = nullptr;
+    if (svt_ctx_stage(ctx, svt_lf_desc_bytes(n_pics, mi_rows), &h, &d)) return svt_set_error(SVT_HIP_ERR_NO_RESOURCES, "lf: scratch");
+    svt_lf_plan plan;
+    int32_t     rc = svt_lf_fill(ctx, n_pics, d_recon, d_lfm, lfm_stride, thr, mi_rows, mi_cols, y_only, h, d, &plan);
+    if (rc) return rc;
+    HIP_TRY(hipMemcpyAsync(d, h, plan.upload_bytes, hipMemcpyHostToDevice, ctx->stream));
+    HIP_TRY(hipEventRecord(ctx->ev_start, ctx->stream));
+    rc = svt_lf_enqueue(ctx, &plan, mi_rows, mi_cols);
+    if (rc) return rc;
+    HIP_TRY(hipEventRecord(ctx->ev_stop, ctx->stream));
     svt_ctx_stage_commit(ctx);
     ctx->timed = 1;
     return SVT_HIP_OK;
diff --git a/svt-vp9_amd/csrc/mc_kernel.hip b/svt-vp9_amd/csrc/mc_kernel.hip
--- a/svt-vp9_amd/csrc/mc_kernel.hip
+++ b/svt-vp9_amd/csrc/mc_kernel.hip
@@ -137,7 +137,11 @@
     }
 }
 
-int mc_launch(svt_hip_ctx *ctx, int n_pics, const svt_mc_picture *pics) {
+}
+
+size_t svt_mc_desc_bytes(int n_pics) { return (sizeof(mc_pic_dev) * (size_t)n_pics + 15) & ~(size_t)15; }
+
+int32_t svt_mc_fill(int n_pics, const svt_mc_picture *pics, void *h_, const void *d, svt_mc_plan *plan) {
     int max_rows = 0, max_cols = 0;
     for (int i = 0; i < n_pics; i++) {
         const svt_mc_picture &p = pics[i];
@@ -150,28 +154,39 @@
         max_rows = p.mi_rows > max_rows ? p.mi_rows : max_rows;
         max_cols = p.mi_cols > max_cols ? p.mi_cols : max_cols;
     }
-    mc_pic_dev *h = nullptr, *d = nullptr;
-    if (svt_ctx_stage(ctx, sizeof(mc_pic_dev) * (size_t)n_pics, (void **)&h, (void **)&d)) return svt_set_error(SVT_HIP_ERR_NO_RESOURCES, "mc: scratch");
+    mc_pic_dev *h = (mc_pic_dev *)h_;
     for (int i = 0; i < n_pics; i++) {
         h[i].mi = pics[i].d_mi; h[i].mi_stride = pics[i].mi_stride; h[i].mi_rows = pics[i].mi_rows; h[i].mi_cols = pics[i].mi_cols;
         h[i].ref[0] = pics[i].ref[0]; h[i].ref[1] = pics[i].ref[1]; h[i].pred = pics[i].pred; h[i].use_subpel = pics[i].use_subpel;
     }
+    plan->d = d; plan->max_rows = max_rows;
+    plan->xblocks = (max_cols + 31) / 32; plan->total = plan->xblocks * max_rows * n_pics; plan->chunk = (plan->total + 7) / 8;
+    return SVT_HIP_OK;
+}
+
+int32_t svt_mc_enqueue(svt_hip_ctx *ctx, const svt_mc_plan *plan) {
+    hipLaunchKernelGGL(svt_mc_kernel, dim3(plan->chunk * 8), dim3(128), 0, ctx->stream, (const mc_pic_dev *)plan->d, plan->max_rows, plan->xblocks, plan->total, plan->chunk);
+    HIP_TRY(hipGetLastError());
+    return SVT_HIP_OK;
+}
+
+extern "C" int32_t svt_hip_inter_pred_batch_device(svt_hip_ctx *ctx, int32_t n_pics, const svt_mc_picture *pics) {
+    if (!ctx || n_pics < 1 || !pics) return svt_set_error(SVT_HIP_ERR_BAD_PARAMETER, "mc: null argument");
+    HIP_TRY(hipSetDevice(ctx->device));
+    const size_t bytes = svt_mc_desc_bytes(n_pics);
+    void        *h = nullptr, *d = nullptr;
+    if (svt_ctx_stage(ctx, bytes, &h, &d)) return svt_set_error(SVT_HIP_ERR_NO_RESOURCES, "mc: scratch");
+    svt_mc_plan plan;
+    int32_t     rc = svt_mc_fill(n_pics, pics, h, d, &plan);
+    if (rc) return rc;
     HIP_TRY(hipMemcpyAsync(d, h, sizeof(mc_pic_dev) * (size_t)n_pics, hipMemcpyHostToDevice, ctx->stream));
     HIP_TRY(hipEventRecord(ctx->ev_start, ctx->stream));
-    const int xblocks = (max_cols + 31) / 32, total = xblocks * max_rows * n_pics, chunk = (total + 7) / 8;
-    hipLaunchKernelGGL(svt_mc_kernel, dim3(chunk * 8), dim3(128), 0, ctx->stream, (const mc_pic_dev *)d, max_rows, xblocks, total, chunk);
-    HIP_TRY(hipGetLastError());
+    rc = svt_mc_enqueue(ctx, &plan);
+    if (rc) return rc;
     HIP_TRY(hipEventRecord(ctx->ev_stop, ctx->stream));
     svt_ctx_stage_commit(ctx);
     ctx->timed = 1;
     return SVT_HIP_OK;
-}
-}
-
-extern "C" int32_t svt_hip_inter_pred_batch_device(svt_hip_ctx *ctx, int32_t n_pics, const svt_mc_picture *pics) {
-    if (!ctx || n_pics < 1 || !pics) return svt_set_error(SVT_HIP_ERR_BAD_PARAMETER, "mc: null argument");
-    HIP_TRY(hipSetDevice(ctx->device));
-    return mc_launch(ctx, n_pics, pics);
 }
 
 extern "C" int32_t svt_hip_inter_pred_frame(svt_hip_ctx *ctx, const svt_mc_mode_info *mi, int32_t mi_stride, int32_t mi_rows, int32_t mi_cols,
@@ -210,7 +225,7 @@
     HIP_TRY(hipMemcpyAsync(dp + ysz, pred_u, csz, hipMemcpyHostToDevice, ctx->stream));
     HIP_TRY(hipMemcpyAsync(dp + ysz + csz, pred_v, csz, hipMemcpyHostToDevice, ctx->stream));
     p.pred.y = dp; p.pred.u = dp + ysz; p.pred.v = dp + ysz + csz; p.pred.y_stride = W; p.pred.uv_stride = W / 2; p.pred.width = W; p.pred.height = H;
-    int32_t rc = mc_launch(ctx, 1, &p);
+    int32_t rc = svt_hip_inter_pred_batch_device(ctx, 1, &p);
     if (rc) return rc;
     HIP_TRY(hipMemcpyAsync(pred_y, dp, ysz, hipMemcpyDeviceToHost, ctx->stream));
     HIP_TRY(hipMemcpyAsync(pred_u, dp + ysz, csz, hipMemcpyDeviceToHost, ctx->stream));
diff --git a/svt-vp9_amd/csrc/refpad_kernel.hip b/svt-vp9_amd/csrc/refpad_kernel.hip
--- a/svt-vp9_amd/csrc/refpad_kernel.hip
+++ b/svt-vp9_amd/csrc/refpad_kernel.hip
@@ -67,15 +67,11 @@
 }
 }
 
-extern "C" int32_t svt_hip_ref_pad_batch_device(svt_hip_ctx *ctx, int32_t n_pics, const svt_yuv_planes *pics, int32_t pad_x, int32_t pad_y) {
-    if (!ctx || n_pics < 1 || !pics) return svt_set_error(SVT_HIP_ERR_BAD_PARAMETER, "ref_pad: null argument");
-    if (pad_x < 0 || pad_y < 0 || (pad_x & 1) || (pad_y & 1)) return svt_set_error(SVT_HIP_ERR_BAD_PARAMETER, "ref_pad: padding must be even and >= 0");
-    if (!pad_x && !pad_y) return SVT_HIP_OK;
-    HIP_TRY(hipSetDevice(ctx->device));
-    const int n_jobs = 3 * n_pics;
-    rp_job   *h = nullptr, *d = nullptr;
-    if (svt_ctx_stage(ctx, sizeof(rp_job) * (size_t)n_jobs, (void **)&h, (void **)&d)) return svt_set_error(SVT_HIP_ERR_NO_RESOURCES, "ref_pad: scratch");
-    int wgs = 0, k = 0;
+size_t svt_rp_desc_bytes(int n_pics) { return (sizeof(rp_job) * 3 * (size_t)n_pics + 15) & ~(size_t)15; }
+
+int32_t svt_rp_fill(int n_pics, const svt_yuv_planes *pics, int32_t pad_x, int32_t pad_y, void *h_, const void *d, svt_rp_plan *plan) {
+    rp_job *h = (rp_job *)h_;
+    int     wgs = 0, k = 0;
     for (int i = 0; i < n_pics; i++) {
         const svt_yuv_planes &P = pics[i];
         if (!P.y || !P.u || !P.v || P.width < 2 || P.height < 2 || (P.width & 1) || (P.height & 1))
@@ -91,10 +87,30 @@
             wgs += (J.h + 2 * J.pad_y + RP_ROWS - 1) / RP_ROWS;
         }
     }
-    HIP_TRY(hipMemcpyAsync(d, h, sizeof(rp_job) * (size_t)n_jobs, hipMemcpyHostToDevice, ctx->stream));
+    plan->d = d; plan->n_jobs = 3 * n_pics; plan->wgs = wgs;
+    return SVT_HIP_OK;
+}
+
+int32_t svt_rp_enqueue(svt_hip_ctx *ctx, const svt_rp_plan *plan) {
+    hipLaunchKernelGGL(svt_refpad_kernel, dim3(plan->wgs), dim3(256), 0, ctx->stream, (const rp_job *)plan->d, plan->n_jobs);
+    HIP_TRY(hipGetLastError());
+    return SVT_HIP_OK;
+}
+
+extern "C" int32_t svt_hip_ref_pad_batch_device(svt_hip_ctx *ctx, int32_t n_pics, const svt_yuv_planes *pics, int32_t pad_x, int32_t pad_y) {
+    if (!ctx || n_pics < 1 || !pics) return svt_set_error(SVT_HIP_ERR_BAD_PARAMETER, "ref_pad: null argument");
+    if (pad_x < 0 || pad_y < 0 || (pad_x & 1) || (pad_y & 1)) return svt_set_error(SVT_HIP_ERR_BAD_PARAMETER, "ref_pad: padding must be even and >= 0");
+    if (!pad_x && !pad_y) return SVT_HIP_OK;
+    HIP_TRY(hipSetDevice(ctx->device));
+    void *h = nullptr, *d = nullptr;
+    if (svt_ctx_stage(ctx, svt_rp_desc_bytes(n_pics), &h, &d)) return svt_set_error(SVT_HIP_ERR_NO_RESOURCES, "ref_pad: scratch");
+    svt_rp_plan plan;
+    int32_t     rc = svt_rp_fill(n_pics, pics, pad_x, pad_y, h, d, &plan);
+    if (rc) return rc;
+    HIP_TRY(hipMemcpyAsync(d, h, sizeof(rp_job) * (size_t)plan.n_jobs, hipMemcpyHostToDevice, ctx->stream));
     HIP_TRY(hipEventRecord(ctx->ev_start, ctx->stream));
-    hipLaunchKernelGGL(svt_refpad_kernel, dim3(wgs), dim3(256), 0, ctx->stream, (const rp_job *)d, n_jobs);
-    HIP_TRY(hipGetLastError());
+    rc = svt_rp_enqueue(ctx, &plan);
+    if (rc) return rc;
     HIP_TRY(hipEventRecord(ctx->ev_stop, ctx->stream));
     svt_ctx_stage_commit(ctx);
     ctx->timed = 1;
diff --git a/svt-vp9_amd/csrc/svt_ctx.h b/svt-vp9_amd/csrc/svt_ctx.h
--- a/svt-vp9_amd/csrc/svt_ctx.h
+++ b/svt-vp9_amd/csrc/svt_ctx.h
@@ -49,10 +49,32 @@
 void    svt_ctx_stage_commit(svt_hip_ctx *ctx);
 void   *svt_ctx_slot(svt_hip_ctx *ctx, int slot, size_t bytes);
 
-int32_t svt_tq_launch_device_lists(svt_hip_ctx *ctx, const uint8_t *d_src, const uint8_t *d_pred, uint8_t *const *recon_set, int n_set,
+struct svt_tq_pic_rec {
+    svt_lf_mode_info *lf_mi;
+    uint8_t          *nz;
+    uint16_t         *eob_map;
+    int32_t           mi_stride, pad_;
+    svt_tq_pic_geom   g;
+};
+
+int32_t svt_tq_launch_device_lists(svt_hip_ctx *ctx, const uint8_t *d_src, const uint8_t *d_pred, const uint8_t *const *d_recon_set,
                                    const svt_tq_block *d_blocks, const int32_t cap[4], const int32_t *d_off_cnt, const svt_quant_tables *d_qtabs,
                                    const int16_t *d_iscan, int16_t *d_qcoeff, int16_t *d_dqcoeff, uint16_t *d_eob, uint64_t *d_dist,
                                    const uint32_t *d_pos, const void *d_geom, int geom_stride, const uint32_t *d_iscan_off, int sb_cols);
+
+struct svt_mc_plan { const void *d; int max_rows, xblocks, total, chunk; };
+size_t  svt_mc_desc_bytes(int n_pics);
+int32_t svt_mc_fill(int n_pics, const svt_mc_picture *pics, void *h, const void *d, svt_mc_plan *plan);
+int32_t svt_mc_enqueue(svt_hip_ctx *ctx, const svt_mc_plan *plan);
+struct svt_lf_plan { const void *d; uint32_t *cnt; int n_pics, max_rows, max_cols, cnt_words; svt_lf_thresh thr; size_t upload_bytes; };
+size_t  svt_lf_desc_bytes(int n_pics, const int32_t *mi_rows);
+int32_t svt_lf_fill(svt_hip_ctx *ctx, int n_pics, const svt_yuv_planes *d_recon, const svt_lf_mask *const *d_lfm, const int32_t *lfm_stride,
+                    const svt_lf_thresh *thr, const int32_t *mi_rows, const int32_t *mi_cols, int32_t y_only, void *h, void *d, svt_lf_plan *plan);
+int32_t svt_lf_enqueue(svt_hip_ctx *ctx, const svt_lf_plan *plan, const int32_t *mi_rows, const int32_t *mi_cols);
+struct svt_rp_plan { const void *d; int n_jobs, wgs; };
+size_t  svt_rp_desc_bytes(int n_pics);
+int32_t svt_rp_fill(int n_pics, const svt_yuv_planes *pics, int32_t pad_x, int32_t pad_y, void *h, const void *d, svt_rp_plan *plan);
+int32_t svt_rp_enqueue(svt_hip_ctx *ctx, const svt_rp_plan *plan);
 
 int32_t svt_intra_launch(svt_hip_ctx *ctx, const svt_encdec_picture *p, int32_t width, int32_t height, int32_t mi_stride, const svt_quant_tables *d_qtabs,
                          const int16_t *d_iscan, const uint32_t iscan_off[16], int32_t *d_sync, int32_t *d_status, int32_t mixed);
diff --git a/svt-vp9_amd/csrc/tq_core.h b/svt-vp9_amd/csrc/tq_core.h
--- a/svt-vp9_amd/csrc/tq_core.h
+++ b/svt-vp9_amd/csrc/tq_core.h
@@ -1,6 +1,7 @@
 #ifndef SVT_TQ_CORE_H
 #define SVT_TQ_CORE_H
 #include <hip/hip_runtime.h>
+#include <stddef.h>
 #include "svt_ctx.h"
 #include "txfm1d.h"
 #include "encdec_core.h"
@@ -18,6 +19,22 @@
     const int32_t *p; int s;
     const uint32_t *pos; const uint8_t *geom; int geom_stride; const uint32_t *iscan_off; int sb_cols;
 };
+
+__device__ __forceinline__ void tq_store_maps(const tq_dev_count &dc, const uint32_t p, const int eob) {
+    const int pic = (int)(p >> 24) & 63, plane = (int)(p >> 22) & 3, y4 = (int)(p >> 11) & 0x7ff, x4 = (int)p & 0x7ff;
+    const svt_tq_pic_rec *M = (const svt_tq_pic_rec *)(dc.geom + (size_t)pic * dc.geom_stride - offsetof(svt_tq_pic_rec, g));
+    if (!M->eob_map) return;
+    const int w4 = M->g.width >> 2, h4 = M->g.height >> 2;
+    const int pw4 = plane ? w4 >> 1 : w4;
+    const int off = plane == 0 ? 0 : w4 * h4 + (plane == 2 ? (w4 >> 1) * (h4 >> 1) : 0);
+    M->eob_map[off + y4 * pw4 + x4] = (uint16_t)eob;
+    if (eob) {
+        const int uy = plane ? y4 : y4 >> 1, ux = plane ? x4 : x4 >> 1;
+        const int sb_type = M->lf_mi[uy * M->mi_stride + ux].sb_type;
+        const int w8 = svt_blk_w8(sb_type), h8 = svt_blk_h8(sb_type);
+        M->nz[(uy - uy % h8) * M->mi_stride + (ux - ux % w8)] = 1;
+    }
+}
 
 struct tq_walk { int per_xcd, first, step, base; };
 __device__ __forceinline__ tq_walk tq_walk_of(int ngroups) {
diff --git a/svt-vp9_amd/csrc/tq_kernel.hip b/svt-vp9_amd/csrc/tq_kernel.hip
--- a/svt-vp9_amd/csrc/tq_kernel.hip
+++ b/svt-vp9_amd/csrc/tq_kernel.hip
@@ -57,8 +57,9 @@
     }
     int32_t *bits_slot = nullptr;
     if constexpr (RATE) bits_slot = ra.bits + blk;
-    tq_block_body<N, RATE, DIST>(k, active, i, t, srow, prow, qtabs, iscan_all, qcoeff, dqcoeff, eob_out + blk, dist_out ? dist_out + 2 * blk : nullptr, bits_slot,
-                                 ra.T, s_tc, s_scan, recon_set ? (uint8_t *)recon_set[(k.pad_[0] >> 4) & 7] : recon);
+    const int eob = tq_block_body<N, RATE, DIST>(k, active, i, t, srow, prow, qtabs, iscan_all, qcoeff, dqcoeff, eob_out + blk, dist_out ? dist_out + 2 * blk : nullptr,
+                                                 bits_slot, ra.T, s_tc, s_scan, recon_set ? (uint8_t *)recon_set[(k.pad_[0] >> 4) & 7] : recon);
+    if constexpr (!RATE && !DIST) if (dc.pos && active && i == 0) tq_store_maps(dc, dc.pos[blk], eob);
     tq_block_sync();
   }
 }
@@ -250,7 +251,7 @@
 }
 
 template <int N, bool RATE, bool DIST>
-__global__ __launch_bounds__(256) void svt_tq_lane_kernel(const uint8_t *__restrict__ src, const uint8_t *__restrict__ pred,
+__global__ __launch_bounds__(256) __attribute__((amdgpu_waves_per_eu((RATE || DIST) ? 1 : 8))) void svt_tq_lane_kernel(const uint8_t *__restrict__ src, const uint8_t *__restrict__ pred,
                                                           uint8_t *__restrict__ recon, const svt_tq_block *__restrict__ blocks,
                                                           int n_blocks, const svt_quant_tables *__restrict__ qtabs,
                                                           const int16_t *__restrict__ iscan_all, int16_t *__restrict__ qcoeff,
@@ -284,6 +285,12 @@
         svt_tq_block_from_pos(pc, txcfg<N>::size, (const svt_tq_pic_geom *)(dc.geom + (size_t)svt_tq_pos_pic(pc) * dc.geom_stride), dc.iscan_off, dc.sb_cols, &k);
     } else k = blocks[blk];
     tq_lane_block<N, RATE, DIST>(k, blk, src, pred, recon, qtabs, iscan_all, qcoeff, dqcoeff, eob_out, dist_out, ra, s_tc, s_vc, recon_set);
+    if constexpr (!RATE && !DIST) if (dc.pos) {
+        int tid = (int)threadIdx.x;
+        asm volatile("" : "+v"(tid) : : "memory");
+        const int b2 = (wk.base + gj) * 256 + tid;
+        tq_store_maps(dc, dc.pos[b2], eob_out[b2]);
+    }
   }
 }
 
@@ -341,17 +348,11 @@
 }
 }
 
-int32_t svt_tq_launch_device_lists(svt_hip_ctx *ctx, const uint8_t *d_src, const uint8_t *d_pred, uint8_t *const *recon_set, int n_set,
+int32_t svt_tq_launch_device_lists(svt_hip_ctx *ctx, const uint8_t *d_src, const uint8_t *d_pred, const uint8_t *const *d_set,
                                    const svt_tq_block *d_blocks, const int32_t cap[4], const int32_t *d_off_cnt, const svt_quant_tables *d_qtabs,
                                    const int16_t *d_iscan, int16_t *d_qcoeff, int16_t *d_dqcoeff, uint16_t *d_eob, uint64_t *d_dist,
                                    const uint32_t *d_pos, const void *d_geom, int geom_stride, const uint32_t *d_iscan_off, int sb_cols) {
-    HIP_TRY(hipSetDevice(ctx->device));
-    void *h = nullptr, *d = nullptr;
-    if (svt_ctx_stage(ctx, 8 * sizeof(void *), &h, &d)) return svt_set_error(SVT_HIP_ERR_NO_RESOURCES, "tq: descriptor buffers");
-    for (int i = 0; i < 8; i++) ((uint8_t **)h)[i] = i < n_set ? recon_set[i] : nullptr;
-    HIP_TRY(hipMemcpyAsync(d, h, 8 * sizeof(void *), hipMemcpyHostToDevice, ctx->stream));
-    const uint8_t *const *d_set = (const uint8_t *const *)d;
-    const tq_rate_args none = {nullptr, nullptr, nullptr};
+    const tq_rate_args    none = {nullptr, nullptr, nullptr};
     hipError_t rc = hipSuccess;
 #define TQ_DEV(N, S, D) launch_tq<N, false, D>(ctx, d_src, d_pred, nullptr, d_blocks, cap[S], d_qtabs, d_iscan, d_qcoeff, d_dqcoeff, d_eob, d_dist, none, d_set, tq_dev_count{d_off_cnt, S, d_pos, (const uint8_t *)d_geom, geom_stride, d_iscan_off, sb_cols})
     if (d_dist) {
@@ -366,7 +367,6 @@
         if (rc == hipSuccess) rc = TQ_DEV(32, 3, false);
     }
 #undef TQ_DEV
-    svt_ctx_stage_commit(ctx);
     if (rc != hipSuccess) return svt_set_hip_error(rc, __FILE__, __LINE__);
     return SVT_HIP_OK;
 }
```

New measurement: 6171. -1.4%, worse.
